# dpkn31/Yade-OpenFOAM-coupling

Hardware: AMD Instinct MI355X
Metric: coupled_steps_per_sec (pimpleFoamYade 4-way, 10M particles / 4M cells per GPU) (higher is better)
Workload: dtype f64

## Files before the change

### yade-openfoam-coupling_amd/csrc/common.hpp

```cpp
#pragma once
#include <hip/hip_runtime.h>

#include <algorithm>
#include <cmath>
#include <cstdarg>
#include <cstdint>
#include <cstdio>
#include <cstring>
#include <string>
#include <vector>

#include "../../include/foamyade_hip.h"

namespace fy {

struct Options {
    std::string tree_cache_dir;
    int rebin_interval;
    int strip_blocks;
    bool halo_overlap;
    int ipc_slot_mb;
    long long ipc_timeout_ms;
    bool wire_trace;
    bool explicit_tree;
    bool no_locate_lists;
    int locate_stack;
    bool locate_wide;
    bool no_deep_vcycle;
    long long mg_replicate_below;
    bool localcomm_stream;
    bool no_fused_corrector;
    bool faces_from_arrays;
    bool no_pairs;
    bool no_tail_cache;
    int ipc_slot_kb;
};
Options options();

std::string& last_error();
int fail(int code, const char* fmt, ...);
bool pairs_disabled();
bool tail_cache_disabled();
bool locate_wide_forced();

#define FY_HIP(expr)                                                                                      \
    do {                                                                                                  \
        hipError_t _e = (expr);                                                                           \
        if (_e != hipSuccess)                                                                             \
            return ::fy::fail(FY_ERR_HIP, "%s failed: %s (%s:%d)", #expr, hipGetErrorString(_e), __FILE__, __LINE__); \
    } while (0)

#define FY_TRY(expr)                 \
    do {                             \
        int _rc = (expr);            \
        if (_rc != FY_OK) return _rc; \
    } while (0)

template <class T>
struct DevBuf {
    T* p = nullptr;
    size_t n = 0;
    DevBuf() = default;
    DevBuf(const DevBuf&) = delete;
    DevBuf& operator=(const DevBuf&) = delete;
    ~DevBuf() { release(); }
    void release() {
        if (p) (void)hipFree(p);
        p = nullptr;
        n = 0;
    }
    int reserve(size_t count) {
        if (count <= n) return FY_OK;
        release();
        size_t cap = count + count / 8 + 64;
        hipError_t e = hipMalloc((void**)&p, cap * sizeof(T));
        if (e != hipSuccess) {
            p = nullptr;
            return fail(FY_ERR_HIP, "hipMalloc(%zu bytes) failed: %s", cap * sizeof(T), hipGetErrorString(e));
        }
        n = cap;
        return FY_OK;
    }
    int alloc_exact(size_t count) {
        release();
        if (count == 0) return FY_OK;
        hipError_t e = hipMalloc((void**)&p, count * sizeof(T));
        if (e != hipSuccess) {
            p = nullptr;
            return fail(FY_ERR_HIP, "hipMalloc(%zu bytes) failed: %s", count * sizeof(T), hipGetErrorString(e));
        }
        n = count;
        return FY_OK;
    }
};

template <class T>
struct HostBuf {
    T* p = nullptr;
    size_t n = 0;
    HostBuf() = default;
    HostBuf(const HostBuf&) = delete;
    HostBuf& operator=(const HostBuf&) = delete;
    ~HostBuf() { release(); }
    void release() {
        if (p) (void)hipHostFree(p);
        p = nullptr;
        n = 0;
    }
    T* data() { return p; }
    T& operator[](size_t i) { return p[i]; }
    int reserve(size_t count) {
        if (count <= n) return FY_OK;
        release();
        const size_t cap = count + count / 8 + 64;
        hipError_t e = hipHostMalloc((void**)&p, cap * sizeof(T), hipHostMallocDefault);
        if (e != hipSuccess) {
            p = nullptr;
            return fail(FY_ERR_HIP, "hipHostMalloc(%zu bytes) failed: %s", cap * sizeof(T), hipGetErrorString(e));
        }
        n = cap;
        return FY_OK;
    }
};

struct EventTimer {
    hipEvent_t a = nullptr, b = nullptr;
    bool armed = false;
    int init() {
        FY_HIP(hipEventCreate(&a));
        FY_HIP(hipEventCreate(&b));
        return FY_OK;
    }
    void destroy() {
        if (a) (void)hipEventDestroy(a);
        if (b) (void)hipEventDestroy(b);
        a = b = nullptr;
    }
    void start(hipStream_t s) { (void)hipEventRecord(a, s); armed = true; }
    void stop(hipStream_t s) { (void)hipEventRecord(b, s); }
    double ms() {
        if (!armed) return 0.0;
        float t = 0.f;
        (void)hipEventSynchronize(b);
        (void)hipEventElapsedTime(&t, a, b);
        armed = false;
        return (double)t;
    }
};

struct PhaseMarks {
    static constexpr int kMax = 8;
    hipEvent_t ev[kMax] = {};
    bool set_[kMax] = {};
    int init() { for (auto& e : ev) FY_HIP(hipEventCreate(&e)); return FY_OK; }
    void destroy() { for (auto& e : ev) { if (e) (void)hipEventDestroy(e); e = nullptr; } }
    void clear() { for (auto& b : set_) b = false; }
    void mark(int i, hipStream_t s) { (void)hipEventRecord(ev[i], s); set_[i] = true; }
    double ms(int i, int j) {
        if (!set_[i] || !set_[j]) return 0.0;
        float t = 0.f;
        (void)hipEventSynchronize(ev[j]);
        (void)hipEventElapsedTime(&t, ev[i], ev[j]);
        return (double)t;
    }
};

struct KernelClock {
    std::vector<hipEvent_t> a, b;
    size_t used = 0;
    double total_ms = 0.0;
    int64_t launches = 0;
    bool on = false;
    size_t per_collect = 1;
    bool open_ = false;
    void begin(hipStream_t s) {
        open_ = false;
        if (!on || used >= per_collect) return;
        if (used == a.size()) { hipEvent_t x, y; (void)hipEventCreate(&x); (void)hipEventCreate(&y); a.push_back(x); b.push_back(y); }
        (void)hipEventRecord(a[used], s);
        open_ = true;
    }
    void end(hipStream_t s) {
        if (!open_) return;
        (void)hipEventRecord(b[used], s);
        ++used;
// ... 21 lines not shown
```

### yade-openfoam-coupling_amd/csrc/coupling.cpp

```cpp
#include "coupling.hpp"
#include "ldu.hpp"

#include <algorithm>
#include <cmath>
#include <chrono>
#include <cstdlib>
#include <functional>
#include <thread>

#include <sys/stat.h>
#include <unistd.h>

#include <atomic>

namespace fy {

static std::atomic<int> g_kernel_flags{-1};
static bool kernel_flag(int bit) {
    if (g_kernel_flags.load(std::memory_order_relaxed) < 0) (void)options();
    return (g_kernel_flags.load(std::memory_order_relaxed) >> bit) & 1;
}
bool pairs_disabled() { return kernel_flag(0); }
bool tail_cache_disabled() { return kernel_flag(1); }
bool locate_wide_forced() { return kernel_flag(2); }

Options options() {
    auto on = [](const char* nm) { const char* e = getenv(nm); return e != nullptr && *e != 0 && strcmp(e, "0") != 0; };
    auto num = [](const char* nm, long long unset) { const char* e = getenv(nm); return e ? atoll(e) : unset; };
    Options q{};
    if (const char* d = getenv("FOAMYADE_TREE_CACHE_DIR")) q.tree_cache_dir = d;
    q.rebin_interval = std::max(1, (int)num("FOAMYADE_REBIN_INTERVAL", 32));
    q.strip_blocks = (int)num("FOAMYADE_STRIP_BLOCKS", -1);
    q.halo_overlap = getenv("FOAMYADE_HALO_OVERLAP") == nullptr || on("FOAMYADE_HALO_OVERLAP");
    q.ipc_slot_mb = (int)num("FOAMYADE_IPC_SLOT_MB", 0);
    q.ipc_timeout_ms = num("FOAMYADE_IPC_TIMEOUT_MS", 0);
    q.wire_trace = getenv("FOAMYADE_WIRE_TRACE") != nullptr;
    q.explicit_tree = on("FOAMYADE_EXPLICIT_TREE");
    q.no_locate_lists = on("FOAMYADE_NO_LOCATE_LISTS");
    q.locate_stack = (int)num("FOAMYADE_LOCATE_STACK", -1);
    q.locate_wide = num("FOAMYADE_LOCATE_WIDE", 0) != 0;
    q.no_deep_vcycle = on("FOAMYADE_NO_DEEP_VCYCLE");
    q.mg_replicate_below = std::max(0LL, num("FOAMYADE_MG_REPLICATE_BELOW", 0));
    const char* ls = getenv("FOAMYADE_LOCALCOMM_STREAM");
    q.localcomm_stream = ls != nullptr && ls[0] == '1';
    q.no_fused_corrector = on("FOAMYADE_NO_FUSED_CORRECTOR");
    q.faces_from_arrays = on("FOAMYADE_FACES_FROM_ARRAYS");
    q.no_pairs = on("FOAMYADE_NO_PAIRS");
    q.no_tail_cache = on("FOAMYADE_NO_TAIL_CACHE");
    q.ipc_slot_kb = (int)num("FOAMYADE_IPC_SLOT_KB", 0);
    g_kernel_flags.store((q.no_pairs ? 1 : 0) | (q.no_tail_cache ? 2 : 0) | (q.locate_wide ? 4 : 0), std::memory_order_relaxed);
    return q;
}

std::string& last_error() {
    static thread_local std::string e;
    return e;
}

int fail(int code, const char* fmt, ...) {
    char buf[1024];
    va_list ap;
    va_start(ap, fmt);
    vsnprintf(buf, sizeof(buf), fmt, ap);
    va_end(ap);
    last_error() = buf;
    return code;
}

static const int TAG_SZ_BUFF = 1003, TAG_GRID_BBOX = 1001, TAG_YADE_DATA = 1002, TAG_FORCE = 1005, TAG_SEARCH_RES = 1004,
                 TAG_FLUID_DT = 1050, TAG_YADE_DT = 1060;

#define FY_TR(expr)                                                                             \
    do {                                                                                        \
        if ((expr) != 0) return fail(FY_ERR_TRANSPORT, "transport call failed: %s", #expr);     \
    } while (0)

int Coupling::create(const fy_mesh_desc* m, const fy_field_ptrs* f, int gaussian_interp, const fy_transport* tr, int device_ordinal) {
    if (!m || !f || m->n_cells <= 0 || !m->centres || !m->volumes) return fail(FY_ERR_INVALID, "fy_create: bad mesh/fields");
    int ndev = 0;
    if (hipGetDeviceCount(&ndev) != hipSuccess || ndev == 0)
        return fail(FY_ERR_NO_DEVICE, "no HIP device visible: libfoamyade_hip has no CPU path");
    if (device_ordinal < 0 || device_ordinal >= ndev) return fail(FY_ERR_INVALID, "device ordinal %d out of range (%d devices)", device_ordinal, ndev);
    device = device_ordinal;
    opt = options();
    FY_HIP(hipSetDevice(device));
    if (ext_stream) { stream = ext_stream; owns_stream = false; }
    else { FY_HIP(hipStreamCreate(&stream)); owns_stream = true; }
    mesh = *m;
    mesh.centres = nullptr; mesh.volumes = nullptr; mesh.xf = mesh.yf = mesh.zf = nullptr;
    n_cells = m->n_cells;
    gaussian = gaussian_interp != 0;
    structured = m->nx > 0;
    rectilinear = structured && m->xf && m->yf && m->zf;
    if (!gaussian && !structured && !ldu_geo) return fail(FY_ERR_UNSUPPORTED, "point-force mode needs the structured block description, or a general mesh's face addressing (fy_ldu_solver): the findCell stand-ins");
    if (structured && (int64_t)m->nx * m->ny * m->nz != m->n_cells) return fail(FY_ERR_INVALID, "nx*ny*nz != n_cells");
    if (tr) { transport = *tr; has_transport = true; }

    if (has_transport) {
        comm_sz_diff = std::abs(transport.world_size - transport.local_size);
        serial_yade = (comm_sz_diff == 1);
    } else {
        comm_sz_diff = 0; serial_yade = true;
    }

    {
        bool exact = structured && !rectilinear && !opt.explicit_tree && m->nx <= 1024 && m->ny <= 1024 && m->nz <= 4096 &&
                     n_cells < (1 << 25);
        if (exact)
            for (int k = 0; k < m->nz && exact; ++k) for (int j = 0; j < m->ny && exact; ++j) for (int i = 0; i < m->nx; ++i) {
                const size_t c = (size_t)i + (size_t)m->nx * (j + (size_t)m->ny * k);
                const double x = m->origin[0] + ((double)i + 0.5) * m->dx, y = m->origin[1] + ((double)j + 0.5) * m->dx, z = m->origin[2] + ((double)k + 0.5) * m->dx;
                if (x != m->centres[3 * c] || y != m->centres[3 * c + 1] || z != m->centres[3 * c + 2]) { exact = false; break; }
            }
        std::vector<int32_t> pre;
        std::string cache;
        const std::string& cache_dir = opt.tree_cache_dir;
        if (exact && !cache_dir.empty()) {
            char nm[512];
            snprintf(nm, sizeof(nm), "%s/fy_tree_%dx%dx%d_%016llx.bin", cache_dir.c_str(), m->nx, m->ny, m->nz,
                     (unsigned long long)(std::hash<double>()(m->dx) ^ (std::hash<double>()(m->origin[0]) << 1) ^ (std::hash<double>()(m->origin[1]) << 2) ^ (std::hash<double>()(m->origin[2]) << 3)));
            cache = nm;
        }
        auto load_cache = [&]() -> bool {
            FILE* f = fopen(cache.c_str(), "rb");
            if (!f) return false;
            pre.resize((size_t)n_cells);
            bool ok = fread(pre.data(), sizeof(int32_t), (size_t)n_cells, f) == (size_t)n_cells && fgetc(f) == EOF;
            fclose(f);
            for (size_t q = 0; ok && q < pre.size(); ++q) ok = pre[q] >= 0 && pre[q] < n_cells;
            if (!ok) pre.clear();
            return ok;
        };
        bool have = false, hold_lock = false;
        const std::string lock = cache + ".lock";
        if (!cache.empty()) {
            have = load_cache();
            if (!have) {
                const double kStaleLock = 60.0;
                auto lock_age = [&]() -> double {
                    struct stat sb;
                    if (stat(lock.c_str(), &sb) != 0) return -1.0;
                    return difftime(time(nullptr), sb.st_mtime);
                };
                for (int attempt = 0; attempt < 2 && !have && !hold_lock; ++attempt) {
                    FILE* lf = fopen(lock.c_str(), "wx");
                    if (lf) { fclose(lf); hold_lock = true; break; }
                    const int max_spins = (int)(kStaleLock * 20);
                    for (int spin = 0; spin < max_spins && !have; ++spin) {
                        const double age = lock_age();
                        if (age < 0 || age > kStaleLock) break;
                        std::this_thread::sleep_for(std::chrono::milliseconds(50));
                        have = load_cache();
                    }
                    if (!have) have = load_cache();
                    if (!have && lock_age() > kStaleLock) remove(lock.c_str());
                }
            }
        }
        const bool publish = !cache.empty() && !have;
        std::vector<KdNode> nodes;
        if (!have) {
            unsigned hw = std::thread::hardware_concurrency();
            build_kdtree_preorder(m->centres, n_cells, nodes, (int)std::min(hw ? hw : 1u, 8u));
            pre.resize((size_t)n_cells);
            for (size_t q = 0; q < nodes.size(); ++q) pre[q] = nodes[q].id;
            if (publish) {
                char sfx[64];
                snprintf(sfx, sizeof(sfx), ".tmp.%ld.%zx", (long)getpid(), std::hash<std::thread::id>()(std::this_thread::get_id()));
                const std::string tmp = cache + sfx;
                bool ok = false;
                if (FILE* f = fopen(tmp.c_str(), "wb")) {
                    ok = fwrite(pre.data(), sizeof(int32_t), pre.size(), f) == pre.size();
                    ok = (fclose(f) == 0) && ok;
                }
                if (!ok || rename(tmp.c_str(), cache.c_str()) != 0) remove(tmp.c_str());
            }
        }
        if (hold_lock) remove(lock.c_str());
        tree_levels = kdtree_levels(n_cells);
        if (exact) {
            std::vector<uint32_t> packed((size_t)n_cells);
            for (size_t q = 0; q < packed.size(); ++q) {
                const int id = pre[q];
                const int i = id % m->nx, j = (id / m->nx) % m->ny, k = id / (m->nx * m->ny);
                packed[q] = (uint32_t)i | ((uint32_t)j << 10) | ((uint32_t)k << 20);
            }
            FY_TRY(d_tree_packed.alloc_exact(packed.size()));
            FY_HIP(hipMemcpyAsync(d_tree_packed.p, packed.data(), packed.size() * sizeof(uint32_t), hipMemcpyHostToDevice, stream));
            implicit.ox = m->origin[0]; implicit.oy = m->origin[1]; implicit.oz = m->origin[2]; implicit.dx = m->dx;
            implicit.nx = m->nx; implicit.ny = m->ny; implicit.nz = m->nz;
            use_implicit = true;
            FY_HIP(hipStreamSynchronize(stream));
        } else {
            if (nodes.empty()) {
                build_kdtree_preorder(m->centres, n_cells, nodes, 1);
            }
            FY_TRY(d_tree.alloc_exact(nodes.size()));
            FY_HIP(hipMemcpyAsync(d_tree.p, nodes.data(), nodes.size() * sizeof(KdNode), hipMemcpyHostToDevice, stream));
            FY_HIP(hipStreamSynchronize(stream));
// ... 1238 lines not shown
```

### yade-openfoam-coupling_amd/csrc/fv_kernels.hip

```cpp
#include "fv_kernels.hpp"

#include "common.hpp"

#ifndef FY_FVK_GRADED
#define FY_FVK_GRADED 0
#endif

namespace fy {
#if FY_FVK_GRADED
namespace gr {
#endif
namespace {

constexpr double kSmall = 1e-15;

__device__ __forceinline__ void ijk_of(const FvGeo& g, int t, int& i, int& j, int& k) {
    i = t % g.nx;
    const int q = t / g.nx;
    j = q % g.ny;
    k = q / g.ny;
}
__device__ __forceinline__ int cidx(const FvGeo& g, int i, int j, int k) { return i + g.nx * (j + g.ny * (k + g.gz)); }
__device__ __forceinline__ int stride_of(const FvGeo& g, int d) { return d == 0 ? 1 : d == 1 ? g.nx : g.nx * g.ny; }
__device__ __forceinline__ size_t g_row_stride(const FvGeo& g) { return 3 * (size_t)g.nx * g.ny * (size_t)(g.nz + 2 * g.gz); }
// ... 426 lines not shown
    } else {
        const int c = cidx(g, i, j, k);
        fl = af * rAUf[f] * geo_sfd_face(g, D, q, ndim(g, D), i, j, k) * (p[c] - p[c - stride_of(g, D)]);
    }
    const double fa = fl / af;
    pflux[f] = g.pimple ? (phiForces[f] - fa) / rAUf[f] : fl;
    phi[f] = phiHbyA[f] - fa;
}
__global__ __launch_bounds__(256) void k_flux_correct_cells(FvGeo g, const double* __restrict__ p, CFace3 phiHbyA, CFace3 rAUf, CFace3 alphaf, CFace3 psn,
                                                            CFace3 phiForces, Face3 pflux, Face3 phi) {
    const int t = fv_block(g, blockIdx.x, gridDim.x) * 256 + (int)threadIdx.x;
    if (t >= g.Nc) return;
    int i, j, k; ijk_of(g, t, i, j, k);
#define FY_CALL(D, fi, fj, fk) { const size_t f = (size_t)fid(g, D, fi, fj, fk); \
        flux_correct_face<D>(g, f, fi, fj, fk, p, phiHbyA.a[D], rAUf.a[D], alphaf.a[D], psn.a[D], phiForces.a[D], pflux.a[D], phi.a[D]); }
    FY_CELL_FACES(g, i, j, k, FY_CALL);
#undef FY_CALL
}

__global__ __launch_bounds__(256) void k_courant(FvGeo g, CFace3 phi, double* __restrict__ partials) {
    double v[2] = {0.0, 0.0};
    FY_RED_LOOP_G(g, t) {
        int i, j, k; ijk_of(g, t, i, j, k);
        double s = 0.0;
#pragma unroll
        for (int d = 0; d < 3; ++d)
#pragma unroll
            for (int sd = 0; sd < 2; ++sd) s += fabs(phi.a[d][cface(g, d, sd, i, j, k)]);
        v[0] = fmax(v[0], s * geo_rV(g, i, j, k));
        v[1] += s;
    }
    const int mx[2] = {1, 0};
    block_reduce_store<2>(v, mx, partials, fy_lb, fy_stride);
}

__global__ __launch_bounds__(256) void k_pre_coupling(FvGeo g, const double* __restrict__ U, const double* __restrict__ p,
                                                      const double* __restrict__ alpha, CFace3 psn, double* __restrict__ vGrad,
                                                      double* __restrict__ gradP, double* __restrict__ divT, double* __restrict__ Gout,
                                                      int write_vgrad, int write_pfields, CFace3 phi, double* __restrict__ ddtU, double* __restrict__ Uold_out,
                                                      double* __restrict__ cellrec, double rec_two_nu, double rec_rhoF, Face3 dcorr) {
    const int t = fv_block(g, blockIdx.x, gridDim.x) * 256 + (int)threadIdx.x;
    if (t >= g.Nc) return;
    int i, j, k; ijk_of(g, t, i, j, k);
    const int c = t + g.c0;
    const bool pf = g.pimple && write_pfields;
    const int ijk[3] = {i, j, k};
    bool bnd[3][2];
#pragma unroll
    for (int d = 0; d < 3; ++d)
#pragma unroll
        for (int s = 0; s < 2; ++s) bnd[d][s] = onb(g, d, s, i, j, k);
    const double uc[3] = {U[3 * (size_t)c], U[3 * (size_t)c + 1], U[3 * (size_t)c + 2]};
    const double pc = pf ? p[c] : 0.0, ac = pf ? alpha[c] : 0.0;
    double un6[3][2][3], pn6[3][2], an6[3][2];
#pragma unroll
    for (int d = 1; d < 3; ++d)
#pragma unroll
        for (int s = 0; s < 2; ++s) {
            const int nb = bnd[d][s] ? c : c + (s ? stride_of(g, d) : -stride_of(g, d));
            un6[d][s][0] = U[3 * (size_t)nb]; un6[d][s][1] = U[3 * (size_t)nb + 1]; un6[d][s][2] = U[3 * (size_t)nb + 2];
            pn6[d][s] = pf ? p[nb] : 0.0; an6[d][s] = pf ? alpha[nb] : 0.0;
        }
    const bool want_phi = ddtU != nullptr || dcorr.a[0] != nullptr;
    double phf[3][2];
#pragma unroll
    for (int d = 0; d < 3; ++d)
#pragma unroll
        for (int s = 0; s < 2; ++s) phf[d][s] = want_phi ? phi.a[d][cface(g, d, s, i, j, k)] : 0.0;
    const int lane = threadIdx.x & 63;
    {
        const int xm = (lane == 0 && i > 0) ? c - 1 : c, xp = (lane == 63 && i + 1 < g.nx) ? c + 1 : c;
        double em[3] = {0, 0, 0}, ep[3] = {0, 0, 0}, epm = 0, epp = 0, eam = 0, eap = 0;
        if (lane == 0 || lane == 63) {
            for (int q = 0; q < 3; ++q) { em[q] = U[3 * (size_t)xm + q]; ep[q] = U[3 * (size_t)xp + q]; }
            if (pf) { epm = p[xm]; epp = p[xp]; eam = alpha[xm]; eap = alpha[xp]; }
        }
#pragma unroll
        for (int q = 0; q < 3; ++q) { un6[0][0][q] = wave_prev(uc[q]); un6[0][1][q] = wave_next(uc[q]); }
        pn6[0][0] = wave_prev(pc); pn6[0][1] = wave_next(pc); an6[0][0] = wave_prev(ac); an6[0][1] = wave_next(ac);
        if (lane == 0 && i > 0) { for (int q = 0; q < 3; ++q) un6[0][0][q] = em[q]; pn6[0][0] = epm; an6[0][0] = eam; }
        if (lane == 63 && i + 1 < g.nx) { for (int q = 0; q < 3; ++q) un6[0][1][q] = ep[q]; pn6[0][1] = epp; an6[0][1] = eap; }
    }
    if (Uold_out) { Uold_out[3 * (size_t)c] = uc[0]; Uold_out[3 * (size_t)c + 1] = uc[1]; Uold_out[3 * (size_t)c + 2] = uc[2]; }
    double lap[3] = {0, 0, 0}, T[9], conv[3] = {0, 0, 0}, gp3[3] = {0, 0, 0};
#pragma unroll
    for (int d = 0; d < 3; ++d) {
        double fv[2][3], fp[2] = {0, 0};
#pragma unroll
        for (int s = 0; s < 2; ++s) {
            if (bnd[d][s]) {
                const int patch = 2 * d + s;
                if (g.u_bc[patch] == 0) { fv[s][0] = g.u_val[patch][0]; fv[s][1] = g.u_val[patch][1]; fv[s][2] = g.u_val[patch][2]; }
                else { fv[s][0] = uc[0]; fv[s][1] = uc[1]; fv[s][2] = uc[2]; }
                if (g.u_bc[patch] == 2) fv[s][d] = 0.0;
                if (pf) {
                    fp[s] = pbv(g, p, psn, c, d, s, cface(g, d, s, i, j, k));
                    for (int q = 0; q < 3; ++q) lap[q] += 1.0 * geo_Af(g, d, i, j, k) * (fv[s][q] - uc[q]) * geo_rhalf(g, d, ijk[d]);
                }
            } else {
                const double* un = un6[d][s];
                const int qc = ijk[d];
                for (int q = 0; q < 3; ++q) fv[s][q] = geo_lerp_side(g, d, s, qc, uc[q], un[q]);
                if (pf) {
                    fp[s] = geo_lerp_side(g, d, s, qc, pc, pn6[d][s]);
                    const double af = geo_lerp_side(g, d, s, qc, ac, an6[d][s]);
                    for (int q = 0; q < 3; ++q) lap[q] += af * geo_Af(g, d, i, j, k) * (un[q] - uc[q]) * geo_rdelta(g, d, qc + s);
                }
            }
        }
        if (dcorr.a[0]) {
#pragma unroll
            for (int s = 0; s < 2; ++s)
                if (owns_face(g, d, s, i, j, k)) {
                    const int fi = i + (d == 0 ? s : 0), fj = j + (d == 1 ? s : 0), fk = k + (d == 2 ? s : 0);
                    const int f = cface(g, d, s, i, j, k);
                    const double uf = fv[s][d] * geo_Af(g, d, fi, fj, fk);
                    const double po = phf[d][s];
                    const double phiCorr = po - uf;
                    const bool fixes = bnd[d][s] && g.u_bc[2 * d + s] == 0;
                    const double coef = fixes ? 0.0 : 1.0 - fmin(fabs(phiCorr) / (fabs(po) + kSmall), 1.0);
                    dcorr.a[d][f] = coef * (1.0 / g.dt) * phiCorr;
                }
        }
        const double rhd = geo_rh(g, d, ijk[d]);
        for (int q = 0; q < 3; ++q) T[3 * d + q] = (fv[1][q] - fv[0][q]) * rhd;
        if (pf) gp3[d] = (fp[1] - fp[0]) * rhd;
        if (ddtU) {
#pragma unroll
            for (int s = 0; s < 2; ++s) {
                const double flux = (s ? 1.0 : -1.0) * phf[d][s];
                for (int q = 0; q < 3; ++q) conv[q] += flux * fv[s][q];
            }
        }
    }
    if (ddtU)
        for (int q = 0; q < 3; ++q) ddtU[3 * (size_t)c + q] = conv[q] * geo_rV(g, i, j, k);
    if (write_vgrad)
        for (int q = 0; q < 9; ++q) vGrad[9 * (size_t)c + q] = T[q];
    if (pf)
        for (int q = 0; q < 3; ++q) gradP[3 * (size_t)c + q] = gp3[q];
    if (pf) {
        double dT[3];
        for (int q = 0; q < 3; ++q) { dT[q] = 2 * g.nu * (lap[q] * geo_rV(g, i, j, k)); divT[3 * (size_t)c + q] = dT[q]; }
        if (cellrec) {
            double2* r = reinterpret_cast<double2*>(cellrec + 8 * (size_t)c);
            r[0] = make_double2(uc[0], uc[1]);
            r[1] = make_double2(uc[2], ac);
            r[2] = make_double2(((rec_two_nu * dT[0]) * rec_rhoF) - gp3[0], ((rec_two_nu * dT[1]) * rec_rhoF) - gp3[1]);
            r[3] = make_double2(((rec_two_nu * dT[2]) * rec_rhoF) - gp3[2], geo_V(g, i, j, k));
        }
    }
    if (Gout) {
        const double tr = T[0] + T[4] + T[8];
        const double an = g.nut ? alpha[c] * (g.nu + g.nut[c]) : alpha[c] * g.nu;
        const size_t rs = g_row_stride(g);
        for (int a = 0; a < 3; ++a)
            for (int b = 0; b < 3; ++b) Gout[(size_t)a * rs + 3 * (size_t)c + b] = an * (T[3 * b + a] - (a == b ? (2.0 / 3.0) * tr : 0.0));
    }
}

__global__ __launch_bounds__(256) void k_div_G(FvGeo g, const double* __restrict__ G, double* __restrict__ divG) {
    const int t = fv_block(g, blockIdx.x, gridDim.x) * 256 + (int)threadIdx.x;
    if (t >= g.Nc) return;
    int i, j, k; ijk_of(g, t, i, j, k);
    const int c = t + g.c0;
    const int ijk[3] = {i, j, k};
    const double g0[3] = {G[3 * (size_t)c], G[3 * (size_t)c + 1], G[3 * (size_t)c + 2]};
    double gx[2][3];
    x_neighbours3(G, c, i, g.nx, g0, gx[0], gx[1]);
    bool bnd[3][2];
    double own[3][3], nbv[3][2][3];
#pragma unroll
    for (int q = 0; q < 3; ++q) { own[0][q] = g0[q]; nbv[0][0][q] = gx[0][q]; nbv[0][1][q] = gx[1][q]; }
#pragma unroll
    for (int d = 0; d < 3; ++d)
#pragma unroll
        for (int s = 0; s < 2; ++s) bnd[d][s] = onb(g, d, s, i, j, k);
#pragma unroll
    for (int d = 1; d < 3; ++d) {
        const double* Gd = G + (size_t)d * g_row_stride(g);
#pragma unroll
        for (int q = 0; q < 3; ++q) own[d][q] = Gd[3 * (size_t)c + q];
#pragma unroll
        for (int s = 0; s < 2; ++s) {
            const int nb = bnd[d][s] ? c : c + (s ? stride_of(g, d) : -stride_of(g, d));
#pragma unroll
            for (int q = 0; q < 3; ++q) nbv[d][s][q] = Gd[3 * (size_t)nb + q];
        }
    }
    double acc[3] = {0, 0, 0};
#pragma unroll
    for (int d = 0; d < 3; ++d) {
        double fv[2][3];
#pragma unroll
        for (int s = 0; s < 2; ++s)
            for (int q = 0; q < 3; ++q) fv[s][q] = bnd[d][s] ? own[d][q] : geo_lerp_side(g, d, s, ijk[d], own[d][q], nbv[d][s][q]);
        for (int q = 0; q < 3; ++q) acc[q] += (fv[1][q] - fv[0][q]) * geo_rh(g, d, ijk[d]);
    }
    for (int q = 0; q < 3; ++q) divG[3 * (size_t)c + q] = acc[q];
}

__global__ __launch_bounds__(256) void k_smagorinsky_nut(FvGeo g, const double* __restrict__ vGrad, double ck, double ce, double delta, double* __restrict__ nut) {
    const int t = blockIdx.x * 256 + threadIdx.x;
    if (t >= g.Nc) return;
    const int c = t + g.c0;
    delta = geo_delta(g, delta, c);
    double T[9];
#pragma unroll
    for (int q = 0; q < 9; ++q) T[q] = vGrad[9 * (size_t)c + q];
    const double Dxx = T[0], Dyy = T[4], Dzz = T[8];
    const double Dxy = 0.5 * (T[1] + T[3]), Dxz = 0.5 * (T[2] + T[6]), Dyz = 0.5 * (T[5] + T[7]);
    const double trD = Dxx + Dyy + Dzz;
    const double a = ce / delta;
    const double b = (2.0 / 3.0) * trD;
    const double third = (1.0 / 3.0) * trD;
    const double dd = (Dxx - third) * Dxx + (Dyy - third) * Dyy + (Dzz - third) * Dzz + 2.0 * (Dxy * Dxy) + 2.0 * (Dxz * Dxz) + 2.0 * (Dyz * Dyz);
    const double cc = 2.0 * ck * delta * dd;
    const double r = (-b + sqrt(b * b + 4.0 * a * cc)) / (2.0 * a);
    const double kk = r * r;
    nut[c] = ck * delta * sqrt(kk);
}

__device__ __forceinline__ double wall_epsilon(const FvGeo& g, const TurbEqn& e, double kc, int c, int i, int j, int k) {
#if FY_FVK_GRADED
    double sum = 0.0;
    int W = 0;
#pragma unroll
    for (int d = 0; d < 3; ++d)
#pragma unroll
        for (int s = 0; s < 2; ++s)
            if (e.wall[2 * d + s] && onb(g, d, s, i, j, k)) { sum += e.cmu75 * pow(kc, 1.5) / (e.kappa * geo_ywall(g, d, c)); ++W; }
    return sum / (double)W;
#else
    return e.cmu75 * pow(kc, 1.5) / (e.kappa * geo_ywall(g, 0, c));
#endif
}

__global__ __launch_bounds__(256) void k_assemble_turb(FvGeo g, TurbEqn e, const double* __restrict__ kf, const double* __restrict__ ef,
                                                       const double* __restrict__ alpha, CFace3 alphaf, CFace3 phi, const double* __restrict__ vGrad,
                                                       const double* __restrict__ U, Mom7 M, double* __restrict__ b3, double* __restrict__ x3) {
    const int t = blockIdx.x * 256 + threadIdx.x;
    if (t >= g.Nc) return;
    int i, j, k; ijk_of(g, t, i, j, k);
    const int c = t + g.c0;
    const double nu = g.nu, dt = g.dt, V = geo_V(g, i, j, k);
    const double aP = alpha[c], nutc = g.nut[c];
    const double* X = e.mode == 1 ? ef : kf;
    const double xc = X[c];
    double dg = aP * V / dt;
    double src = aP * V * xc / dt;
    double sumPhi = 0.0, an[6];
#pragma unroll
    for (int d = 0; d < 3; ++d)
#pragma unroll
        for (int s = 0; s < 2; ++s) {
            const int f = cface(g, d, s, i, j, k);
            const double af = alphaf.a[d][f];
            const double pv = (s ? 1.0 : -1.0) * phi.a[d][f];
            const double phio = af * pv;
            sumPhi += pv;
            if (onb(g, d, s, i, j, k)) {
                an[2 * d + s] = 0.0;
                const int patch = 2 * d + s;
                const double nb = nut_boundary(g, patch, c);
                const double gam = (af * (nu + nb / e.sigma)) * geo_sfd(g, d, s, i, j, k);
                if (e.bc[patch] == 1) {
                    const double gb = kBfac * gam;
                    dg += gb;
                    src += (-phio + gb) * e.val[patch];
                } else {
                    dg += phio;
                }
            } else {
                const int nbc = c + (s ? stride_of(g, d) : -stride_of(g, d));
                const int qc = d == 0 ? i : d == 1 ? j : k;
                const double gam = geo_lerp_side(g, d, s, qc, aP * (nu + nutc / e.sigma), alpha[nbc] * (nu + g.nut[nbc] / e.sigma)) * geo_sfd(g, d, s, i, j, k);
                const double wP = geo_wown(g, d, s, qc);
#if FY_FVK_GRADED
                const double cP = e.upwind ? fmax(phio, 0.0) : wP * phio, cN = e.upwind ? fmin(phio, 0.0) : (1.0 - wP) * phio;
#else
                const double cP = e.upwind ? fmax(phio, 0.0) : wP * phio, cN = e.upwind ? fmin(phio, 0.0) : wP * phio;
#endif
                dg += cP + gam;
                an[2 * d + s] = cN - gam;
            }
        }
    double T[9];
#pragma unroll
    for (int q = 0; q < 9; ++q) T[q] = vGrad[9 * (size_t)c + q];
    const double tr2 = 2.0 * (T[0] + T[4] + T[8]);
    double GG = 0.0;
#pragma unroll
    for (int a = 0; a < 3; ++a)
#pragma unroll
        for (int b = 0; b < 3; ++b) GG += T[3 * a + b] * ((T[3 * a + b] + T[3 * b + a]) - (a == b ? (1.0 / 3.0) * tr2 : 0.0));
    double G = nutc * GG;
    int Wc = 0;
    double Gw = 0.0;
    if (e.mode != 0) {
#pragma unroll
        for (int d = 0; d < 3; ++d)
#pragma unroll
            for (int s = 0; s < 2; ++s)
                if (e.wall[2 * d + s] && onb(g, d, s, i, j, k)) {
                    const int patch = 2 * d + s;
                    double ub[3];
                    Ub(g, U, c, patch, ub);
                    const double ywall = geo_ywall(g, d, c);
                    const double d0 = (ub[0] - U[3 * (size_t)c]) / ywall, d1 = (ub[1] - U[3 * (size_t)c + 1]) / ywall, d2 = (ub[2] - U[3 * (size_t)c + 2]) / ywall;
                    const double magGradUw = sqrt(d0 * d0 + d1 * d1 + d2 * d2);
                    Gw += (nut_boundary(g, patch, c) + nu) * magGradUw * e.cmu25 * sqrt(kf[c]) / (e.kappa * ywall);
                    ++Wc;
                }
        if (Wc) G = Gw / (double)Wc;
    }
    const double divU = sumPhi * geo_rV(g, i, j, k);
    double Su, c1, c2;
    if (e.mode == 0) { Su = aP * G; c1 = (2.0 / 3.0) * aP * divU; c2 = e.ce * aP * sqrt(xc) / geo_delta(g, e.delta, c); }
    else if (e.mode == 1) { const double kc = kf[c]; Su = e.c1 * aP * G * xc / kc; c1 = ((2.0 / 3.0) * e.c1 - e.c3) * aP * divU; c2 = e.c2 * aP * xc / kc; }
    else { Su = aP * G; c1 = (2.0 / 3.0) * aP * divU; c2 = aP * ef[c] / xc; }
    dg += V * (fmax(c1, 0.0) + c2);
    src += V * Su - V * fmin(c1, 0.0) * xc;
    if (e.relax > 0) {
        double so = 0.0;
        for (int q = 0; q < 6; ++q) so += fabs(an[q]);
        const double dn = fmax(fabs(dg), so) / e.relax;
        src += (dn - dg) * xc;
        dg = dn;
    }
    double x0 = xc;
    if (e.mode == 1) {
        if (Wc) {
            const double v = wall_epsilon(g, e, kf[c], c, i, j, k);
            for (int q = 0; q < 6; ++q) an[q] = 0.0;
            src = dg * v;
            x0 = v;
        } else {
#pragma unroll
            for (int d = 0; d < 3; ++d)
#pragma unroll
                for (int s = 0; s < 2; ++s)
                    if (!onb(g, d, s, i, j, k)) {
                        const int ni = i + (d == 0 ? (s ? 1 : -1) : 0), nj = j + (d == 1 ? (s ? 1 : -1) : 0), nk = k + (d == 2 ? (s ? 1 : -1) : 0);
                        bool nwall = false;
#pragma unroll
                        for (int d2 = 0; d2 < 3; ++d2)
#pragma unroll
                            for (int s2 = 0; s2 < 2; ++s2) nwall = nwall || (e.wall[2 * d2 + s2] && onb(g, d2, s2, ni, nj, nk));
                        if (nwall) {
                            const int nbc = c + (s ? stride_of(g, d) : -stride_of(g, d));
                            src -= an[2 * d + s] * wall_epsilon(g, e, kf[nbc], nbc, ni, nj, nk);
                            an[2 * d + s] = 0.0;
                        }
                    }
        }
    }
    M.diag[c] = dg;
    for (int q = 0; q < 6; ++q) M.an[q][c] = an[q];
    b3[3 * (size_t)c] = src; b3[3 * (size_t)c + 1] = 0.0; b3[3 * (size_t)c + 2] = 0.0;
    x3[3 * (size_t)c] = x0; x3[3 * (size_t)c + 1] = 0.0; x3[3 * (size_t)c + 2] = 0.0;
}

__global__ __launch_bounds__(256) void k_turb_finish(FvGeo g, TurbEqn e, const double* __restrict__ x3, double* __restrict__ Xf, int nut_mode, double cmu,
                                                     const double* __restrict__ ef, double* __restrict__ nut) {
    const int t = blockIdx.x * 256 + threadIdx.x;
    if (t >= g.Nc) return;
    int i, j, k; ijk_of(g, t, i, j, k);
    const int c = t + g.c0;
    const double xc = x3[3 * (size_t)c];
    double xb = xc;
    if (!(xc > 0.0)) {
        const double mP = fmax(xc, e.xmin);
        double av = 0.0;
#if FY_FVK_GRADED
        double asum = 0.0;
#endif
#pragma unroll
        for (int d = 0; d < 3; ++d)
#pragma unroll
            for (int s = 0; s < 2; ++s) {
                double xf;
                if (onb(g, d, s, i, j, k)) {
                    const int patch = 2 * d + s;
                    xf = fmax(e.bc[patch] == 1 ? e.val[patch] : xc, e.xmin);
                } else {
                    const int nbc = c + (s ? stride_of(g, d) : -stride_of(g, d));
                    xf = geo_lerp_side(g, d, s, d == 0 ? i : d == 1 ? j : k, mP, fmax(x3[3 * (size_t)nbc], e.xmin));
                }
#if FY_FVK_GRADED
                const double Afc = geo_Af(g, d, i, j, k);
                av += Afc * xf; asum += Afc;
#else
                av += xf;
#endif
            }
#if FY_FVK_GRADED
        xb = fmax(xc, av / asum);
#else
        xb = fmax(xc, av / 6.0);
#endif
    }
    xb = fmax(xb, e.xmin);
    Xf[c] = xb;
    if (nut_mode == 1) nut[c] = e.ck * sqrt(xb) * geo_delta(g, e.delta, c);
    else if (nut_mode == 2) nut[c] = cmu * (xb * xb) / ef[c];
}

__device__ __forceinline__ double magsqr3(const double* __restrict__ F, int c) {
    const double a = F[3 * (size_t)c], b = F[3 * (size_t)c + 1], e = F[3 * (size_t)c + 2];
    return (a * a + b * b) + e * e;
}
__global__ __launch_bounds__(256) void k_grad_magsqr(FvGeo g, const double* __restrict__ U, double* __restrict__ gradL) {
    const int t = blockIdx.x * 256 + threadIdx.x;
    if (t >= g.Nc) return;
    int i, j, k; ijk_of(g, t, i, j, k);
    const int c = t + g.c0;
    const double lc = magsqr3(U, c);
#pragma unroll
    for (int d = 0; d < 3; ++d) {
        double fv[2];
#pragma unroll
        for (int s = 0; s < 2; ++s) {
            if (onb(g, d, s, i, j, k)) { double b[3]; Ub(g, U, c, 2 * d + s, b); fv[s] = (b[0] * b[0] + b[1] * b[1]) + b[2] * b[2]; }
            else fv[s] = geo_lerp_side(g, d, s, d == 0 ? i : d == 1 ? j : k, lc, magsqr3(U, c + (s ? stride_of(g, d) : -stride_of(g, d))));
        }
        gradL[3 * (size_t)c + d] = (fv[1] - fv[0]) * geo_rh(g, d, d == 0 ? i : d == 1 ? j : k);
    }
}
__device__ __forceinline__ double limiter_fn(int scheme, double twoByk, double r) {
    switch (scheme) {
        case 3: return fmax(fmin(twoByk * r, 1.0), 0.0);
        case 4: return (r + fabs(r)) / (1.0 + fabs(r));
        case 5: return fmax(fmin(fmin(2.0 * r, 0.5 * r + 0.5), 2.0), 0.0);
        case 6: return fmax(fmin(fmin(r, 1.0), 2.0), 0.0);
        case 7: return fmax(fmax(fmin(2.0 * r, 1.0), fmin(r, 2.0)), 0.0);
        default: return fmax(fmin((3.0 + r) / 4.0, 2.0), 0.0);
    }
}
__device__ __forceinline__ double limited_weight(const FvGeo& g, const double* __restrict__ U, const double* __restrict__ gradL, int d, int qn, int own,
                                                 int nei, double flux) {
    const double gradf = magsqr3(U, nei) - magsqr3(U, own);
    const double gradcf = (1.0 / geo_rdelta(g, d, qn)) * gradL[3 * (size_t)(flux > 0 ? own : nei) + d];
    double r;
    if (fabs(gradcf) >= 1000.0 * fabs(gradf)) r = 2.0 * 1000.0 * (gradcf >= 0 ? 1.0 : -1.0) * (gradf >= 0 ? 1.0 : -1.0) - 1.0;
    else r = 2.0 * (gradcf / gradf) - 1.0;
    const double lim = limiter_fn(g.upwind, g.lim_twoByk, r);
#if FY_FVK_GRADED
    const double wl = geo_wlow(g, d, qn);
#else
    const double wl = 0.5;
#endif
    return lim * wl + (1.0 - lim) * (flux >= 0 ? 1.0 : 0.0);
}

template <bool LIMITED>
__global__ __launch_bounds__(256) void k_assemble_momentum(FvGeo g, const double* __restrict__ U, const double* __restrict__ Uold,
                                                           const double* __restrict__ alpha, const double* __restrict__ alphaOld, CFace3 alphaf,
                                                           CFace3 phi, const double* __restrict__ uSource, const double* __restrict__ uSourceDrag,
                                                           const double* __restrict__ divG, const double* __restrict__ vGrad, Mom7 M,
                                                           double* __restrict__ src, double* __restrict__ rAU) {
    const int t = fv_block(g, blockIdx.x, gridDim.x) * 256 + (int)threadIdx.x;
    if (t >= g.Nc) return;
    int i, j, k; ijk_of(g, t, i, j, k);
    const int c = t + g.c0;
    const double nu = g.nu, dt = g.dt, V = geo_V(g, i, j, k);
    const bool pim = g.pimple != 0;
    const double aP = pim ? alpha[c] : 1.0, aP0 = pim ? alphaOld[c] : 1.0;
    double dg = aP * V / dt;
    double s3[3];
    for (int q = 0; q < 3; ++q) s3[q] = aP0 * V * Uold[3 * (size_t)c + q] / dt;
    double divAPhi = 0.0, an[6];
    double bd[3] = {0.0, 0.0, 0.0};
#pragma unroll
    for (int d = 0; d < 3; ++d)
#pragma unroll
        for (int s = 0; s < 2; ++s) {
            const int f = cface(g, d, s, i, j, k);
            double af = 1.0;
            if (pim) {
                if (alphaf.a[0]) af = alphaf.a[d][f];
                else if (!onb(g, d, s, i, j, k)) af = lerp_face(g, d, s, (d == 0 ? i : d == 1 ? j : k) + s, aP, alpha[c + (s ? stride_of(g, d) : -stride_of(g, d))]);
            }
            const double phio = (s ? 1.0 : -1.0) * af * phi.a[d][f];
            divAPhi += phio;
            const double geo = geo_sfd(g, d, s, i, j, k);
            double gam = nu * af * geo;
            if (g.nut) {
                if (onb(g, d, s, i, j, k)) {
                    const double nb = nut_boundary(g, 2 * d + s, c);
                    gam = (af * (nu + nb)) * geo;
                } else {
                    const int nbc = c + (s ? stride_of(g, d) : -stride_of(g, d));
                    gam = geo_lerp_side(g, d, s, d == 0 ? i : d == 1 ? j : k, aP * (nu + g.nut[c]), alpha[nbc] * (nu + g.nut[nbc])) * geo;
                }
            }
            if (onb(g, d, s, i, j, k)) {
                an[2 * d + s] = 0.0;
                const int patch = 2 * d + s;
                if (g.u_bc[patch] == 0) {
                    const double gb = kBfac * gam;
                    dg += gb;
                    for (int q = 0; q < 3; ++q) s3[q] += (-phio + gb) * g.u_val[patch][q];
                } else {
                    if (g.u_bc[patch] == 2) bd[d] += kBfac * gam;
                    dg += phio;
                }
            } else {
                const double wP = geo_wown(g, d, s, d == 0 ? i : d == 1 ? j : k);
#if FY_FVK_GRADED
                double cP = g.upwind ? fmax(phio, 0.0) : wP * phio, cN = g.upwind ? fmin(phio, 0.0) : (1.0 - wP) * phio;
#else
                double cP = g.upwind ? fmax(phio, 0.0) : wP * phio, cN = g.upwind ? fmin(phio, 0.0) : wP * phio;
#endif
                if (LIMITED) {
                    const int nb = c + (s ? stride_of(g, d) : -stride_of(g, d));
                    const int qc = d == 0 ? i : d == 1 ? j : k;
                    const double w = limited_weight(g, U, vGrad, d, qc + s, s ? c : nb, s ? nb : c, af * phi.a[d][f]);
                    cP = s ? phio * w : phio * (1.0 - w);
                    cN = s ? phio * (1.0 - w) : phio * w;
                }
                dg += cP + gam;
                an[2 * d + s] = cN - gam;
                if (g.upwind == 2) {
                    const int nb = c + (s ? stride_of(g, d) : -stride_of(g, d));
                    const int uw = phio > 0.0 ? c : nb;
                    const double half = (phio > 0.0 ? (s ? 0.5 : -0.5) : (s ? -0.5 : 0.5)) * geo_hc(g, d, uw);
                    for (int q = 0; q < 3; ++q) s3[q] -= phio * (half * vGrad[9 * (size_t)uw + 3 * d + q]);
                }
            }
        }
    if (pim) {
        const double S = (alpha[c] - alphaOld[c]) / dt + divAPhi / V;
        dg -= V * S;
        dg -= V * uSourceDrag[c];
        for (int q = 0; q < 3; ++q) s3[q] += V * divG[3 * (size_t)c + q];
        double so = 0.0;
        for (int q = 0; q < 6; ++q) so += fabs(an[q]);
        if (g.u_relax > 0) {
            const double dn = fmax(fabs(dg + ((bd[0] + bd[1]) + bd[2])), so) / g.u_relax;
            for (int q = 0; q < 3; ++q) s3[q] += (dn - dg) * U[3 * (size_t)c + q];
            dg = dn;
        }
    } else {
        for (int q = 0; q < 3; ++q) s3[q] += V * uSource[3 * (size_t)c + q];
    }
    M.diag[c] = dg;
    for (int q = 0; q < 6; ++q) M.an[q][c] = an[q];
    for (int q = 0; q < 3; ++q) src[3 * (size_t)c + q] = s3[q];
    double bav = 0.0;
    if (M.bd) { for (int q = 0; q < 3; ++q) M.bd[3 * (size_t)c + q] = bd[q]; bav = ((bd[0] + bd[1]) + bd[2]) / 3.0; }
    rAU[c] = 1.0 / ((dg + bav) / V);
}

__global__ __launch_bounds__(256) void k_bmom(FvGeo g, const double* __restrict__ src, const double* __restrict__ p, CFace3 psn,
                                              CFace3 phiForces, CFace3 rAUf, double* __restrict__ bmom) {
    const int t = fv_block(g, blockIdx.x, gridDim.x) * 256 + (int)threadIdx.x;
    if (t >= g.Nc) return;
    int i, j, k; ijk_of(g, t, i, j, k);
    const int c = t + g.c0;
    double out[3];
#pragma unroll
    for (int d = 0; d < 3; ++d) {
        if (!g.pimple) {
            double fv[2];
#pragma unroll
            for (int s = 0; s < 2; ++s) {
                if (onb(g, d, s, i, j, k)) fv[s] = pbv(g, p, psn, c, d, s, cface(g, d, s, i, j, k));
                else fv[s] = geo_lerp_side(g, d, s, d == 0 ? i : d == 1 ? j : k, p[c], p[c + (s ? stride_of(g, d) : -stride_of(g, d))]);
            }
            out[d] = src[3 * (size_t)c + d] - geo_V(g, i, j, k) * ((fv[1] - fv[0]) * geo_rh(g, d, d == 0 ? i : d == 1 ? j : k));
        } else {
            double sm = 0;
#pragma unroll
            for (int s = 0; s < 2; ++s) {
                const int f = cface(g, d, s, i, j, k);
                double sng;
                const double rds = geo_rdist(g, d, s, i, j, k);
                if (onb(g, d, s, i, j, k)) { const double pbd = pbv(g, p, psn, c, d, s, f); sng = s ? (pbd - p[c]) * rds : (p[c] - pbd) * rds; }
                else sng = s ? (p[c + stride_of(g, d)] - p[c]) * rds : (p[c] - p[c - stride_of(g, d)]) * rds;
                sm += phiForces.a[d][f] / rAUf.a[d][f] - sng * geo_Af(g, d, i, j, k);
            }
            out[d] = src[3 * (size_t)c + d] + geo_V(g, i, j, k) * (sm / (2.0 * geo_Af(g, d, i, j, k)));
        }
    }
    for (int d = 0; d < 3; ++d) bmom[3 * (size_t)c + d] = out[d];
}

__global__ __launch_bounds__(256) void k_bmom_faces(FvGeo g, const double* __restrict__ rAU, const double* __restrict__ uSource, const double* __restrict__ src,
                                                    const double* __restrict__ p, CFace3 psn, Face3 rf_out, Face3 pf_out, double* __restrict__ bmom) {
    const int t = fv_block(g, blockIdx.x, gridDim.x) * 256 + (int)threadIdx.x;
    if (t >= g.Nc) return;
    int i, j, k; ijk_of(g, t, i, j, k);
    const int c = t + g.c0;
    const int ijk[3] = {i, j, k};
    bool bnd[3][2]; int nb[3][2], fx[3][2];
#pragma unroll
    for (int d = 0; d < 3; ++d)
#pragma unroll
        for (int s = 0; s < 2; ++s) {
            bnd[d][s] = onb(g, d, s, i, j, k);
            nb[d][s] = bnd[d][s] ? c : c + (s ? stride_of(g, d) : -stride_of(g, d));
            fx[d][s] = cface(g, d, s, i, j, k);
        }
    const double rc = rAU[c], pc = p[c];
    const double us[3] = {uSource[3 * (size_t)c], uSource[3 * (size_t)c + 1], uSource[3 * (size_t)c + 2]};
    const double sr[3] = {src[3 * (size_t)c], src[3 * (size_t)c + 1], src[3 * (size_t)c + 2]};
    double rn[3][2], un[3][2], pn[3][2];
#pragma unroll
    for (int d = 0; d < 3; ++d)
#pragma unroll
        for (int s = 0; s < 2; ++s) { rn[d][s] = rAU[nb[d][s]]; un[d][s] = uSource[3 * (size_t)nb[d][s] + d]; pn[d][s] = p[nb[d][s]]; }
    double out[3];
#pragma unroll
    for (int d = 0; d < 3; ++d) {
        double sm = 0;
#pragma unroll
        for (int s = 0; s < 2; ++s) {
            const int q = ijk[d] + s;
            const int fi = i + (d == 0 ? s : 0), fj = j + (d == 1 ? s : 0), fk = k + (d == 2 ? s : 0);
            const bool b = bnd[d][s];
            const double Afc = geo_Af(g, d, fi, fj, fk);
            const double r = b ? rc : lerp_face(g, d, s, q, rc, rn[d][s]);
            const double fl = b ? 0.0 : lerp_face(g, d, s, q, rc * us[d], rn[d][s] * un[d][s]) * Afc;
            const double pfv = fl + r * (g.g[d] * Afc);
            if (owns_face(g, d, s, i, j, k)) { pf_out.a[d][fx[d][s]] = pfv; if (rf_out.a[0]) rf_out.a[d][fx[d][s]] = r; }
            double sng;
            const double rds = geo_rdist(g, d, s, i, j, k);
            if (b) { const double pbd = pbv(g, p, psn, c, d, s, fx[d][s]); sng = s ? (pbd - pc) * rds : (pc - pbd) * rds; }
            else sng = s ? (pn[d][s] - pc) * rds : (pc - pn[d][s]) * rds;
            sm += pfv / r - sng * geo_Af(g, d, i, j, k);
        }
        out[d] = sr[d] + geo_V(g, i, j, k) * (sm / (2.0 * geo_Af(g, d, i, j, k)));
    }
    for (int d = 0; d < 3; ++d) bmom[3 * (size_t)c + d] = out[d];
}

template <bool WITH_H>
__global__ __launch_bounds__(256) void k_mom_pass(FvGeo g, Mom7 M, const double* __restrict__ b, const double* __restrict__ x,
                                                  double* __restrict__ xn, const double* __restrict__ xsum, double n_glob, double* __restrict__ partials,
                                                  const double* __restrict__ hsrc, const double* __restrict__ rAU, double* __restrict__ HbyA) {
    double v[6] = {0, 0, 0, 0, 0, 0};
    const double xb[3] = {xsum[0] / n_glob, xsum[1] / n_glob, xsum[2] / n_glob};
    FY_RED_LOOP_G(g, t) {
        int i, j, k; ijk_of(g, t, i, j, k);
        const int c = t + g.c0;
        const double dg = M.diag[c];
        double dq[3] = {dg, dg, dg};
        if (M.bd) for (int q = 0; q < 3; ++q) dq[q] += M.bd[3 * (size_t)c + q];
        double off[3] = {0, 0, 0}, rowsum = dg;
        const double xc[3] = {x[3 * (size_t)c], x[3 * (size_t)c + 1], x[3 * (size_t)c + 2]};
        double hacc[3] = {0, 0, 0};
        if (WITH_H) { hacc[0] = hsrc[3 * (size_t)c]; hacc[1] = hsrc[3 * (size_t)c + 1]; hacc[2] = hsrc[3 * (size_t)c + 2]; }
        double xx[2][3];
        x_neighbours3(x, c, i, g.nx, xc, xx[0], xx[1]);
#pragma unroll
        for (int d = 0; d < 3; ++d)
#pragma unroll
            for (int s = 0; s < 2; ++s)
                if (!onb(g, d, s, i, j, k)) {
                    const int nb = c + (s ? stride_of(g, d) : -stride_of(g, d));
                    const double a = M.an[2 * d + s][c];
                    rowsum += a;
                    double xv[3];
                    if (d == 0) for (int q = 0; q < 3; ++q) xv[q] = xx[s][q];
                    else for (int q = 0; q < 3; ++q) xv[q] = x[3 * (size_t)nb + q];
                    for (int q = 0; q < 3; ++q) off[q] += a * xv[q];
                    if (WITH_H) for (int q = 0; q < 3; ++q) hacc[q] -= a * xv[q];
                }
        if (WITH_H) {
            if (M.bd) {
                const double b0 = M.bd[3 * (size_t)c], b1 = M.bd[3 * (size_t)c + 1], b2 = M.bd[3 * (size_t)c + 2];
                const double bav = ((b0 + b1) + b2) / 3.0;
                hacc[0] += (bav - b0) * xc[0]; hacc[1] += (bav - b1) * xc[1]; hacc[2] += (bav - b2) * xc[2];
            }
            const double r = rAU[c];
            for (int q = 0; q < 3; ++q) HbyA[3 * (size_t)c + q] = r * (hacc[q] * geo_rV(g, i, j, k));
        }
        for (int q = 0; q < 3; ++q) {
            const double bq = b[3 * (size_t)c + q];
            const double Ax = dq[q] * xc[q] + off[q];
            const double Aref = (rowsum + (dq[q] - dg)) * xb[q];
            v[q] += fabs(bq - Ax);
            v[3 + q] += fabs(Ax - Aref) + fabs(bq - Aref);
            xn[3 * (size_t)c + q] = (bq - off[q]) / dq[q];
        }
    }
    const int mx[6] = {0, 0, 0, 0, 0, 0};
    block_reduce_store<6>(v, mx, partials, fy_lb, fy_stride);
// ... 23 lines not shown
                const double a = M.an[2 * d + s][c];
                for (int q = 0; q < 3; ++q) acc[q] -= a * U[3 * (size_t)nb + q];
            }
    if (M.bd) {
        const double b0 = M.bd[3 * (size_t)c], b1 = M.bd[3 * (size_t)c + 1], b2 = M.bd[3 * (size_t)c + 2];
        const double bav = ((b0 + b1) + b2) / 3.0;
        acc[0] += (bav - b0) * U[3 * (size_t)c]; acc[1] += (bav - b1) * U[3 * (size_t)c + 1]; acc[2] += (bav - b2) * U[3 * (size_t)c + 2];
    }
    const double r = rAU[c];
    for (int q = 0; q < 3; ++q) HbyA[3 * (size_t)c + q] = r * (acc[q] * geo_rV(g, i, j, k));
}

template <bool MATRIX>
__global__ __launch_bounds__(256) void k_assemble_pressure(FvGeo g, CFace3 phiHbyA, CFace3 rAUf, CFace3 alphaf, CFace3 psn,
                                                           const double* __restrict__ alpha, const double* __restrict__ alphaOld, PMat A,
                                                           double* __restrict__ rhs) {
    const int t = fv_block(g, blockIdx.x, gridDim.x) * 256 + (int)threadIdx.x;
    if (t >= g.Nc) return;
    int i, j, k; ijk_of(g, t, i, j, k);
    const int c = t + g.c0;
    const bool refc = g.need_ref && (i + g.nx * (j + g.ny * (k + g.kglob0))) == g.p_ref_cell;
    double dg = 0.0, r = 0.0, up[3] = {0, 0, 0};
#pragma unroll
    for (int d = 0; d < 3; ++d)
#pragma unroll
        for (int s = 0; s < 2; ++s) {
            const int f = cface(g, d, s, i, j, k);
            const double af = g.pimple ? alphaf.a[d][f] : 1.0;
            double ph = (s ? 1.0 : -1.0) * af * phiHbyA.a[d][f];
            const bool b = onb(g, d, s, i, j, k);
            if (b && g.p_bc[2 * d + s] == 2) ph = (s ? 1.0 : -1.0) * af * (phiHbyA.a[d][f] - rAUf.a[d][f] * geo_Af(g, d, i, j, k) * psn.a[d][f]);
            r -= ph;
            if (b) {
                const int patch = 2 * d + s;
                if (g.p_bc[patch] == 1) { const double gb = kBfac * af * rAUf.a[d][f] * geo_sfd(g, d, s, i, j, k); dg += gb; r += gb * g.p_val[patch]; }
            } else if (MATRIX || refc) {
                const double gg = af * rAUf.a[d][f] * geo_sfd(g, d, s, i, j, k);
                dg += gg;
                if (s) up[d] = gg;
            }
        }
    if (g.pimple) r -= geo_V(g, i, j, k) * (alpha[c] - alphaOld[c]) / g.dt;
    if (refc) { r += dg * g.p_ref_value; dg += dg; }
    if (MATRIX) { A.diag[c] = dg; A.ux[c] = up[0]; A.uy[c] = up[1]; A.uz[c] = up[2]; }
    rhs[c] = r;
}

__global__ __launch_bounds__(256) void k_p_ghost_uz(FvGeo g, CFace3 rAUf, CFace3 alphaf, PMat A) {
    const int t = blockIdx.x * 256 + threadIdx.x;
    if (t >= g.nx * g.ny) return;
    const double af = g.pimple ? alphaf.a[2][t] : 1.0;
    A.uz[g.c0 - g.nx * g.ny + t] = af * rAUf.a[2][t] * g.dx;
}

__global__ __launch_bounds__(256) void k_cont_err(FvGeo g, CFace3 phi, CFace3 alphaf, const double* __restrict__ alpha,
                                                  const double* __restrict__ alphaOld, double* __restrict__ partials) {
    double v[2] = {0, 0};
    FY_RED_LOOP_G(g, t) {
        int i, j, k; ijk_of(g, t, i, j, k);
        const int c = t + g.c0;
        double dv = 0;
#pragma unroll
        for (int d = 0; d < 3; ++d)
#pragma unroll
            for (int s = 0; s < 2; ++s) { const int f = cface(g, d, s, i, j, k); dv += (s ? 1.0 : -1.0) * (g.pimple ? alphaf.a[d][f] : 1.0) * phi.a[d][f]; }
        double ce = dv * geo_rV(g, i, j, k);
        if (g.pimple) ce += (alpha[c] - alphaOld[c]) / g.dt;
        v[0] += fabs(ce) * geo_V(g, i, j, k);
        v[1] += ce * geo_V(g, i, j, k);
    }
    const int mx[2] = {0, 0};
    block_reduce_store<2>(v, mx, partials, fy_lb, fy_stride);
}

template <bool DIAG>
__global__ __launch_bounds__(256) void k_U_correct(FvGeo g, const double* __restrict__ HbyA, const double* __restrict__ rAU,
                                                   const double* __restrict__ p, CFace3 psn, CFace3 phiForces, CFace3 pflux, CFace3 alphaf,
                                                   CFace3 rAUf, double* __restrict__ U, CFace3 phi, const double* __restrict__ alpha,
                                                   const double* __restrict__ alphaOld, double* __restrict__ partials) {
    double v[4] = {0, 0, 0, 0};
    FY_RED_LOOP_G(g, t) {
        int i, j, k; ijk_of(g, t, i, j, k);
        const int c = t + g.c0;
        const double r = rAU[c];
        double out[3];
        double dv = 0.0, sp = 0.0;
#pragma unroll
        for (int d = 0; d < 3; ++d) {
            if (!g.pimple) {
                double fv[2];
#pragma unroll
                for (int s = 0; s < 2; ++s) {
                    if (onb(g, d, s, i, j, k)) fv[s] = pbv(g, p, psn, c, d, s, cface(g, d, s, i, j, k));
                    else fv[s] = geo_lerp_side(g, d, s, d == 0 ? i : d == 1 ? j : k, p[c], p[c + (s ? stride_of(g, d) : -stride_of(g, d))]);
                }
                out[d] = HbyA[3 * (size_t)c + d] - r * ((fv[1] - fv[0]) * geo_rh(g, d, d == 0 ? i : d == 1 ? j : k));
            } else {
                double sm = 0;
#pragma unroll
                for (int s = 0; s < 2; ++s) sm += pflux.a[d][cface(g, d, s, i, j, k)];
                out[d] = HbyA[3 * (size_t)c + d] + r * (sm / (2.0 * geo_Af(g, d, i, j, k)));
            }
            if (DIAG) {
#pragma unroll
                for (int s = 0; s < 2; ++s) {
                    const int f = cface(g, d, s, i, j, k);
                    const double ph = phi.a[d][f];
                    dv += (s ? 1.0 : -1.0) * (g.pimple ? alphaf.a[d][f] : 1.0) * ph;
                    sp += fabs(ph);
                }
            }
        }
        for (int d = 0; d < 3; ++d) U[3 * (size_t)c + d] = out[d];
        if (DIAG) {
            double ce = dv * geo_rV(g, i, j, k);
            if (g.pimple) ce += (alpha[c] - alphaOld[c]) / g.dt;
            v[0] += fabs(ce) * geo_V(g, i, j, k);
            v[1] += ce * geo_V(g, i, j, k);
            v[2] = fmax(v[2], sp * geo_rV(g, i, j, k));
            v[3] += sp;
        }
    }
    if (DIAG) {
        const int mx[4] = {0, 0, 1, 0};
        block_reduce_store<4>(v, mx, partials, fy_lb, fy_stride);
    }
}

struct FaceSrc { CFace3 arr; const double* cell; };
template <int D>
__device__ __forceinline__ double alphaf_at(const FvGeo& g, const FaceSrc& a, size_t f, int fi, int fj, int fk) {
    if (!a.cell) return a.arr.a[D][f];
    const int q = D == 0 ? fi : D == 1 ? fj : fk;
    if (face_low_b(g, D, q) || face_high_b(g, D, q)) return 1.0;
    const int c = cidx(g, fi, fj, fk);
    return geo_lerp(g, D, q, a.cell[c - stride_of(g, D)], a.cell[c]);
}
template <int D>
__device__ __forceinline__ double rAUf_at(const FvGeo& g, const FaceSrc& a, size_t f, int fi, int fj, int fk) {
    if (!a.cell) return a.arr.a[D][f];
    const int q = D == 0 ? fi : D == 1 ? fj : fk;
    if (face_low_b(g, D, q)) return a.cell[cidx(g, fi, fj, fk)];
    if (face_high_b(g, D, q)) return a.cell[cidx(g, fi - (D == 0), fj - (D == 1), fk - (D == 2))];
    const int c = cidx(g, fi, fj, fk);
    return geo_lerp(g, D, q, a.cell[c - stride_of(g, D)], a.cell[c]);
}
#define FY_ALL_FACES(i, j, k, CALL) \
    do { CALL(0, 0, i, j, k); CALL(0, 1, i + 1, j, k); CALL(1, 0, i, j, k); CALL(1, 1, i, j + 1, k); CALL(2, 0, i, j, k); CALL(2, 1, i, j, k + 1); } while (0)


__device__ __forceinline__ double ub_normal(const FvGeo& g, int patch, int d, double own_d) {
    return g.u_bc[patch] == 0 ? g.u_val[patch][d] : (g.u_bc[patch] == 2 ? 0.0 : own_d);
}
template <bool DIAG, bool FFC>
__global__ __launch_bounds__(256) void k_corr_back(FvGeo g, const double* __restrict__ p, CFace3 phiHbyA, FaceSrc rAUf, FaceSrc alphaf, CFace3 psn,
                                                   CFace3 phiForces, Face3 phi, const double* __restrict__ HbyA, const double* __restrict__ rAU,
                                                   double* __restrict__ U, const double* __restrict__ alpha, const double* __restrict__ alphaOld,
                                                   double* __restrict__ partials) {
    double v[4] = {0, 0, 0, 0};
    FY_RED_LOOP_G(g, t) {
        int i, j, k; ijk_of(g, t, i, j, k);
        const int c = t + g.c0;
        const int ijk[3] = {i, j, k};
        const bool pim = g.pimple != 0;
        bool bnd[3][2]; int nb[3][2], fx[3][2];
#pragma unroll
        for (int d = 0; d < 3; ++d)
#pragma unroll
            for (int s = 0; s < 2; ++s) {
                bnd[d][s] = onb(g, d, s, i, j, k);
                nb[d][s] = bnd[d][s] ? c : c + (s ? stride_of(g, d) : -stride_of(g, d));
                fx[d][s] = cface(g, d, s, i, j, k);
            }
        const double pc = p[c], rc = rAU[c], ac = pim ? alpha[c] : 1.0;
        const double hb[3] = {HbyA[3 * (size_t)c], HbyA[3 * (size_t)c + 1], HbyA[3 * (size_t)c + 2]};
        double pn[3][2], rfv[3][2], afv[3][2], phh[3][2], pfo[3][2];
#pragma unroll
        for (int d = 0; d < 3; ++d)
#pragma unroll
            for (int s = 0; s < 2; ++s) {
                pn[d][s] = p[nb[d][s]];
                phh[d][s] = phiHbyA.a[d][fx[d][s]];
                pfo[d][s] = pim ? phiForces.a[d][fx[d][s]] : 0.0;
                if (FFC) { rfv[d][s] = rAU[nb[d][s]]; afv[d][s] = pim ? alpha[nb[d][s]] : 1.0; }
                else { rfv[d][s] = rAUf.arr.a[d][fx[d][s]]; afv[d][s] = pim ? alphaf.arr.a[d][fx[d][s]] : 1.0; }
            }
        double pfl[3][2], ph[3][2];
#pragma unroll
        for (int d = 0; d < 3; ++d)
#pragma unroll
            for (int s = 0; s < 2; ++s) {
                const int q = ijk[d] + s;
                const int fi = i + (d == 0 ? s : 0), fj = j + (d == 1 ? s : 0), fk = k + (d == 2 ? s : 0);
                const bool b = bnd[d][s];
                if (FFC) {
                    afv[d][s] = pim ? (b ? 1.0 : lerp_face(g, d, s, q, ac, afv[d][s])) : 1.0;
                    rfv[d][s] = b ? rc : lerp_face(g, d, s, q, rc, rfv[d][s]);
                }
                const double af = afv[d][s], rf = rfv[d][s];
                double fl = 0.0;
                if (b) {
                    const int patch = 2 * d + s;
                    if (g.p_bc[patch] == 1) { const double gb = kBfac * af * rf * geo_sfd_face(g, d, q, ndim(g, d), fi, fj, fk); fl = s ? gb * (g.p_val[patch] - pc) : gb * (pc - g.p_val[patch]); }
                    else if (g.p_bc[patch] == 2) fl = af * rf * geo_Af(g, d, fi, fj, fk) * psn.a[d][fx[d][s]];
                } else {
                    fl = af * rf * geo_sfd_face(g, d, q, ndim(g, d), fi, fj, fk) * (s ? pn[d][s] - pc : pc - pn[d][s]);
                }
                const double fa = fl / af;
                pfl[d][s] = pim ? (pfo[d][s] - fa) / rf : fl;
                ph[d][s] = phh[d][s] - fa;
                if (owns_face(g, d, s, i, j, k)) phi.a[d][fx[d][s]] = ph[d][s];
            }
        double out[3];
        double dv = 0.0, sp = 0.0;
#pragma unroll
        for (int d = 0; d < 3; ++d) {
            if (!pim) {
                double fv[2];
#pragma unroll
                for (int s = 0; s < 2; ++s) {
                    if (bnd[d][s]) fv[s] = pbv(g, p, psn, c, d, s, fx[d][s]);
                    else fv[s] = geo_lerp_side(g, d, s, ijk[d], pc, pn[d][s]);
                }
                out[d] = hb[d] - rc * ((fv[1] - fv[0]) * geo_rh(g, d, ijk[d]));
            } else {
                double sm = 0;
#pragma unroll
                for (int s = 0; s < 2; ++s) sm += pfl[d][s];
                out[d] = hb[d] + rc * (sm / (2.0 * geo_Af(g, d, i, j, k)));
            }
            if (DIAG) {
#pragma unroll
                for (int s = 0; s < 2; ++s) {
                    dv += (s ? 1.0 : -1.0) * (pim ? afv[d][s] : 1.0) * ph[d][s];
                    sp += fabs(ph[d][s]);
                }
            }
        }
        for (int d = 0; d < 3; ++d) U[3 * (size_t)c + d] = out[d];
        if (DIAG) {
            double ce = dv * geo_rV(g, i, j, k);
            if (pim) ce += (ac - alphaOld[c]) / g.dt;
            v[0] += fabs(ce) * geo_V(g, i, j, k);
            v[1] += ce * geo_V(g, i, j, k);
            v[2] = fmax(v[2], sp * geo_rV(g, i, j, k));
            v[3] += sp;
        }
    }
    if (DIAG) {
        const int mx[4] = {0, 0, 1, 0};
        block_reduce_store<4>(v, mx, partials, fy_lb, fy_stride);
    }
}

template <bool STORE_A, bool FFC>
__global__ __launch_bounds__(256) __attribute__((amdgpu_waves_per_eu(4))) void k_corr_front(FvGeo g, const double* __restrict__ HbyA, const double* __restrict__ U, CFace3 dcorr,
                                                    FaceSrc rAUf, FaceSrc alphaf, CFace3 phiForces, Face3 phiHbyA, Face3 psn,
                                                    const double* __restrict__ rAU, const double* __restrict__ alpha, const double* __restrict__ alphaOld, PMat A,
                                                    double* __restrict__ rhs, const double* __restrict__ x, const double* __restrict__ xbar_dev, double xsum_val,
                                                    double inv_n, double* __restrict__ res, double* __restrict__ partials) {
    double v[2] = {0, 0};
    const double xbar = (xbar_dev ? xbar_dev[0] : xsum_val) * inv_n;
    FY_RED_LOOP_G(g, t) {
        int i, j, k; ijk_of(g, t, i, j, k);
        const int c = t + g.c0;
        const int ijk[3] = {i, j, k};
        const bool pim = g.pimple != 0;
        const bool refc = g.need_ref && (i + g.nx * (j + g.ny * (k + g.kglob0))) == g.p_ref_cell;
        bool bnd[3][2]; int nb[3][2], fx[3][2];
#pragma unroll
        for (int d = 0; d < 3; ++d)
#pragma unroll
            for (int s = 0; s < 2; ++s) {
                bnd[d][s] = onb(g, d, s, i, j, k);
                nb[d][s] = bnd[d][s] ? c : c + (s ? stride_of(g, d) : -stride_of(g, d));
                fx[d][s] = cface(g, d, s, i, j, k);
            }
        const double xc = x[c], ac = pim ? alpha[c] : 1.0;
        const double rc = FFC ? rAU[c] : 0.0;
        const double hb[3] = {HbyA[3 * (size_t)c], HbyA[3 * (size_t)c + 1], HbyA[3 * (size_t)c + 2]};
        double hn[3][2], dc[3][2], pfo[3][2], xn[3][2], rfv[3][2], afv[3][2];
#pragma unroll
        for (int d = 0; d < 3; ++d)
#pragma unroll
            for (int s = 0; s < 2; ++s) {
                hn[d][s] = HbyA[3 * (size_t)nb[d][s] + d];
                dc[d][s] = dcorr.a[d][fx[d][s]];
                pfo[d][s] = pim ? phiForces.a[d][fx[d][s]] : 0.0;
                xn[d][s] = x[nb[d][s]];
                if (FFC) { rfv[d][s] = rAU[nb[d][s]]; afv[d][s] = pim ? alpha[nb[d][s]] : 1.0; }
                else { rfv[d][s] = rAUf.arr.a[d][fx[d][s]]; afv[d][s] = pim ? alphaf.arr.a[d][fx[d][s]] : 1.0; }
            }
        double dg = 0.0, r = 0.0, up[3] = {0, 0, 0};
        double gg6[3][2];
#pragma unroll
        for (int d = 0; d < 3; ++d)
#pragma unroll
            for (int s = 0; s < 2; ++s) {
                const int q = ijk[d] + s;
                const int fi = i + (d == 0 ? s : 0), fj = j + (d == 1 ? s : 0), fk = k + (d == 2 ? s : 0);
                const bool b = bnd[d][s];
                const int patch = 2 * d + s;
                if (FFC) {
                    afv[d][s] = pim ? (b ? 1.0 : lerp_face(g, d, s, q, ac, afv[d][s])) : 1.0;
                    rfv[d][s] = b ? rc : lerp_face(g, d, s, q, rc, rfv[d][s]);
                }
                const double af = afv[d][s], rf = rfv[d][s];
                const double Afc = geo_Af(g, d, fi, fj, fk);
                double pv = (b ? ub_normal(g, patch, d, hb[d]) : lerp_face(g, d, s, q, hb[d], hn[d][s])) * Afc;
                double add = rf * dc[d][s];
                if (pim) add *= af;
                pv += add;
                if (pim) pv += pfo[d][s];
                const bool own = owns_face(g, d, s, i, j, k);
                if (own) phiHbyA.a[d][fx[d][s]] = pv;
                double ph = (s ? 1.0 : -1.0) * af * pv;
                gg6[d][s] = 0.0;
                if (b) {
                    if (g.p_bc[patch] == 2) {
                        const double ubd = ub_normal(g, patch, d, g.u_bc[patch] == 1 ? U[3 * (size_t)c + d] : 0.0);
                        const double psn_v = (pv - ubd * Afc) / (rf * Afc);
                        if (own) psn.a[d][fx[d][s]] = psn_v;
                        ph = (s ? 1.0 : -1.0) * af * (pv - rf * geo_Af(g, d, i, j, k) * psn_v);
                    }
                    r -= ph;
                    if (g.p_bc[patch] == 1) { const double gb = kBfac * af * rf * geo_sfd(g, d, s, i, j, k); dg += gb; r += gb * g.p_val[patch]; }
                } else {
                    r -= ph;
                    const double gg = af * rf * geo_sfd(g, d, s, i, j, k);
                    dg += gg; gg6[d][s] = gg;
                    if (s) up[d] = gg;
                }
            }
        if (pim) r -= geo_V(g, i, j, k) * (ac - alphaOld[c]) / g.dt;
        if (refc) { r += dg * g.p_ref_value; dg += dg; }
        if (STORE_A) { A.diag[c] = dg; A.ux[c] = up[0]; A.uy[c] = up[1]; A.uz[c] = up[2]; }
        rhs[c] = r;
        double Ax = dg * xc, rs = dg;
#pragma unroll
        for (int d = 0; d < 3; ++d)
#pragma unroll
            for (int s = 0; s < 2; ++s)
                if (!bnd[d][s]) { Ax -= gg6[d][s] * xn[d][s]; rs -= gg6[d][s]; }
        const double Aref = rs * xbar;
        const double rr = r - Ax;
        res[c] = rr;
        v[0] += fabs(rr);
        v[1] += fabs(Ax - Aref) + fabs(r - Aref);
    }
    const int mx[2] = {0, 0};
    block_reduce_store<2>(v, mx, partials, fy_lb, fy_stride);
}

__device__ __forceinline__ double p_row(const PMat& A, const double* __restrict__ x, int c) {
    const int sy = A.nx, sz = A.nx * A.ny, last = A.ntot - 1;
    const int xm = max(c - 1, 0), xp = min(c + 1, last), ym = max(c - sy, 0), yp = min(c + sy, last), zm = max(c - sz, 0), zp = min(c + sz, last);
    const double uxc = A.ux[c], uyc = A.uy[c], uzc = A.uz[c];
    const double t0 = A.ux[xm] * x[xm], t1 = uxc * x[xp], t2 = A.uy[ym] * x[ym], t3 = uyc * x[yp], t4 = A.uz[zm] * x[zm], t5 = uzc * x[zp];
    double a = A.diag[c] * x[c];
    a = (c >= 1) ? a - t0 : a;
    a = (c + 1 < A.ntot) ? a - t1 : a;
    a = (c >= sy) ? a - t2 : a;
    a = (c + sy < A.ntot) ? a - t3 : a;
    a = (c >= sz) ? a - t4 : a;
    a = (c + sz < A.ntot) ? a - t5 : a;
    return a;
}
__device__ __forceinline__ double p_rowsum(const PMat& A, int c) {
    const int sy = A.nx, sz = A.nx * A.ny;
    double rs = A.diag[c];
    if (c >= 1) rs -= A.ux[c - 1];
    if (c + 1 < A.ntot) rs -= A.ux[c];
    if (c >= sy) rs -= A.uy[c - sy];
    if (c + sy < A.ntot) rs -= A.uy[c];
    if (c >= sz) rs -= A.uz[c - sz];
    if (c + sz < A.ntot) rs -= A.uz[c];
    return rs;
}

__global__ __launch_bounds__(256) void k_p_apply(PMat A, const double* __restrict__ x, double* __restrict__ y) {
    const int t = swz_block(blockIdx.x, gridDim.x) * 256 + threadIdx.x;
    if (t >= A.N) return;
    const int c = t + A.c0;
    y[c] = p_row(A, x, c);
}

template <bool WITH_R>
__global__ __launch_bounds__(256) void k_p_apply_dot(PMat A, const double* __restrict__ x, const double* __restrict__ r, double* __restrict__ y, double* __restrict__ partials) {
    double v[2] = {0, 0};
    FY_RED_LOOP(t, A.N) {
        const int c = t + A.c0;
        const double a = p_row(A, x, c);
        y[c] = a;
        const double xc = x[c];
        if (WITH_R) v[0] += xc * r[c];
        v[1] += a * xc;
    }
    if (WITH_R) {
        const int mx[2] = {0, 0};
        block_reduce_store<2>(v, mx, partials);
    } else {
        double v1[1] = {v[1]};
        const int mx[1] = {0};
        block_reduce_store<1>(v1, mx, partials + gridDim.x);
// ... 641 lines not shown
    }
    if (cached) for (int c = tid; c < T.cache_n; c += 1024) T.x1[0][c] = lx1[c];
}

__global__ __launch_bounds__(256) void k_mg_prolong_add(PMat A, double* __restrict__ x, PMat C, const double* __restrict__ xc) {
    const int t = blockIdx.x * 256 + threadIdx.x;
    if (t >= A.N) return;
    const int i = t % A.nx, q = t / A.nx, j = q % A.ny, k = q / A.ny;
    x[t + A.c0] += xc[C.c0 + (i >> 1) + C.nx * ((j >> 1) + C.ny * (k >> 1))];
}

__global__ __launch_bounds__(256) void k_mg_prolong_add_planes(PMat A, int kofs, double* __restrict__ x, PMat C, const double* __restrict__ xc) {
    const int t = blockIdx.x * 256 + threadIdx.x;
    if (t >= A.N) return;
    const int i = t % A.nx, q = t / A.nx, j = q % A.ny, k = q / A.ny + kofs;
    const int K = k >= 0 ? (k >> 1) : -((1 - k) >> 1);
    x[t + A.c0] += xc[C.c0 + (i >> 1) + C.nx * ((j >> 1) + C.ny * K)];
}

template <int Q>
__global__ __launch_bounds__(1024) void k_mg_coarse_factor(PMat A, int bw, double* __restrict__ fac) {
    extern __shared__ double B[];
    __shared__ int bad;
    const int N = A.N, tid = threadIdx.x, NT = (int)blockDim.x, Wd = bw + 1, sy = A.nx, sz = A.nx * A.ny;
    if (tid == 0) bad = 0;
    for (int e = tid; e < N * Wd; e += NT) B[e] = 0.0;
    __syncthreads();
    for (int c = tid; c < N; c += NT) {
        double* row = B + (size_t)c * Wd;
        row[0] += A.diag[c];
        if (c >= 1) row[1] -= A.ux[c - 1];
        if (A.ny > 1 && c >= sy && sy <= bw) row[sy] -= A.uy[c - sy];
        if (A.nz > 1 && c >= sz && sz <= bw) row[sz] -= A.uz[c - sz];
    }
    __syncthreads();
    int ua[Q], ub[Q];
#pragma unroll
    for (int q = 0; q < Q; ++q) {
        const int e = tid + NT * q;
        int a = (int)((sqrt(8.0 * (double)e + 1.0) - 1.0) * 0.5);
        while ((a + 1) * (a + 2) / 2 <= e) ++a;
        while (a * (a + 1) / 2 > e) --a;
        ua[q] = a; ub[q] = e - a * (a + 1) / 2;
    }
    for (int j = 0; j < N; ++j) {
        const double d = B[(size_t)j * Wd];
        if (!(d > 0.0) || !(d < 1e300)) { if (tid == 0) bad = 1; break; }
        const double id = 1.0 / d;
        const int m = min(bw, N - 1 - j);
#pragma unroll
        for (int q = 0; q < Q; ++q) {
            const int a = ua[q], b = ub[q];
            if (a < m) B[(size_t)(j + 1 + a) * Wd + (a - b)] -= (B[(size_t)(j + 1 + a) * Wd + 1 + a] * B[(size_t)(j + 1 + b) * Wd + 1 + b]) * id;
        }
        __syncthreads();
    }
    __syncthreads();
    if (!bad) {
        for (int i = tid; i < N; i += NT) fac[3 + (size_t)i * Wd] = 1.0 / sqrt(B[(size_t)i * Wd]);
        for (int e = tid; e < N * Wd; e += NT) {
            const int i = e / Wd, dd = e - i * Wd;
            if (dd >= 1) fac[3 + e] = dd <= i ? B[e] / sqrt(B[(size_t)(i - dd) * Wd]) : 0.0;
        }
    }
    if (tid == 0) { fac[0] = (double)N; fac[1] = (double)bw; fac[2] = bad ? 0.0 : 1.0; }
}

__global__ __launch_bounds__(1024) void k_mg_coarse_solve(PMat A, const double* __restrict__ b, double* __restrict__ x, double* __restrict__ tmp,
                                                          int sweeps, double w, const double* __restrict__ fac) {
    if (fac && A.N <= kMgDirectMax && fac[2] == 1.0) {
        extern __shared__ double fac_lds[];
        const int bw = (int)fac[1], cnt = A.N * (bw + 1);
        for (int q = threadIdx.x; q < cnt; q += 1024) fac_lds[q] = fac[3 + q];
        __syncthreads();
        if (threadIdx.x < 64) coarse_band_solve(fac_lds, A.N, bw, b, x, threadIdx.x);
        return;
    }
    const int c = threadIdx.x;
    const bool act = c < A.N;
    double* cur = x;
    double* nxt = tmp;
    if (act) cur[c] = w * b[c] / A.diag[c];
    __syncthreads();
    for (int s = 1; s < sweeps; ++s) {
        if (act) nxt[c] = cur[c] + w * (b[c] - p_row(A, cur, c)) / A.diag[c];
        __syncthreads();
        double* t = cur; cur = nxt; nxt = t;
    }
    if (cur != x) { if (act) x[c] = cur[c]; }
}

__global__ __launch_bounds__(256) void k_relax_field(double* __restrict__ x, const double* __restrict__ prev, double alpha, size_t n) {
    const size_t i = (size_t)blockIdx.x * 256 + threadIdx.x;
    if (i < n) x[i] = prev[i] + alpha * (x[i] - prev[i]);
}

__global__ __launch_bounds__(256) void k_copy(double* __restrict__ dst, const double* __restrict__ src, size_t n) {
    const size_t i = (size_t)blockIdx.x * 256 + threadIdx.x;
    if (i < n) dst[i] = src[i];
}

__global__ __launch_bounds__(256) void k_add(double* __restrict__ y, const double* __restrict__ x, size_t n) {
    const size_t i = (size_t)blockIdx.x * 256 + threadIdx.x;
    if (i < n) y[i] += x[i];
}

inline int fv_grid(const FvGeo& g) { return g.win_nblk > 0 ? g.win_nblk : div_up(g.Nc, 256); }
inline int fv_red_grid(const FvGeo& g) { return g.win_nblk > 0 ? g.win_nblk : red_blocks(g.Nc); }

#define FY_LAUNCH_CHECK()                                                                                     \
    do {                                                                                                      \
        hipError_t _e = hipGetLastError();                                                                    \
        if (_e != hipSuccess) return fail(FY_ERR_HIP, "kernel launch failed: %s (%s:%d)", hipGetErrorString(_e), __FILE__, __LINE__); \
    } while (0)

}

int launch_reduce_finalize(hipStream_t s, const double* partials, int n_cells, int nslots, const int* ops, double* out, unsigned long long* flag,
                           unsigned long long seq) {
    hipLaunchKernelGGL(k_reduce_finalize, dim3(nslots), dim3(1024), 0, s, partials, red_blocks(n_cells), ops, out, flag, seq);
    FY_LAUNCH_CHECK();
    return FY_OK;
}

int launch_flux_of(hipStream_t s, FvGeo g, const double* F, Face3 out) {
    hipLaunchKernelGGL(k_flux_of<0>, dim3(div_up(fv_fsize(g, 0), 256)), dim3(256), 0, s, g, F, out.a[0]);
    hipLaunchKernelGGL(k_flux_of<1>, dim3(div_up(fv_fsize(g, 1), 256)), dim3(256), 0, s, g, F, out.a[1]);
    hipLaunchKernelGGL(k_flux_of<2>, dim3(div_up(fv_fsize(g, 2), 256)), dim3(256), 0, s, g, F, out.a[2]);
    FY_LAUNCH_CHECK();
    return FY_OK;
}

int launch_courant(hipStream_t s, FvGeo g, CFace3 phi, double* partials) {
    hipLaunchKernelGGL(k_courant, dim3(fv_red_grid(g)), dim3(256), 0, s, g, phi, partials);
    FY_LAUNCH_CHECK();
    return FY_OK;
}

int launch_pre_coupling(hipStream_t s, FvGeo g, const double* U, const double* p, const double* alpha, CFace3 psn, double* vGrad,
                        double* gradP, double* divT, double* Gout, int write_vgrad, int write_pfields, CFace3 phi, double* ddtU, double* Uold_out,
                        double* cellrec, double rec_nu, double rec_rhoF, Face3 dcorr) {
    hipLaunchKernelGGL(k_pre_coupling, dim3(fv_grid(g)), dim3(256), 0, s, g, U, p, alpha, psn, vGrad, gradP, divT, Gout, write_vgrad, write_pfields,
                       phi, ddtU, Uold_out, cellrec, 2.0 * rec_nu, rec_rhoF, dcorr);
    FY_LAUNCH_CHECK();
    return FY_OK;
}

int launch_interp_alpha(hipStream_t s, FvGeo g, const double* alpha, Face3 af) {
    hipLaunchKernelGGL(k_interp_alpha_cells, dim3(fv_grid(g)), dim3(256), 0, s, g, alpha, af);
    FY_LAUNCH_CHECK();
    return FY_OK;
}

int launch_div_G(hipStream_t s, FvGeo g, const double* G, double* divG) {
    hipLaunchKernelGGL(k_div_G, dim3(fv_grid(g)), dim3(256), 0, s, g, G, divG);
    FY_LAUNCH_CHECK();
    return FY_OK;
}

int launch_assemble_turb(hipStream_t s, FvGeo g, TurbEqn e, const double* k, const double* eps, const double* alpha, CFace3 alphaf, CFace3 phi,
                         const double* vGrad, const double* U, Mom7 M, double* b3, double* x3) {
    hipLaunchKernelGGL(k_assemble_turb, dim3(fv_grid(g)), dim3(256), 0, s, g, e, k, eps, alpha, alphaf, phi, vGrad, U, M, b3, x3);
    FY_LAUNCH_CHECK();
    return FY_OK;
}

int launch_turb_finish(hipStream_t s, FvGeo g, TurbEqn e, const double* x3, double* X, int nut_mode, double cmu, const double* eps, double* nut) {
    hipLaunchKernelGGL(k_turb_finish, dim3(fv_grid(g)), dim3(256), 0, s, g, e, x3, X, nut_mode, cmu, eps, nut);
    FY_LAUNCH_CHECK();
    return FY_OK;
}

int launch_smagorinsky_nut(hipStream_t s, FvGeo g, const double* vGrad, double ck, double ce, double delta, double* nut) {
    hipLaunchKernelGGL(k_smagorinsky_nut, dim3(fv_grid(g)), dim3(256), 0, s, g, vGrad, ck, ce, delta, nut);
    FY_LAUNCH_CHECK();
    return FY_OK;
}

int launch_assemble_momentum(hipStream_t s, FvGeo g, const double* U, const double* Uold, const double* alpha, const double* alphaOld,
                             CFace3 alphaf, CFace3 phi, const double* uSource, const double* uSourceDrag, const double* divG, const double* vGrad,
                             Mom7 M, double* src, double* rAU) {
    if (g.upwind >= 3) hipLaunchKernelGGL(k_assemble_momentum<true>, dim3(fv_grid(g)), dim3(256), 0, s, g, U, Uold, alpha, alphaOld, alphaf, phi, uSource,
                                          uSourceDrag, divG, vGrad, M, src, rAU);
    else hipLaunchKernelGGL(k_assemble_momentum<false>, dim3(fv_grid(g)), dim3(256), 0, s, g, U, Uold, alpha, alphaOld, alphaf, phi, uSource,
                            uSourceDrag, divG, vGrad, M, src, rAU);
    FY_LAUNCH_CHECK();
    return FY_OK;
}
int launch_grad_magsqr(hipStream_t s, FvGeo g, const double* U, double* gradL) {
    hipLaunchKernelGGL(k_grad_magsqr, dim3(fv_grid(g)), dim3(256), 0, s, g, U, gradL);
    FY_LAUNCH_CHECK();
    return FY_OK;
}

int launch_interp_rAU(hipStream_t s, FvGeo g, const double* rAU, Face3 rf) {
    hipLaunchKernelGGL(k_interp_rAU<0>, dim3(div_up(fv_fsize(g, 0), 256)), dim3(256), 0, s, g, rAU, rf.a[0]);
    hipLaunchKernelGGL(k_interp_rAU<1>, dim3(div_up(fv_fsize(g, 1), 256)), dim3(256), 0, s, g, rAU, rf.a[1]);
    hipLaunchKernelGGL(k_interp_rAU<2>, dim3(div_up(fv_fsize(g, 2), 256)), dim3(256), 0, s, g, rAU, rf.a[2]);
    FY_LAUNCH_CHECK();
    return FY_OK;
}

int launch_bmom(hipStream_t s, FvGeo g, const double* src, const double* p, CFace3 psn, CFace3 phiForces, CFace3 rAUf, double* bmom) {
    hipLaunchKernelGGL(k_bmom, dim3(fv_grid(g)), dim3(256), 0, s, g, src, p, psn, phiForces, rAUf, bmom);
    FY_LAUNCH_CHECK();
    return FY_OK;
}

int launch_bmom_faces(hipStream_t s, FvGeo g, const double* rAU, const double* uSource, const double* src, const double* p, CFace3 psn, Face3 rAUf_out,
                      Face3 phiForces, double* bmom) {
    hipLaunchKernelGGL(k_bmom_faces, dim3(fv_grid(g)), dim3(256), 0, s, g, rAU, uSource, src, p, psn, rAUf_out, phiForces, bmom);
    FY_LAUNCH_CHECK();
    return FY_OK;
}

int launch_mom_pass(hipStream_t s, FvGeo g, Mom7 M, const double* b, const double* x, double* xn, const double* xsum, double n_glob, double* partials,
                    const double* hsrc, const double* rAU, double* HbyA) {
    if (HbyA) hipLaunchKernelGGL(k_mom_pass<true>, dim3(fv_red_grid(g)), dim3(256), 0, s, g, M, b, x, xn, xsum, n_glob, partials, hsrc, rAU, HbyA);
    else hipLaunchKernelGGL(k_mom_pass<false>, dim3(fv_red_grid(g)), dim3(256), 0, s, g, M, b, x, xn, xsum, n_glob, partials, hsrc, rAU, HbyA);
    FY_LAUNCH_CHECK();
    return FY_OK;
}

int launch_sum3(hipStream_t s, const double* x, int n, double* partials) {
    hipLaunchKernelGGL(k_sum3, dim3(red_blocks(n)), dim3(256), 0, s, x, n, partials);
    FY_LAUNCH_CHECK();
    return FY_OK;
}

int launch_HbyA(hipStream_t s, FvGeo g, Mom7 M, const double* src, const double* U, const double* rAU, double* HbyA) {
    hipLaunchKernelGGL(k_HbyA, dim3(fv_grid(g)), dim3(256), 0, s, g, M, src, U, rAU, HbyA);
    FY_LAUNCH_CHECK();
    return FY_OK;
}

int launch_phiHbyA(hipStream_t s, FvGeo g, const double* HbyA, const double* U, const double* Uold, CFace3 phiOld, CFace3 rAUf,
                   CFace3 alphaf, CFace3 phiForces, Face3 out, Face3 psn, Face3 ddtc, int keep) {
    if (keep == 1) hipLaunchKernelGGL(k_phiHbyA_cells<1>, dim3(fv_grid(g)), dim3(256), 0, s, g, HbyA, U, Uold, phiOld, rAUf, alphaf, phiForces, out, psn, ddtc);
    else if (keep == 2) hipLaunchKernelGGL(k_phiHbyA_cells<2>, dim3(fv_grid(g)), dim3(256), 0, s, g, HbyA, U, Uold, phiOld, rAUf, alphaf, phiForces, out, psn, ddtc);
    else hipLaunchKernelGGL(k_phiHbyA_cells<0>, dim3(fv_grid(g)), dim3(256), 0, s, g, HbyA, U, Uold, phiOld, rAUf, alphaf, phiForces, out, psn, ddtc);
    FY_LAUNCH_CHECK();
    return FY_OK;
}

int launch_adjust_phi_sums(hipStream_t s, FvGeo g, CFace3 phiHbyA, CFace3 phiForces, double* partials) {
    hipLaunchKernelGGL(k_adjust_phi_sums, dim3(fv_red_grid(g)), dim3(256), 0, s, g, phiHbyA, phiForces, partials);
    FY_LAUNCH_CHECK();
    return FY_OK;
}

int launch_adjust_phi_apply(hipStream_t s, FvGeo g, const double* sums, Face3 phiHbyA, CFace3 phiForces, CFace3 rAUf, const double* U, Face3 psn, int* err) {
    const size_t nbf = 2 * ((size_t)g.ny * g.nz + (size_t)g.nx * g.nz + (size_t)g.nx * g.ny);
    hipLaunchKernelGGL(k_adjust_phi_apply, dim3(div_up(nbf, 256)), dim3(256), 0, s, g, sums, phiHbyA, phiForces, rAUf, U, psn, err);
    FY_LAUNCH_CHECK();
    return FY_OK;
}

int launch_rAUf_phi_forces(hipStream_t s, FvGeo g, const double* rAU, const double* uSource, Face3 rf, Face3 out) {
    hipLaunchKernelGGL(k_rAUf_phi_forces_cells, dim3(fv_grid(g)), dim3(256), 0, s, g, rAU, uSource, rf, out);
    FY_LAUNCH_CHECK();
    return FY_OK;
}

int launch_assemble_pressure(hipStream_t s, FvGeo g, CFace3 phiHbyA, CFace3 rAUf, CFace3 alphaf, CFace3 psn, const double* alpha,
                             const double* alphaOld, PMat A, double* rhs, bool matrix) {
    if (matrix) hipLaunchKernelGGL(k_assemble_pressure<true>, dim3(fv_grid(g)), dim3(256), 0, s, g, phiHbyA, rAUf, alphaf, psn, alpha, alphaOld, A, rhs);
    else hipLaunchKernelGGL(k_assemble_pressure<false>, dim3(fv_grid(g)), dim3(256), 0, s, g, phiHbyA, rAUf, alphaf, psn, alpha, alphaOld, A, rhs);
    FY_LAUNCH_CHECK();
    return FY_OK;
}

int launch_flux_correct(hipStream_t s, FvGeo g, const double* p, CFace3 phiHbyA, CFace3 rAUf, CFace3 alphaf, CFace3 psn, CFace3 phiForces, Face3 pflux, Face3 phi) {
    hipLaunchKernelGGL(k_flux_correct_cells, dim3(fv_grid(g)), dim3(256), 0, s, g, p, phiHbyA, rAUf, alphaf, psn, phiForces, pflux, phi);
    FY_LAUNCH_CHECK();
    return FY_OK;
}

int launch_cont_err(hipStream_t s, FvGeo g, CFace3 phi, CFace3 alphaf, const double* alpha, const double* alphaOld, double* partials) {
    hipLaunchKernelGGL(k_cont_err, dim3(fv_red_grid(g)), dim3(256), 0, s, g, phi, alphaf, alpha, alphaOld, partials);
    FY_LAUNCH_CHECK();
    return FY_OK;
}

int launch_U_correct(hipStream_t s, FvGeo g, const double* HbyA, const double* rAU, const double* p, CFace3 psn, CFace3 phiForces,
                     CFace3 pflux, CFace3 alphaf, CFace3 rAUf, double* U) {
    hipLaunchKernelGGL(k_U_correct<false>, dim3(fv_red_grid(g)), dim3(256), 0, s, g, HbyA, rAU, p, psn, phiForces, pflux, alphaf, rAUf, U, CFace3{}, nullptr, nullptr, nullptr);
    FY_LAUNCH_CHECK();
    return FY_OK;
}

int launch_U_correct_diag(hipStream_t s, FvGeo g, const double* HbyA, const double* rAU, const double* p, CFace3 psn, CFace3 phiForces,
                          CFace3 pflux, CFace3 alphaf, CFace3 rAUf, double* U, CFace3 phi, const double* alpha, const double* alphaOld, double* partials) {
    hipLaunchKernelGGL(k_U_correct<true>, dim3(fv_red_grid(g)), dim3(256), 0, s, g, HbyA, rAU, p, psn, phiForces, pflux, alphaf, rAUf, U, phi, alpha, alphaOld, partials);
    FY_LAUNCH_CHECK();
    return FY_OK;
}

int launch_corr_back(hipStream_t s, FvGeo g, const double* p, CFace3 phiHbyA, CFace3 rAUf, CFace3 alphaf, CFace3 psn, CFace3 phiForces, Face3 phi,
                     const double* HbyA, const double* rAU, double* U, const double* alpha, const double* alphaOld, double* partials, bool faces_from_cells) {
    const FaceSrc rs{rAUf, faces_from_cells ? rAU : nullptr}, as{alphaf, faces_from_cells ? alpha : nullptr};
    const dim3 grid(fv_red_grid(g)), blk(256);
#define FY_BACK(DG, FC) hipLaunchKernelGGL((k_corr_back<DG, FC>), grid, blk, 0, s, g, p, phiHbyA, rs, as, psn, phiForces, phi, HbyA, rAU, U, alpha, alphaOld, partials)
    if (partials) { if (faces_from_cells) FY_BACK(true, true); else FY_BACK(true, false); }
    else { if (faces_from_cells) FY_BACK(false, true); else FY_BACK(false, false); }
#undef FY_BACK
    FY_LAUNCH_CHECK();
    return FY_OK;
}

int launch_corr_front(hipStream_t s, FvGeo g, const double* HbyA, const double* U, CFace3 dcorr, CFace3 rAUf, CFace3 alphaf, CFace3 phiForces, Face3 phiHbyA,
                      Face3 psn, const double* rAU, const double* alpha, const double* alphaOld, PMat A, double* rhs, bool store_A, const double* x,
                      const double* xsum_dev, double xsum_val, double inv_n, double* res, double* partials, bool faces_from_cells) {
    const FaceSrc rs{rAUf, faces_from_cells ? rAU : nullptr}, as{alphaf, faces_from_cells ? alpha : nullptr};
    const dim3 grid(fv_red_grid(g)), blk(256);
#define FY_FRONT(SA, FC) hipLaunchKernelGGL((k_corr_front<SA, FC>), grid, blk, 0, s, g, HbyA, U, dcorr, rs, as, phiForces, phiHbyA, psn, rAU, alpha, alphaOld, A, rhs, \
                                            x, xsum_dev, xsum_val, inv_n, res, partials)
    if (store_A) { if (faces_from_cells) FY_FRONT(true, true); else FY_FRONT(true, false); }
    else { if (faces_from_cells) FY_FRONT(false, true); else FY_FRONT(false, false); }
#undef FY_FRONT
    FY_LAUNCH_CHECK();
    return FY_OK;
}

static bool al16(const void* p) { return (reinterpret_cast<uintptr_t>(p) & 15u) == 0; }
static bool pairs_ok(const PMat& A) {
    return !pairs_disabled() && A.N >= 2 && A.nx % 2 == 0 && A.c0 % 2 == 0 && A.N % 2 == 0 && A.ntot % 2 == 0 && al16(A.diag) && al16(A.ux) && al16(A.uy) && al16(A.uz);
}
static bool pairs_ok(int n, int c0) {
    return !pairs_disabled() && n >= 2 && n % 2 == 0 && c0 % 2 == 0;
}

int launch_p_apply(hipStream_t s, PMat A, const double* x, double* y) {
    if (pairs_ok(A) && al16(x) && al16(y)) {
        hipLaunchKernelGGL(k_p_apply2, dim3(div_up(A.N, 512)), dim3(256), 0, s, A, x, y);
        FY_LAUNCH_CHECK();
        return FY_OK;
    }
    hipLaunchKernelGGL(k_p_apply, dim3(div_up(A.N, 256)), dim3(256), 0, s, A, x, y);
    FY_LAUNCH_CHECK();
    return FY_OK;
}

int launch_p_apply_dot(hipStream_t s, PMat A, const double* x, const double* r, double* y, double* partials) {
    if (pairs_ok(A) && al16(x) && al16(y) && al16(r)) {
        if (r) hipLaunchKernelGGL(k_p_apply_dot2<true>, dim3(red_blocks(A.N)), dim3(128), 0, s, A, x, r, y, partials);
        else hipLaunchKernelGGL(k_p_apply_dot2<false>, dim3(red_blocks(A.N)), dim3(128), 0, s, A, x, r, y, partials);
    }
    else if (r) hipLaunchKernelGGL(k_p_apply_dot<true>, dim3(red_blocks(A.N)), dim3(256), 0, s, A, x, r, y, partials);
    else hipLaunchKernelGGL(k_p_apply_dot<false>, dim3(red_blocks(A.N)), dim3(256), 0, s, A, x, r, y, partials);
    FY_LAUNCH_CHECK();
    return FY_OK;
}

int launch_p_init(hipStream_t s, PMat A, const double* b, const double* x, const double* xsum_dev, double xsum_val, double inv_n, double* r, double* partials) {
    hipLaunchKernelGGL(k_p_init, dim3(red_blocks(A.N)), dim3(256), 0, s, A, b, x, xsum_dev, xsum_val, inv_n, r, partials);
    FY_LAUNCH_CHECK();
    return FY_OK;
}

int launch_dot(hipStream_t s, int n, int c0, const double* a, const double* b, double* partials) {
    hipLaunchKernelGGL(k_dot, dim3(red_blocks(n)), dim3(256), 0, s, n, c0, a, b, partials);
    FY_LAUNCH_CHECK();
    return FY_OK;
}

int launch_pcg_cg_update(hipStream_t s, int n, int c0, const double* u, const double* w, double* p, double* sv, double* x, double* r, double* sc, int it, double* partials) {
    if (pairs_ok(n, c0) && al16(u) && al16(w) && al16(p) && al16(sv) && al16(x) && al16(r)) {
        if (it == 0) hipLaunchKernelGGL(k_pcg_cg_update2<true>, dim3(red_blocks(n)), dim3(128), 0, s, n, c0, u, w, p, sv, x, r, sc, it, partials);
        else hipLaunchKernelGGL(k_pcg_cg_update2<false>, dim3(red_blocks(n)), dim3(128), 0, s, n, c0, u, w, p, sv, x, r, sc, it, partials);
    }
    else if (it == 0) hipLaunchKernelGGL(k_pcg_cg_update<true>, dim3(red_blocks(n)), dim3(256), 0, s, n, c0, u, w, p, sv, x, r, sc, it, partials);
    else hipLaunchKernelGGL(k_pcg_cg_update<false>, dim3(red_blocks(n)), dim3(256), 0, s, n, c0, u, w, p, sv, x, r, sc, it, partials);
    FY_LAUNCH_CHECK();
    return FY_OK;
}

int launch_jacobi_precond(hipStream_t s, PMat A, const double* r, double* z) {
    hipLaunchKernelGGL(k_jacobi_precond, dim3(div_up(A.N, 256)), dim3(256), 0, s, A, r, z);
    FY_LAUNCH_CHECK();
    return FY_OK;
}

int launch_mg_ref_term(hipStream_t s, PMat A0, int ref_local, double* out) {
    hipLaunchKernelGGL(k_mg_ref_term, dim3(1), dim3(64), 0, s, A0, ref_local, out);
    FY_LAUNCH_CHECK();
    return FY_OK;
}

int launch_mg_coarsen(hipStream_t s, PMat F, PMat C, int ref_c, const double* ref_term) {
    hipLaunchKernelGGL(k_mg_coarsen, dim3(div_up(C.N, 256)), dim3(256), 0, s, F, C, ref_term ? ref_c : -1, ref_term);
    FY_LAUNCH_CHECK();
    return FY_OK;
}

int launch_mg_smooth_first(hipStream_t s, PMat A, const double* b, double* x, double w) {
    hipLaunchKernelGGL(k_mg_smooth_first, dim3(div_up(A.N, 256)), dim3(256), 0, s, A, b, x, w);
    FY_LAUNCH_CHECK();
    return FY_OK;
}

int launch_mg_smooth_two_from_zero(hipStream_t s, PMat A, const double* b, double* xn, double w, double w2) {
    if (pairs_ok(A) && al16(b) && al16(xn)) hipLaunchKernelGGL(k_mg_smooth_two_from_zero2, dim3(div_up(A.N, 512)), dim3(256), 0, s, A, b, xn, w, w2);
    else hipLaunchKernelGGL(k_mg_smooth_two_from_zero, dim3(div_up(A.N, 256)), dim3(256), 0, s, A, b, xn, w, w2);
    FY_LAUNCH_CHECK();
    return FY_OK;
}

int launch_mg_smooth_dot(hipStream_t s, PMat A, const double* b, const double* x, double* xn, double w, double* partials) {
    if (pairs_ok(A) && al16(b) && al16(x) && al16(xn)) hipLaunchKernelGGL(k_mg_smooth_dot2, dim3(red_blocks(A.N)), dim3(128), 0, s, A, b, x, xn, w, partials);
    else hipLaunchKernelGGL(k_mg_smooth_dot, dim3(red_blocks(A.N)), dim3(256), 0, s, A, b, x, xn, w, partials);
    FY_LAUNCH_CHECK();
    return FY_OK;
}

int launch_mg_smooth(hipStream_t s, PMat A, const double* b, const double* x, double* xn, double w) {
    if (pairs_ok(A) && al16(b) && al16(x) && al16(xn)) hipLaunchKernelGGL(k_mg_smooth2, dim3(div_up(A.N, 512)), dim3(256), 0, s, A, b, x, xn, w);
    else hipLaunchKernelGGL(k_mg_smooth, dim3(div_up(A.N, 256)), dim3(256), 0, s, A, b, x, xn, w);
    FY_LAUNCH_CHECK();
    return FY_OK;
}

static int band_width(const PMat& A) { return A.nz > 1 ? A.nx * A.ny : (A.ny > 1 ? A.nx : 1); }
static size_t fac_lds_bytes(int N, int bw) { return (size_t)N * (size_t)(bw + 1) * sizeof(double); }
static int allow_big_lds(const void* fn) {
    return hipFuncSetAttribute(fn, hipFuncAttributeMaxDynamicSharedMemorySize, (int)fac_lds_bytes(kMgDirectMax, kMgDirectBand)) == hipSuccess ? FY_OK
           : fail(FY_ERR_HIP, "hipFuncSetAttribute(MaxDynamicSharedMemorySize) failed");
}

int mg_coarse_factor_doubles(PMat A) { return 3 + A.N * (band_width(A) + 1); }
bool mg_coarse_direct_ok(PMat A) { return A.c0 == 0 && A.N <= kMgDirectMax && band_width(A) <= kMgDirectBand; }

int launch_mg_coarse_factor(hipStream_t s, PMat A, double* fac) {
    if (!(mg_coarse_direct_ok)(A)) return fail(FY_ERR_INVALID, "direct coarse solve: level of %d cells, band %d (ghost offset %d)", A.N, band_width(A), A.c0);
    static bool attr_set = false;
    if (!attr_set) {
        FY_TRY(allow_big_lds(reinterpret_cast<const void*>(k_mg_coarse_factor<1>)));
        FY_TRY(allow_big_lds(reinterpret_cast<const void*>(k_mg_coarse_factor<2>)));
        FY_TRY(allow_big_lds(reinterpret_cast<const void*>(k_mg_coarse_factor<3>)));
        attr_set = true;
    }
    const int bw = band_width(A);
    const int tri = bw * (bw + 1) / 2;
    const int q = tri <= 1024 ? 1 : (tri <= 2048 ? 2 : 3);
    const int nt = std::min(1024, ((tri + q - 1) / q + 63) / 64 * 64);
    if (q == 1) hipLaunchKernelGGL(k_mg_coarse_factor<1>, dim3(1), dim3(nt), fac_lds_bytes(A.N, bw), s, A, bw, fac);
    else if (q == 2) hipLaunchKernelGGL(k_mg_coarse_factor<2>, dim3(1), dim3(nt), fac_lds_bytes(A.N, bw), s, A, bw, fac);
    else hipLaunchKernelGGL(k_mg_coarse_factor<3>, dim3(1), dim3(nt), fac_lds_bytes(A.N, bw), s, A, bw, fac);
    FY_LAUNCH_CHECK();
    return FY_OK;
}

int launch_mg_tail(hipStream_t s, const PMat* A, double* const* x0, double* const* x1, double* const* b, int n, double w, int coarse_sweeps, MgWeights W,
                   const double* fac) {
    if (n < 1 || n > kMgTailMax) return fail(FY_ERR_INVALID, "bad multigrid tail depth %d", n);
    MgTail T;
// ... 119 lines not shown
```

### yade-openfoam-coupling_amd/csrc/fv_kernels_api.inc

```
int launch_reduce_finalize(hipStream_t s, const double* partials, int n_cells, int nslots, const int* ops , double* out,
                           unsigned long long* flag = nullptr, unsigned long long seq = 0);

int launch_flux_of(hipStream_t s, FvGeo g, const double* F, Face3 out);
int launch_courant(hipStream_t s, FvGeo g, CFace3 phi, double* partials);
int launch_pre_coupling(hipStream_t s, FvGeo g, const double* U, const double* p, const double* alpha, CFace3 psn,
                        double* vGrad, double* gradP, double* divT, double* Gout, int write_vgrad, int write_pfields,
                        CFace3 phi = CFace3{}, double* ddtU = nullptr, double* Uold_out = nullptr,
                        double* cellrec = nullptr ,
                        double rec_nu = 0.0, double rec_rhoF = 0.0,
                        Face3 dcorr = Face3{} );
int launch_interp_alpha(hipStream_t s, FvGeo g, const double* alpha, Face3 alphaf);
int launch_div_G(hipStream_t s, FvGeo g, const double* G, double* divG);
int launch_assemble_turb(hipStream_t s, FvGeo g, TurbEqn e, const double* k, const double* eps, const double* alpha, CFace3 alphaf, CFace3 phi,
                         const double* vGrad, const double* U, Mom7 M, double* b3, double* x3);
int launch_turb_finish(hipStream_t s, FvGeo g, TurbEqn e, const double* x3, double* X, int nut_mode, double cmu, const double* eps, double* nut);
int launch_smagorinsky_nut(hipStream_t s, FvGeo g, const double* vGrad, double ck, double ce, double delta, double* nut);
int launch_assemble_momentum(hipStream_t s, FvGeo g, const double* U, const double* Uold, const double* alpha, const double* alphaOld,
                             CFace3 alphaf, CFace3 phi, const double* uSource, const double* uSourceDrag, const double* divG,
                             const double* vGrad , Mom7 M, double* src, double* rAU);
int launch_grad_magsqr(hipStream_t s, FvGeo g, const double* U, double* gradL);
int launch_interp_rAU(hipStream_t s, FvGeo g, const double* rAU, Face3 rAUf);
int launch_adjust_phi_sums(hipStream_t s, FvGeo g, CFace3 phiHbyA, CFace3 phiForces, double* partials);
int launch_adjust_phi_apply(hipStream_t s, FvGeo g, const double* sums, Face3 phiHbyA, CFace3 phiForces, CFace3 rAUf, const double* U, Face3 psn, int* err);
int launch_rAUf_phi_forces(hipStream_t s, FvGeo g, const double* rAU, const double* uSource, Face3 rf, Face3 out);
int launch_bmom(hipStream_t s, FvGeo g, const double* src, const double* p, CFace3 psn, CFace3 phiForces, CFace3 rAUf, double* bmom);
int launch_bmom_faces(hipStream_t s, FvGeo g, const double* rAU, const double* uSource, const double* src, const double* p, CFace3 psn, Face3 rAUf_out,
                      Face3 phiForces, double* bmom);
int launch_mom_pass(hipStream_t s, FvGeo g, Mom7 M, const double* b, const double* x, double* xn, const double* xsum ,
                    double n_glob, double* partials, const double* hsrc = nullptr, const double* rAU = nullptr, double* HbyA = nullptr);
int launch_sum3(hipStream_t s, const double* x, int n, double* partials);
int launch_HbyA(hipStream_t s, FvGeo g, Mom7 M, const double* src, const double* U, const double* rAU, double* HbyA);
int launch_phiHbyA(hipStream_t s, FvGeo g, const double* HbyA, const double* U, const double* Uold, CFace3 phiOld, CFace3 rAUf,
                   CFace3 alphaf, CFace3 phiForces, Face3 phiHbyA, Face3 psn, Face3 ddtc = Face3{} ,
                   int keep = 0 );
int launch_assemble_pressure(hipStream_t s, FvGeo g, CFace3 phiHbyA, CFace3 rAUf, CFace3 alphaf, CFace3 psn, const double* alpha,
                             const double* alphaOld, PMat A, double* rhs, bool matrix = true );
int launch_flux_correct(hipStream_t s, FvGeo g, const double* p, CFace3 phiHbyA, CFace3 rAUf, CFace3 alphaf, CFace3 psn, CFace3 phiForces ,
                        Face3 pflux , Face3 phi);
int launch_cont_err(hipStream_t s, FvGeo g, CFace3 phi, CFace3 alphaf, const double* alpha, const double* alphaOld, double* partials);
int launch_U_correct(hipStream_t s, FvGeo g, const double* HbyA, const double* rAU, const double* p, CFace3 psn, CFace3 phiForces,
                     CFace3 pflux, CFace3 alphaf, CFace3 rAUf, double* U);
int launch_U_correct_diag(hipStream_t s, FvGeo g, const double* HbyA, const double* rAU, const double* p, CFace3 psn, CFace3 phiForces,
                          CFace3 pflux, CFace3 alphaf, CFace3 rAUf, double* U, CFace3 phi, const double* alpha, const double* alphaOld, double* partials);

int launch_corr_back(hipStream_t s, FvGeo g, const double* p, CFace3 phiHbyA, CFace3 rAUf, CFace3 alphaf, CFace3 psn, CFace3 phiForces, Face3 phi,
                     const double* HbyA, const double* rAU, double* U, const double* alpha, const double* alphaOld, double* partials, bool faces_from_cells);
int launch_corr_front(hipStream_t s, FvGeo g, const double* HbyA, const double* U, CFace3 dcorr, CFace3 rAUf, CFace3 alphaf, CFace3 phiForces, Face3 phiHbyA,
                      Face3 psn, const double* rAU, const double* alpha, const double* alphaOld, PMat A, double* rhs, bool store_A, const double* x,
                      const double* xsum_dev, double xsum_val, double inv_n, double* res, double* partials, bool faces_from_cells);

int launch_p_apply(hipStream_t s, PMat A, const double* x, double* y);
int launch_p_apply_dot(hipStream_t s, PMat A, const double* x, const double* r , double* y, double* partials);
int launch_p_init(hipStream_t s, PMat A, const double* b, const double* x, const double* xsum_dev , double xsum_val, double inv_n,
                  double* r, double* partials);
int launch_dot(hipStream_t s, int n, int c0, const double* a, const double* b , double* partials);
int launch_pcg_cg_update(hipStream_t s, int n, int c0, const double* u, const double* w, double* p, double* sv, double* x, double* r, double* sc, int it, double* partials);
int launch_jacobi_precond(hipStream_t s, PMat A, const double* r, double* z);
int launch_mg_coarsen(hipStream_t s, PMat F, PMat C, int ref_c = -1, const double* ref_term = nullptr);
int launch_mg_ref_term(hipStream_t s, PMat A0, int ref_local, double* out);
int launch_mg_smooth_first(hipStream_t s, PMat A, const double* b, double* x, double w);
int launch_mg_smooth_two_from_zero(hipStream_t s, PMat A, const double* b, double* xn, double w, double w2);
int launch_mg_smooth(hipStream_t s, PMat A, const double* b, const double* x, double* xn, double w);
int launch_mg_smooth_dot(hipStream_t s, PMat A, const double* b, const double* x, double* xn, double w, double* partials);
int launch_mg_residual_restrict(hipStream_t s, PMat A, const double* b, const double* x, PMat C, double* bc);
int launch_mg_prolong_add(hipStream_t s, PMat A, double* x, PMat C, const double* xc);
int launch_mg_prolong_add_planes(hipStream_t s, PMat A , int kofs , double* x, PMat C, const double* xc);
int launch_mg_smooth_prolong(hipStream_t s, PMat A, const double* b, const double* x, PMat C, const double* xc, double* xn, double w);
bool mg_coarse_direct_ok(PMat A);
int mg_coarse_factor_doubles(PMat A);
int launch_mg_coarse_factor(hipStream_t s, PMat A, double* fac);
int launch_mg_coarse_solve(hipStream_t s, PMat A, const double* b, double* x, double* tmp, int sweeps, double w, const double* fac = nullptr);
int launch_mg_tail(hipStream_t s, const PMat* A, double* const* x0, double* const* x1, double* const* b, int n, double w, int coarse_sweeps, MgWeights W,
                   const double* fac = nullptr);

int launch_copy_f64(hipStream_t s, double* dst, const double* src, size_t n);
int launch_relax_field(hipStream_t s, double* x, const double* prev, double alpha, size_t n);
int launch_p_ghost_uz(hipStream_t s, FvGeo g, CFace3 rAUf, CFace3 alphaf, PMat A);
int launch_mg_coarsen_ghost(hipStream_t s, PMat F, PMat C);
int launch_add_f64(hipStream_t s, double* y, const double* x, size_t n);
```

### yade-openfoam-coupling_amd/csrc/fv_solver.cpp

```cpp
#include "fv_solver.hpp"

namespace fy {

int Solver::create(const fy_case_desc* c, const fy_transport* tr, int dev, Comm* cm) {
    if (c && (c->convection_scheme < FY_CONVECTION_LINEAR || c->convection_scheme > FY_CONVECTION_QUICK)) return fail(FY_ERR_INVALID, "fy_solver_create: unknown convection_scheme");
    if (c && c->convection_scheme == FY_CONVECTION_LIMITED_LINEAR && !(c->convection_limiter_k >= 0 && c->convection_limiter_k <= 1)) return fail(FY_ERR_INVALID, "fy_solver_create: limitedLinear's coefficient must lie in [0, 1]");
    const bool gradedc = c && (c->hx || c->hy || c->hz);
    if (!c || c->nx <= 0 || c->ny <= 0 || c->nz <= 0 || (!gradedc && !(c->dx > 0)) || !(c->dt > 0)) return fail(FY_ERR_INVALID, "fy_solver_create: bad case");
    if (gradedc) {
        if (!(c->hx && c->hy && c->hz)) return fail(FY_ERR_INVALID, "fy_solver_create: a graded block needs hx, hy AND hz");
        if (cm && cm->size > 1) return fail(FY_ERR_UNSUPPORTED, "fy_solver_create: z-slabs need the uniform block (a graded block runs on one domain)");
        const double* hh[3] = {c->hx, c->hy, c->hz};
        const int nn[3] = {c->nx, c->ny, c->nz};
        for (int a = 0; a < 3; ++a) for (int q = 0; q < nn[a]; ++q) if (!(hh[a][q] > 0)) return fail(FY_ERR_INVALID, "fy_solver_create: graded block with a non-positive cell size");
    }
    int ndev = 0;
    if (hipGetDeviceCount(&ndev) != hipSuccess || ndev == 0) return fail(FY_ERR_NO_DEVICE, "no HIP device visible: libfoamyade_hip has no CPU path");
    if (dev < 0 || dev >= ndev) return fail(FY_ERR_INVALID, "device ordinal out of range");
    cs = *c; device = dev; pimple = c->solver == FY_SOLVER_PIMPLE;
    cs.hx = cs.hy = cs.hz = nullptr;
    comm = cm ? cm : &self_comm;
    FY_HIP(hipSetDevice(device));
    FY_HIP(hipStreamCreate(&stream));
    FY_HIP(hipStreamCreateWithFlags(&comm_stream, hipStreamNonBlocking));
    FY_HIP(hipEventCreateWithFlags(&ev_ready, hipEventDisableTiming));
    FY_HIP(hipEventCreateWithFlags(&ev_halo, hipEventDisableTiming));
    FY_HIP(hipEventCreateWithFlags(&ev_assembled, hipEventDisableTiming));
    FY_HIP(hipEventCreateWithFlags(&ev_usum0, hipEventDisableTiming));
    FY_HIP(hipEventCreateWithFlags(&ev_usum1, hipEventDisableTiming));
    FY_HIP(hipEventCreateWithFlags(&ev_coarse, hipEventDisableTiming));
    FY_HIP(hipEventCreateWithFlags(&ev_factor, hipEventDisableTiming));
    const Options opt = options();
    overlap_halos = opt.halo_overlap;
    fused_corrector = !opt.no_fused_corrector;
    faces_from_cells = !opt.faces_from_arrays;
    comm->set_aux_stream(comm_stream);
    const int S = comm->size;
    if (c->nz % S != 0) return fail(FY_ERR_INVALID, "nz (%d) must be divisible by the number of slabs (%d)", c->nz, S);
    const int nzl = c->nz / S;
    if (S > 1 && (nzl % 2 != 0 || nzl < 2)) return fail(FY_ERR_INVALID, "each slab needs an even number (>= 2) of z-planes, got %d", nzl);
    const int gz = S == 1 ? 0 : (pimple ? 5 : 1);
    if (S > 1 && nzl < gz) return fail(FY_ERR_INVALID, "slab thinner (%d planes) than the particle halo (%d)", nzl, gz);
    plane = (size_t)c->nx * c->ny;
    Nc = (int)(plane * nzl);
    nstore = plane * (size_t)(nzl + 2 * gz);
    Nglob = (int64_t)plane * c->nz;
    g.nx = c->nx; g.ny = c->ny; g.nz = nzl; g.Nc = Nc; g.gz = gz; g.c0 = (int)(plane * gz); g.kglob0 = comm->rank * nzl; g.nzglob = c->nz;
    g.dx = c->dx; g.Af = c->dx * c->dx; g.V = c->dx * c->dx * c->dx;
    g.graded = 0; g.h[0] = g.h[1] = g.h[2] = nullptr;
    total_volume = g.V * (double)Nglob;
    if (gradedc) {
        const double* hh[3] = {c->hx, c->hy, c->hz};
        const int nn[3] = {c->nx, c->ny, c->nz};
        double len[3] = {0, 0, 0};
        for (int a = 0; a < 3; ++a) {
            h_host[a].assign(hh[a], hh[a] + nn[a]);
            for (double v : h_host[a]) len[a] += v;
            FY_TRY(d_h[a].alloc_exact((size_t)nn[a]));
            FY_HIP(hipMemcpyAsync(d_h[a].p, hh[a], (size_t)nn[a] * sizeof(double), hipMemcpyHostToDevice, stream));
            g.h[a] = d_h[a].p;
        }
        FY_HIP(hipStreamSynchronize(stream));
        g.graded = 1;
        g.dx = std::cbrt((h_host[0][0] * h_host[1][0]) * h_host[2][0]);
        g.Af = g.dx * g.dx; g.V = g.dx * g.dx * g.dx;
        total_volume = (len[0] * len[1]) * len[2];
    }
    g.strip_B = g.strip_bp = g.strip_nzx = 0;
    {
        const int want = opt.strip_blocks;
        if (want != 0 && plane % 256 == 0 && nzl % 8 == 0) {
            const int bp = (int)(plane / 256);
            const int target = want > 0 ? want : std::max(1, (int)std::lround(8.0 * c->nx / 256.0));
            int best = 1;
            for (int d = 1; d <= bp; ++d) if (bp % d == 0 && std::abs(d - target) < std::abs(best - target)) best = d;
            g.strip_B = best; g.strip_bp = bp; g.strip_nzx = nzl / 8;
        }
    }
    g.upwind = c->convection_scheme;
    g.lim_twoByk = 2.0 / std::max(c->convection_limiter_k, 1e-15);
    g.rdx = 1.0 / g.dx; g.rhdx = 1.0 / (0.5 * g.dx); g.rV = 1.0 / g.V;
    g.pimple = pimple ? 1 : 0; g.dt = c->dt; g.nu = c->nu;
    bool need_ref = true;
    for (int q = 0; q < 6; ++q) {
        if (c->u_bc[q] != FY_BC_U_FIXED_VALUE && c->u_bc[q] != FY_BC_U_ZERO_GRADIENT && c->u_bc[q] != FY_BC_U_SLIP) return fail(FY_ERR_INVALID, "fy_solver_create: unknown velocity boundary type %d on side %d", c->u_bc[q], q);
        if (c->p_bc[q] != FY_BC_P_ZERO_GRADIENT && c->p_bc[q] != FY_BC_P_FIXED_VALUE && c->p_bc[q] != FY_BC_P_FIXED_FLUX) return fail(FY_ERR_INVALID, "fy_solver_create: unknown pressure boundary type %d on side %d", c->p_bc[q], q);
        g.u_bc[q] = c->u_bc[q]; g.p_bc[q] = c->p_bc[q]; g.p_val[q] = c->p_value[q];
        for (int a = 0; a < 3; ++a) g.u_val[q][a] = c->u_value[q][a];
        if (c->p_bc[q] == FY_BC_P_FIXED_VALUE) need_ref = false;
    }
    for (int a = 0; a < 3; ++a) g.g[a] = c->g[a];
    g.need_ref = need_ref ? 1 : 0; g.p_ref_cell = c->p_ref_cell; g.p_ref_value = c->p_ref_value;
    g.u_relax = c->u_relax;
    if (c->turbulence_model != FY_TURBULENCE_LAMINAR && c->turbulence_model != FY_TURBULENCE_SMAGORINSKY && c->turbulence_model != FY_TURBULENCE_KEQN && c->turbulence_model != FY_TURBULENCE_KEPSILON) return fail(FY_ERR_UNSUPPORTED, "fy_solver_create: unknown turbulence_model %d (DPMTurbulenceModels.C:67-77: laminar Stokes, RAS kEpsilon, LES Smagorinsky, LES kEqn)", c->turbulence_model);
    if (c->turbulence_model != FY_TURBULENCE_LAMINAR) {
        if (!pimple) return fail(FY_ERR_INVALID, "fy_solver_create: icoFoamYade has no turbulence model (icoFoamYade.C:79-85 is laplacian(nu, U))");
        if (!(c->les_ck > 0 && c->les_ce > 0 && c->les_delta_coeff > 0) || c->nut_initial < 0) return fail(FY_ERR_INVALID, "fy_solver_create: Smagorinsky needs Ck, Ce, deltaCoeff > 0 and nut >= 0");
        for (int q = 0; q < 6; ++q) {
            const bool has_k = c->turbulence_model == FY_TURBULENCE_KEQN || c->turbulence_model == FY_TURBULENCE_KEPSILON;
            if (c->nut_bc[q] != FY_BC_NUT_ZERO_GRADIENT && c->nut_bc[q] != FY_BC_NUT_FIXED_VALUE && !((c->nut_bc[q] == FY_BC_WALL_FUNCTION || c->nut_bc[q] == FY_BC_NUT_CALCULATED) && has_k))
                return fail(FY_ERR_INVALID, "fy_solver_create: unknown nut boundary type (nutkWallFunction / calculated need a model with a k equation)");
            g.nut_bc[q] = c->nut_bc[q]; g.nut_val[q] = c->nut_value[q];
        }
        les_delta = c->les_delta_coeff * std::pow(g.V, 1.0 / 3.0);
        {
            if (!(c->wf_kappa > 0 && c->wf_E > 0)) return fail(FY_ERR_INVALID, "fy_solver_create: wall-function constants kappa, E must be positive");
            g.wf_yPlusLam = wall_yplus_lam(c->wf_kappa, c->wf_E); g.wf_kappa = c->wf_kappa; g.wf_E = c->wf_E; g.wf_cmu25 = std::pow(c->ras_cmu, 0.25);
            g.nut_wall_live = 0;
            g.turb_model = c->turbulence_model; g.turb_ck = c->les_ck; g.turb_cmu = c->ras_cmu; g.turb_delta = les_delta; g.turb_dcoeff = c->les_delta_coeff;
            for (int q = 0; q < 6; ++q) {
                g.k_bc[q] = c->k_bc[q]; g.k_val[q] = c->k_value[q];
                g.eps_bc[q] = c->eps_bc[q] == FY_BC_NUT_FIXED_VALUE ? 1 : 0; g.eps_val[q] = c->eps_value[q];
            }
        }
        const bool keqn = c->turbulence_model == FY_TURBULENCE_KEQN, keps = c->turbulence_model == FY_TURBULENCE_KEPSILON;
        if (keqn || keps) {
            if (!(c->k_initial >= 0) || (keps && !(c->k_initial > 0)) || !(c->k_tol >= 0) || c->k_max_iter < 0 || c->k_relax > 1) return fail(FY_ERR_INVALID, "fy_solver_create: the k equation needs k >= 0 (> 0 for kEpsilon), a solver tolerance and a relaxation factor in (0, 1]");
            if (c->k_convection_scheme != FY_CONVECTION_LINEAR && c->k_convection_scheme != FY_CONVECTION_UPWIND) return fail(FY_ERR_UNSUPPORTED, "fy_solver_create: div(alphaPhic,k) must be Gauss linear or Gauss upwind");
            eq_k.mode = keqn ? 0 : 2;
            eq_k.ck = c->les_ck; eq_k.ce = c->les_ce; eq_k.delta = les_delta; eq_k.xmin = 1e-15;
            eq_k.c1 = c->ras_c1; eq_k.c2 = c->ras_c2; eq_k.c3 = c->ras_c3; eq_k.sigma = keqn ? 1.0 : c->ras_sigmak;
            eq_k.relax = c->k_relax; eq_k.upwind = c->k_convection_scheme == FY_CONVECTION_UPWIND ? 1 : 0;
            for (int q = 0; q < 6; ++q) {
                if (c->k_bc[q] != FY_BC_NUT_ZERO_GRADIENT && c->k_bc[q] != FY_BC_NUT_FIXED_VALUE) return fail(FY_ERR_INVALID, "fy_solver_create: unknown k boundary type");
                eq_k.bc[q] = c->k_bc[q]; eq_k.val[q] = c->k_value[q];
            }
        }
        if (keps) {
            if (!(c->eps_initial > 0) || !(c->eps_tol >= 0) || c->eps_max_iter < 0 || c->eps_relax > 1 || !(c->ras_cmu > 0 && c->ras_sigmak > 0 && c->ras_sigmaeps > 0))
                return fail(FY_ERR_INVALID, "fy_solver_create: kEpsilon needs epsilon > 0, Cmu / sigmak / sigmaEps > 0, a solver tolerance and a relaxation factor in (0, 1]");
            if (c->eps_convection_scheme != FY_CONVECTION_LINEAR && c->eps_convection_scheme != FY_CONVECTION_UPWIND) return fail(FY_ERR_UNSUPPORTED, "fy_solver_create: div(alphaPhic,epsilon) must be Gauss linear or Gauss upwind");
            eq_eps = eq_k;
            eq_eps.mode = 1; eq_eps.sigma = c->ras_sigmaeps; eq_eps.xmin = 1e-15;
            eq_eps.relax = c->eps_relax; eq_eps.upwind = c->eps_convection_scheme == FY_CONVECTION_UPWIND ? 1 : 0;
            for (int q = 0; q < 6; ++q) {
                if (c->eps_bc[q] != FY_BC_NUT_ZERO_GRADIENT && c->eps_bc[q] != FY_BC_NUT_FIXED_VALUE && c->eps_bc[q] != FY_BC_WALL_FUNCTION) return fail(FY_ERR_INVALID, "fy_solver_create: unknown epsilon boundary type");
                eq_eps.bc[q] = c->eps_bc[q] == FY_BC_WALL_FUNCTION ? 0 : c->eps_bc[q]; eq_eps.val[q] = c->eps_value[q];
                eq_eps.wall[q] = eq_k.wall[q] = c->eps_bc[q] == FY_BC_WALL_FUNCTION ? 1 : 0;
            }
            eq_eps.cmu75 = eq_k.cmu75 = std::pow(c->ras_cmu, 0.75); eq_eps.cmu25 = eq_k.cmu25 = std::pow(c->ras_cmu, 0.25); eq_eps.kappa = eq_k.kappa = c->wf_kappa;
        }
    }
    if (c->adjust_time_step && !(c->max_co > 0 && c->max_delta_t > 0)) return fail(FY_ERR_INVALID, "adjustTimeStep needs maxCo > 0 and maxDeltaT > 0");
    if (c->u_relax > 1 || c->u_relax_final > 1 || c->p_relax > 1 || c->p_relax_final > 1) return fail(FY_ERR_INVALID, "relaxation factors lie in (0, 1]");
    if (need_ref) {
        double net = 0.0, mag = 0.0;
        bool adjustable = false;
        const double area[3] = {(double)c->ny * c->nz, (double)c->nx * c->nz, (double)c->nx * c->ny};
        for (int q = 0; q < 6; ++q) {
            if (c->u_bc[q] == FY_BC_U_SLIP) continue;
            if (c->u_bc[q] != FY_BC_U_FIXED_VALUE) { adjustable = true; continue; }
            const double un = c->u_value[q][q / 2] * ((q & 1) ? 1.0 : -1.0) * area[q / 2];
            net += un; mag += std::fabs(un);
        }
        if (!adjustable && std::fabs(net) > 1e-8 * (mag + 1e-300))
            return fail(FY_ERR_UNSUPPORTED, "no patch fixes the pressure and the fixed-value velocity patches do not balance (net flux %g of %g): OpenFOAM's adjustPhi "
                                            "ends such a run with 'Continuity error cannot be removed by adjusting the outflow'", net, mag);
        adjust_phi = adjustable || mag > 0.0;
    }

    const size_t n = nstore;
    DevBuf<double>* v3[] = {&U, &Uold, &uSource, &uParticle, &gradP, &divT, &ddtU, &src, &HbyA, &bmom, &divG, &xscr};
    for (auto* b : v3) { FY_TRY(b->alloc_exact(3 * n)); FY_TRY(zero(*b)); }
    DevBuf<double>* v1[] = {&p, &alpha, &uSourceDrag, &mdiag, &rAU, &prhs, &pr, &pw, &pp, &ps, &pzj};
    for (auto* b : v1) { FY_TRY(b->alloc_exact(n)); FY_TRY(zero(*b)); }
    for (auto& b : man) { FY_TRY(b.alloc_exact(n)); FY_TRY(zero(b)); }
    for (int q = 0; q < 6; ++q) if (c->u_bc[q] == FY_BC_U_SLIP && !mbd.p) { FY_TRY(mbd.alloc_exact(3 * n)); FY_TRY(zero(mbd)); }
    FY_TRY(vGrad.alloc_exact(9 * n)); FY_TRY(zero(vGrad));
    if (c->convection_scheme >= FY_CONVECTION_LIMITED_LINEAR) { FY_TRY(gradL.alloc_exact(3 * n)); FY_TRY(zero(gradL)); }
    if (c->turbulence_model != FY_TURBULENCE_LAMINAR) { FY_TRY(nut.alloc_exact(n)); FY_TRY(launch_fill_f64(stream, nut.p, n, c->nut_initial)); g.nut = nut.p; }
    if (c->turbulence_model == FY_TURBULENCE_KEQN || c->turbulence_model == FY_TURBULENCE_KEPSILON) { FY_TRY(kturb.alloc_exact(n)); FY_TRY(launch_fill_f64(stream, kturb.p, n, c->k_initial)); g.kturb = kturb.p; }
    if (c->turbulence_model == FY_TURBULENCE_KEPSILON) { FY_TRY(epsturb.alloc_exact(n)); FY_TRY(launch_fill_f64(stream, epsturb.p, n, c->eps_initial)); g.epsturb = epsturb.p; }
    FY_TRY(Gt.alloc_exact(9 * n)); FY_TRY(zero(Gt));
    for (int d = 0; d < 3; ++d) {
        DevBuf<double>* fs[] = {&phi[d], &phiOld[d], &psn[d], &alphaf[d], &phiHbyA[d], &phiForces[d], &rAUf[d], &pflux[d], &ddtc[d], &dcorr[d]};
        for (auto* b : fs) { FY_TRY(b->alloc_exact(fv_fsize(g, d))); FY_TRY(zero(*b)); }
        FY_TRY(launch_fill_f64(stream, alphaf[d].p, alphaf[d].n, 1.0));
    }
    FY_TRY(launch_fill_f64(stream, alpha.p, n, 1.0));
    FY_TRY(launch_fill_f64(stream, rAU.p, n, 1.0));
    FY_TRY(partials.alloc_exact(8 * (size_t)red_blocks(Nc))); FY_TRY(red_out.alloc_exact(8)); FY_TRY(sc.alloc_exact(8)); FY_TRY(xbar3.alloc_exact(3));
    FY_TRY(zero(partials)); FY_TRY(zero(sc)); FY_TRY(zero(red_out));
    if (adjust_phi) { FY_TRY(adj_sums.alloc_exact(4)); FY_TRY(adj_err.alloc_exact(1)); FY_HIP(hipMemsetAsync(adj_err.p, 0, sizeof(int), stream)); }
    if (hipHostMalloc((void**)&red_host, (kDeferBase + kDeferMax) * sizeof(double), hipHostMallocMapped) == hipSuccess) {
        if (hipHostGetDevicePointer((void**)&red_host_dev, red_host, 0) != hipSuccess) { (void)hipHostFree(red_host); red_host = nullptr; }
    } else {
        red_host = nullptr;
    }
// ... 144 lines not shown
                }
                h[q] = red_host[q];
            }
            return FY_OK;
        }
        FY_TRY(launch_reduce_finalize(stream, partials.p, Nc, nslots, courant ? ops_courant.p : nullptr, red_host_dev));
        FY_HIP(hipStreamSynchronize(stream));
        for (int q = 0; q < nslots; ++q) h[q] = red_host[q];
        return FY_OK;
    }
    FY_TRY(launch_reduce_finalize(stream, partials.p, Nc, nslots, courant ? ops_courant.p : nullptr, red_out.p));
    FY_TRY(comm->allreduce_ops(stream, red_out.p, nslots, courant ? 1u : 0u));
    double* land = (red_host && nslots <= 8) ? red_host : h;
    FY_HIP(hipMemcpyAsync(land, red_out.p, nslots * sizeof(double), hipMemcpyDeviceToHost, stream));
    FY_HIP(hipStreamSynchronize(stream));
    if (land != h) for (int q = 0; q < nslots; ++q) h[q] = land[q];
    return FY_OK;
}
bool Solver::reduce_deferred(int nslots, bool courant, int* slot, int* rc, const int* ops) {
    *rc = FY_OK;
    if (!red_host || n_deferred + nslots > kDeferMax) return false;
    *slot = kDeferBase + n_deferred;
    n_deferred += nslots;
    if (comm->size == 1) {
        *rc = launch_reduce_finalize(stream, partials.p, Nc, nslots, ops ? ops : (courant ? ops_courant.p : nullptr), red_host_dev + *slot);
        return true;
    }
    *rc = launch_reduce_finalize(stream, partials.p, Nc, nslots, ops ? ops : (courant ? ops_courant.p : nullptr), red_out.p);
    if (*rc == FY_OK) {
        *rc = comm->allreduce_ops(stream, red_out.p, nslots, ops ? 4u : (courant ? 1u : 0u));
    }
    if (*rc == FY_OK && hipMemcpyAsync(red_host + *slot, red_out.p, nslots * sizeof(double), hipMemcpyDeviceToHost, stream) != hipSuccess)
        *rc = fail(FY_ERR_HIP, "deferred read-back failed");
    return true;
}
int Solver::reduce_to_device(double* dst) {
    FY_TRY(launch_reduce_finalize(stream, partials.p, Nc, 1, nullptr, dst));
    return comm->allreduce(stream, dst, 1, false);
}

int Solver::solve_vec3(DevBuf<double>& X, const double* rhs, double tol, double rel_tol, int max_iter, int* iters, bool momentum) {
    Comm::Tag tag(comm, momentum ? "momentum_solve" : "turbulence_solve");
    double h[6];
    if (momentum && usum_pending) {
        usum_pending = false;
        FY_HIP(hipStreamWaitEvent(stream, ev_usum1, 0));
    } else {
        FY_TRY(launch_sum3(stream, X.p + 3 * (size_t)g.c0, Nc, partials.p));
        FY_TRY(launch_reduce_finalize(stream, partials.p, Nc, 3, nullptr, xbar3.p));
        FY_TRY(comm->allreduce(stream, xbar3.p, 3, false));
    }
    double* xc = X.p; double* xn = xscr.p;
    double norm[3] = {1, 1, 1}, res0[3] = {0, 0, 0}, res[3];
    int it = 0;
    for (;;) {
        const bool need_x = !(it == 0 && &X == &U && U_ghosts_fresh);
        kc[KC_MOM_PASS].begin(stream);
        const bool with_h = momentum && fused_corrector && cs.n_correctors > 0 && it >= 1;
        FY_TRY(overlapped(XW_MOMENTUM, need_x, [&](hipStream_t on) { return halo(xc, 3, plane, g.nz, g.gz, 1, on); }, [&](const FvGeo& gw) {
            return FVK(launch_mom_pass, stream, gw, M7(momentum), rhs, xc, xn, xbar3.p, (double)Nglob, partials.p, with_h ? src.p : nullptr, with_h ? rAU.p : nullptr,
                       with_h ? HbyA.p : nullptr);
        }));
        if (momentum) hbya_ready = with_h;
        kc[KC_MOM_PASS].end(stream);
        FY_TRY(reduce_read(6, false, h));
        if (it == 0) for (int q = 0; q < 3; ++q) { norm[q] = h[3 + q] + 1e-20; res0[q] = h[q] / norm[q]; }
        bool conv = true;
        for (int q = 0; q < 3; ++q) {
            res[q] = h[q] / norm[q];
            if (!(res[q] < tol || (rel_tol > 0 && res[q] < rel_tol * res0[q]))) conv = false;
        }
        if (conv || it >= max_iter) break;
        std::swap(xc, xn);
        ++it;
    }
    if (xc != X.p) {
        std::swap(X.p, xscr.p);
        if (&X == &U && cpl) cpl->c.dU = U.p;
    }
    if (&X == &U) U_ghosts_fresh = true;
    *iters = it;
    return FY_OK;
}

int Solver::corrector(bool final_inner) {
    Comm::Tag tag(comm, "corrector");
    if (hbya_ready) hbya_ready = false;
    else FY_TRY(overlapped(XW_CORRECTOR, !U_ghosts_fresh, [&](hipStream_t on) { return halo_U(on); },
                           [&](const FvGeo& gw) { return FVK(launch_HbyA, stream, gw, M7(), src.p, U.p, rAU.p, HbyA.p); }));
    if (!pimple && rAU_new) { FY_TRY(halo_cells(rAU, 1, 1)); if (face_arrays) FY_TRY(FVK(launch_interp_rAU, stream, g, rAU.p, F3(rAUf))); }
    MgLev& L = *mg[0];
    const bool fused_front = fused_corrector && !adjust_phi;
    const bool fused_back = fused_corrector;
    const bool ffc = faces_from_cells;
    if (fused_front) {
        clk_pres.begin(stream);
        FY_TRY(prepare_p_init(false));
        FY_TRY(overlapped(XW_CORRECTOR, true, [&](hipStream_t on) {
            comm->group_begin();
            FY_TRY(halo_cells(HbyA, 3, 1, on));
            FY_TRY(halo_p(on));
            return comm->group_end(on);
        }, [&](const FvGeo& gw) {
            return FVK(launch_corr_front, stream, gw, HbyA.p, U.p, C3(dcorr), C3(rAUf), C3(alphaf), C3(phiForces), F3(phiHbyA), F3(psn), rAU.p, alpha.p,  alpha.p,
                       L.A, prhs.p, rAU_new, p.p, p_sum_valid ? nullptr : sc.p + 6, p_sum, 1.0 / (double)Nglob, pr.p, partials.p, ffc);
        }));
    } else {
        FY_TRY(halo_cells(HbyA, 3, 1));
        FY_TRY(FVK(launch_phiHbyA, stream, g, HbyA.p, U.p, Uold.p, C3(phiOld), C3(rAUf), C3(alphaf), C3(phiForces), F3(phiHbyA), F3(psn), F3(ddtc), rAU_new ? 1 : 2));
        if (adjust_phi) {
            FY_TRY(FVK(launch_adjust_phi_sums, stream, g, C3(phiHbyA), C3(phiForces), partials.p));
            FY_TRY(launch_reduce_finalize(stream, partials.p, Nc, 4, nullptr, adj_sums.p));
            FY_TRY(comm->allreduce(stream, adj_sums.p, 4, false));
            FY_TRY(FVK(launch_adjust_phi_apply, stream, g, adj_sums.p, F3(phiHbyA), C3(phiForces), C3(rAUf), U.p, F3(psn), adj_err.p));
        }
        clk_pres.begin(stream);
    }
    for (int no = 0; no <= cs.n_non_orth_correctors; ++no) {
        const bool front_done = fused_front && no == 0;
        if (!front_done) FY_TRY(FVK(launch_assemble_pressure, stream, g, C3(phiHbyA), C3(rAUf), C3(alphaf), C3(psn), alpha.p,  alpha.p, L.A, prhs.p, rAU_new));
        if (rAU_new && L.distributed && comm->has_down() && !mg_deep) FY_TRY(FVK(launch_p_ghost_uz, stream, g, C3(rAUf), C3(alphaf), L.A));
        if (rAU_new) {
            if (comm->size == 1 && cs.p_solver == FY_PSOLVER_PCG_MG && mg.size() > 1) {
                FY_HIP(hipEventRecord(ev_assembled, stream));
                FY_HIP(hipStreamWaitEvent(comm_stream, ev_assembled, 0));
                std::swap(stream, comm_stream);
                coarse_on_side = true; coarse_marked = false;
                const int rc = build_coarse_operators();
                coarse_on_side = false;
                std::swap(stream, comm_stream);
                FY_TRY(rc);
                if (coarse_marked) { FY_HIP(hipEventRecord(ev_factor, comm_stream)); factor_pending = true; }
                else FY_HIP(hipEventRecord(ev_coarse, comm_stream));
                coarse_pending = true;
            } else {
                FY_TRY(build_coarse_operators());
            }
        }
        rAU_new = false;
        FY_TRY(solve_pressure(final_inner && no == cs.n_non_orth_correctors, front_done));
        FY_TRY(wait_factor());
        if (no == cs.n_non_orth_correctors && !fused_back) {
            FY_TRY(halo_p());
            FY_TRY(FVK(launch_flux_correct, stream, g, p.p, C3(phiHbyA), C3(rAUf), C3(alphaf), C3(psn), C3(phiForces), F3(pflux), F3(phi)));
            phi_fresh = true;
            if (pimple && p_relax_now > 0 && p_relax_now < 1) { FY_TRY(launch_relax_field(stream, p.p, pPrev.p, p_relax_now, nstore)); p_sum_valid = false; p_ghosts_fresh = false; }
        }
    }
    clk_pres.end(stream);
    double h[2];
    int slot = 0, rc = FY_OK;
    const bool diag_fused = fuse_diag && red_host && n_deferred + 4 <= kDeferMax;
    if (fused_back) {
        FY_TRY(overlapped(XW_CORRECTOR, !p_ghosts_fresh, [&](hipStream_t on) { return halo_p(on); }, [&](const FvGeo& gw) {
            return FVK(launch_corr_back, stream, gw, p.p, C3(phiHbyA), C3(rAUf), C3(alphaf), C3(psn), C3(phiForces), F3(phi), HbyA.p, rAU.p, U.p, alpha.p,
                        alpha.p, diag_fused ? partials.p : nullptr, ffc);
        }));
        phi_fresh = true;
        U_ghosts_fresh = false;
        if (pimple && p_relax_now > 0 && p_relax_now < 1) { FY_TRY(launch_relax_field(stream, p.p, pPrev.p, p_relax_now, nstore)); p_sum_valid = false; p_ghosts_fresh = false; }
        if (diag_fused) {
            if (!reduce_deferred(4, false, &slot, &rc, ops_diag.p)) return fail(FY_ERR_INVALID, "no room for the deferred diagnostics");
            FY_TRY(rc);
            cont_slots.push_back(slot);
            carry_slot = slot + 2;
            return FY_OK;
        }
        carry_slot = -1;
        if (pimple && !face_arrays) FY_TRY(FVK(launch_interp_alpha, stream, g, alpha.p, F3(alphaf)));
        FY_TRY(FVK(launch_cont_err, stream, g, C3(phi), C3(alphaf), alpha.p,  alpha.p, partials.p));
        if (reduce_deferred(2, false, &slot, &rc)) { FY_TRY(rc); cont_slots.push_back(slot); }
        else { FY_TRY(reduce_read(2, false, h)); note_cont_err(h); }
        return FY_OK;
    }
    if (diag_fused) {
        FY_TRY(FVK(launch_U_correct_diag, stream, g, HbyA.p, rAU.p, p.p, C3(psn), C3(phiForces), C3(pflux), C3(alphaf), C3(rAUf), U.p, C3(phi), alpha.p,
                                      alpha.p, partials.p));
        U_ghosts_fresh = false;
        if (!reduce_deferred(4, false, &slot, &rc, ops_diag.p)) return fail(FY_ERR_INVALID, "no room for the deferred diagnostics");
        FY_TRY(rc);
        cont_slots.push_back(slot);
        carry_slot = slot + 2;
        return FY_OK;
    }
    carry_slot = -1;
    FY_TRY(FVK(launch_cont_err, stream, g, C3(phi), C3(alphaf), alpha.p,  alpha.p, partials.p));
    if (reduce_deferred(2, false, &slot, &rc)) { FY_TRY(rc); cont_slots.push_back(slot); }
    else { FY_TRY(reduce_read(2, false, h)); note_cont_err(h); }
    FY_TRY(FVK(launch_U_correct, stream, g, HbyA.p, rAU.p, p.p, C3(psn), C3(phiForces), C3(pflux), C3(alphaf), C3(rAUf), U.p));
    U_ghosts_fresh = false;
    return FY_OK;
}

int Solver::turbulence_correct() {
    Comm::Tag tag(comm, "turbulence");
    FY_TRY(halo_U());
    FY_TRY(FVK(launch_pre_coupling, stream, g, U.p, p.p, alpha.p, C3(psn), vGrad.p, gradP.p, divT.p, nullptr, 1, 0));
    if (cs.turbulence_model == FY_TURBULENCE_KEQN || cs.turbulence_model == FY_TURBULENCE_KEPSILON) {
        const bool keps = cs.turbulence_model == FY_TURBULENCE_KEPSILON;
        int it = 0;
        FY_TRY(halo_cells(kturb, 1, 1));
        if (keps) {
            FY_TRY(halo_cells(epsturb, 1, 1));
            FY_TRY(FVK(launch_assemble_turb, stream, g, eq_eps, kturb.p, epsturb.p, alpha.p, C3(alphaf), C3(phi), vGrad.p, U.p, M7(), bmom.p, HbyA.p));
            FY_TRY(solve_vec3(HbyA, bmom.p, cs.eps_tol, cs.eps_rel_tol, cs.eps_max_iter, &it));
            st_k_iters += it;
            FY_TRY(halo_cells(HbyA, 3, 1));
            FY_TRY(FVK(launch_turb_finish, stream, g, eq_eps, HbyA.p, epsturb.p, 0, 0.0, nullptr, nullptr));
        }
        FY_TRY(FVK(launch_assemble_turb, stream, g, eq_k, kturb.p, epsturb.p, alpha.p, C3(alphaf), C3(phi), vGrad.p, U.p, M7(), bmom.p, HbyA.p));
        FY_TRY(solve_vec3(HbyA, bmom.p, cs.k_tol, cs.k_rel_tol, cs.k_max_iter, &it));
        st_k_iters += it;
        FY_TRY(halo_cells(HbyA, 3, 1));
        FY_TRY(FVK(launch_turb_finish, stream, g, eq_k, HbyA.p, kturb.p, keps ? 2 : 1, cs.ras_cmu, epsturb.p, nut.p));
        FY_TRY(halo_cells(kturb, 1, 1));
        g.nut_wall_live = 1;
        return halo_cells(nut, 1, 1);
    }
    FY_TRY(FVK(launch_smagorinsky_nut, stream, g, vGrad.p, cs.les_ck, cs.les_ce, les_delta, nut.p));
    return halo_cells(nut, 1, 1);
}

int Solver::step() {
    Comm::Tag tag(comm, "step_start");
    FY_HIP(hipSetDevice(device));
    st = fy_step_stats{}; st.cont_err_cumulative = cumulative_cont_err;
    clk_mom.on = clk_pres.on = timing; clk_mom.per_collect = clk_pres.per_collect = 1024; clk_mom.reset(); clk_pres.reset();
    if (timing) tim[3].start(stream);
    if (sources_pending) { FY_TRY(cpl->c.set_source_zero()); sources_pending = false; }
    double h[2];
    const bool carried = carry_valid;
    carry_valid = false; carry_slot = -1;
    if (!carried) FY_TRY(FVK(launch_courant, stream, g, C3(phi), partials.p));
    n_deferred = 0; cont_slots.clear(); courant_slot = -1;
    if (carried) note_courant(carry_h);
    if (cs.adjust_time_step) {
        if (!carried) { FY_TRY(reduce_read(2, true, h)); note_courant(h); }
        const double maxDeltaTFact = cs.max_co / (st.courant_max + 1e-15);
        const double deltaTFact = std::min(std::min(maxDeltaTFact, 1.0 + 0.1 * maxDeltaTFact), 1.2);
        cs.dt = std::min(deltaTFact * cs.dt, cs.max_delta_t);
        g.dt = cs.dt;
    } else if (!carried) {
        int slot = 0, rc = FY_OK;
        if (reduce_deferred(2, true, &slot, &rc)) { FY_TRY(rc); courant_slot = slot; }
        else { FY_TRY(reduce_read(2, true, h)); note_courant(h); }
    }
    st.delta_t = cs.dt;
    if (cs.n_correctors > 0) {
        for (int d = 0; d < 3; ++d) { std::swap(phi[d].p, phiOld[d].p); std::swap(phi[d].n, phiOld[d].n); }
        phi_fresh = false;
    } else {
        for (int d = 0; d < 3; ++d) FY_TRY(launch_copy_f64(stream, phiOld[d].p, phi[d].p, phi[d].n));
    }
    const unsigned fm = cpl->c.force_models;
    const bool curl_models = (fm & (FY_FORCE_GAUSSIAN_TORQUE | FY_FORCE_SAFFMAN_MEI_LIFT)) != 0;
    const bool want_vgrad = !pimple || curl_models, want_ddtU = pimple && (fm & FY_FORCE_ADDED_MASS);
    double* rec_out = (pimple && comm->size == 1) ? cpl->c.d_cellrec.p : nullptr;
    const bool defer_sweep = comm->size == 1 && cpl->c.gaussian;
    auto sweep_on = [&](const FvGeo& gw) -> int {
        return FVK(launch_pre_coupling, stream, gw, U.p, p.p, alpha.p, C3(psn), vGrad.p, gradP.p, divT.p, nullptr, want_vgrad ? 1 : 0, 1, phi_now(),
                   want_ddtU ? ddtU.p : nullptr, Uold.p, rec_out, cpl->c.nu, cpl->c.rhoF,
                   (fused_corrector && !adjust_phi) ? F3(dcorr) : Face3{});
    };
    std::function<int()> pre_sweep = [&]() -> int { return sweep_on(g); };
    auto opening_exchange = [&](hipStream_t on) -> int {
        comm->group_begin();
        FY_TRY(halo_cells(U, 3, g.gz > 1 ? g.gz : 1, on));
        if (!p_ghosts_fresh) FY_TRY(halo_cells(p, 1, 1, on));
        FY_TRY(halo_cells(alpha, 1, 1, on));
        return comm->group_end(on);
    };
    if (defer_sweep) {
        FY_TRY(opening_exchange(stream));
        cpl->c.mid_hook = [](void* u) -> int { return (*static_cast<std::function<int()>*>(u))(); };
        cpl->c.mid_hook_user = &pre_sweep;
    } else {
        cpl->c.mid_hook = nullptr;
        FY_TRY(overlapped(XW_STEP, true, opening_exchange, sweep_on));
    }
    p_ghosts_fresh = true; U_ghosts_fresh = true;
    if (comm->size > 1 && g.gz > 0) {
        const size_t gh = 3 * plane * (size_t)g.gz;
        FY_TRY(launch_copy_f64(stream, Uold.p, U.p, gh));
        FY_TRY(launch_copy_f64(stream, Uold.p + 3 * plane * (size_t)(g.gz + g.nz), U.p + 3 * plane * (size_t)(g.gz + g.nz), gh));
    }
    cpl->c.cellrec_external = rec_out != nullptr;

    if (timing) tim[0].start(stream);
    comm->tag = "particle";
    if (g.gz > 1) {
        const bool side_ch = cpl->c.slab.aux != nullptr;
        hipStream_t on = side_ch ? comm_stream : stream;
        if (side_ch) {
            if (!ev_fields) FY_HIP(hipEventCreateWithFlags(&ev_fields, hipEventDisableTiming));
            FY_HIP(hipEventRecord(ev_ready, stream));
            FY_HIP(hipStreamWaitEvent(comm_stream, ev_ready, 0));
        }
        comm->group_begin();
        FY_TRY(halo_cells(gradP, 3, g.gz, on)); FY_TRY(halo_cells(divT, 3, g.gz, on));
        if (curl_models) FY_TRY(halo_cells(vGrad, 9, g.gz, on));
        if (want_ddtU) FY_TRY(halo_cells(ddtU, 3, g.gz, on));
        FY_TRY(comm->group_end(on));
        if (side_ch) { FY_HIP(hipEventRecord(ev_fields, comm_stream)); cpl->c.slab.fields_event = ev_fields; }
    }
    usum_pending = false;
    if (comm->size == 1 && cs.momentum_predictor) {
        if (!usum_partials.p) FY_TRY(usum_partials.alloc_exact(3 * (size_t)red_blocks(Nc)));
        FY_HIP(hipEventRecord(ev_usum0, stream));
        FY_HIP(hipStreamWaitEvent(comm_stream, ev_usum0, 0));
        FY_TRY(launch_sum3(comm_stream, U.p + 3 * (size_t)g.c0, Nc, usum_partials.p));
        FY_TRY(launch_reduce_finalize(comm_stream, usum_partials.p, Nc, 3, nullptr, xbar3.p));
        FY_HIP(hipEventRecord(ev_usum1, comm_stream));
        usum_pending = true;
    }
    {
        cpl->c.async_results = true;
        const int rc = cpl->c.set_particle_action(cs.dt);
        cpl->c.mid_hook = nullptr; cpl->c.mid_hook_user = nullptr;
        FY_TRY(rc);
    }
    if (timing) { tim[0].stop(stream); }
    comm->tag = "momentum";

    if (pimple && face_arrays) FY_TRY(FVK(launch_interp_alpha, stream, g, alpha.p, F3(alphaf)));
    const int nOuter = pimple ? std::max(cs.n_outer_correctors, 1) : 1;
    for (int outer = 0; outer < nOuter; ++outer) {
        const bool final_outer = outer == nOuter - 1;
        g.u_relax = (final_outer && cs.u_relax_final > 0) ? cs.u_relax_final : cs.u_relax;
        p_relax_now = (final_outer && cs.p_relax_final > 0) ? cs.p_relax_final : cs.p_relax;
        if (pimple && p_relax_now > 0 && p_relax_now < 1) {
            if (!pPrev.p) FY_TRY(pPrev.alloc_exact(nstore));
            FY_TRY(launch_copy_f64(stream, pPrev.p, p.p, nstore));
        }
        clk_mom.begin(stream);
        if (pimple) {
            if (outer > 0) FY_TRY(halo_U());
            FY_TRY(FVK(launch_pre_coupling, stream, g, U.p, p.p, alpha.p, C3(psn), vGrad.p, gradP.p, divT.p, Gt.p, g.upwind == 2 ? 1 : 0, 0));
            FY_TRY(overlapped(XW_MOMENTUM, true, [&](hipStream_t on) { return halo(Gt.p + 2 * 3 * nstore, 3, plane, g.nz, g.gz, 1, on); },
                              [&](const FvGeo& gw) { return FVK(launch_div_G, stream, gw, Gt.p, divG.p); }));
        }
        if (g.upwind == 2) FY_TRY(halo_cells(vGrad, 9, 1));
        if (g.upwind >= 3) {
            FY_TRY(halo_U());
            FY_TRY(FVK(launch_grad_magsqr, stream, g, U.p, gradL.p));
            FY_TRY(halo_cells(gradL, 3, 1));
        }
        FY_TRY(FVK(launch_assemble_momentum, stream, g, U.p, Uold.p, alpha.p,  alpha.p, face_arrays ? C3(alphaf) : CFace3{}, phi_now(), uSource.p, uSourceDrag.p,
                                        divG.p, g.upwind >= 3 ? gradL.p : vGrad.p, M7(), src.p, rAU.p));
        rAU_new = true; hbya_ready = false;
        const bool bmom_fused = pimple && cs.momentum_predictor && fused_corrector;
        if (pimple) {
            if (cpl->c.slab.tail_pending) { FY_HIP(hipStreamWaitEvent(stream, cpl->c.slab.ev_tail, 0)); cpl->c.slab.tail_pending = false; }
            if (bmom_fused) {
                FY_TRY(overlapped(XW_MOMENTUM, true, [&](hipStream_t on) { return halo_cells(rAU, 1, 1, on); }, [&](const FvGeo& gw) {
                    return FVK(launch_bmom_faces, stream, gw, rAU.p, uSource.p, src.p, p.p, C3(psn), face_arrays ? F3(rAUf) : Face3{}, F3(phiForces), bmom.p);
                }));
            } else {
                FY_TRY(halo_cells(rAU, 1, 1));
                FY_TRY(FVK(launch_rAUf_phi_forces, stream, g, rAU.p, uSource.p, F3(rAUf), F3(phiForces)));
            }
        }
        if (cs.momentum_predictor) {
            if (!bmom_fused) FY_TRY(FVK(launch_bmom, stream, g, src.p, p.p, C3(psn), C3(phiForces), C3(rAUf), bmom.p));
            int it = 0;
            FY_TRY(solve_momentum(&it));
            st.u_iters_total += it;
        }
        clk_mom.end(stream);
        for (int corr = 0; corr < cs.n_correctors; ++corr) FY_TRY(corrector(outer == nOuter - 1 && corr == cs.n_correctors - 1));
        if (g.nut && final_outer) FY_TRY(turbulence_correct());
    }
    FY_TRY(cpl->c.finish_results());
    avg.elapsed += cs.dt;
    if (avg.on()) FY_TRY(avg.sample(stream, cs.dt, [this](const std::string& nm, int* comp) { return avg_source(nm, comp); }));
    if (hold_sources) sources_pending = true;
    else FY_TRY(cpl->c.set_source_zero());
    if (timing) tim[3].stop(stream);
    FY_HIP(hipStreamSynchronize(stream));
    if (adjust_phi) {
        int e = 0;
        FY_HIP(hipMemcpy(&e, adj_err.p, sizeof(int), hipMemcpyDeviceToHost));
        if (e) return fail(FY_ERR_UNSUPPORTED, "adjustPhi: continuity error cannot be removed by adjusting the outflow (the in- and outflow through the "
                                               "fixed-value patches do not balance and no adjustable outflow is left) -- OpenFOAM stops here too");
    }
    if (courant_slot >= 0) note_courant(red_host + courant_slot);
    for (int sl : cont_slots) note_cont_err(red_host + sl);
    if (carry_slot >= 0) { carry_h[0] = red_host[carry_slot]; carry_h[1] = red_host[carry_slot + 1]; carry_valid = true; }
    if (timing) {
        clk_mom.collect(); clk_pres.collect();
        st.ms_momentum = clk_mom.total_ms; st.ms_pressure = clk_pres.total_ms;
        st.ms_particle = tim[0].ms() - cpl->c.marks.ms(6, 7);
        st.ms_total = tim[3].ms();
        st.ms_other = st.ms_total - st.ms_particle - st.ms_momentum - st.ms_pressure;
        for (auto& k : kc) k.collect();
        avg.clock.collect();
    }
    if (xwait_timing) {
        for (auto& k : clk_xwait) k.collect();
    }
    return FY_OK;
}

int Solver::field(const char* name, double** ptr, size_t* count) {
    const std::string s = name ? name : "";
    const size_t n = (size_t)Nc;
    struct E { const char* nm; double* p; size_t c; int comp; };
    const E tab[] = {{"U", U.p, 3 * n, 3}, {"p", p.p, n, 1}, {"phi_x", phi[0].p, phi[0].n, 0}, {"phi_y", phi[1].p, phi[1].n, 0}, {"phi_z", phi[2].p, phi[2].n, 0},
                     {"rAU", rAU.p, n, 1}, {"HbyA", HbyA.p, 3 * n, 3}, {"p_rhs", prhs.p, n, 1}, {"mom_diag", mdiag.p, n, 1}, {"mom_src", src.p, 3 * n, 3},
                     {"alpha", alpha.p, n, 1}, {"uSource", uSource.p, 3 * n, 3}, {"uSourceDrag", uSourceDrag.p, n, 1}, {"uParticle", uParticle.p, 3 * n, 3},
                     {"gradP", gradP.p, 3 * n, 3}, {"divT", divT.p, 3 * n, 3}, {"vGrad", vGrad.p, 9 * n, 9}, {"ddtU", ddtU.p, 3 * n, 3}, {"nut", nut.p, n, 1}, {"k", kturb.p, n, 1}, {"epsilon", epsturb.p, n, 1}};
    for (const E& e : tab) if (s == e.nm) {
        if (!e.p) return fail(FY_ERR_INVALID, "solver field '%s' does not exist in this case (no turbulence model)", s.c_str());
        const bool transport = cs.turbulence_model == FY_TURBULENCE_KEQN || cs.turbulence_model == FY_TURBULENCE_KEPSILON;
        if (transport && (s == "HbyA" || s == "mom_diag" || s == "mom_src"))
            return fail(FY_ERR_UNSUPPORTED, "solver field '%s' is overwritten by the turbulence transport solve in this case (kEqn / kEpsilon reuse the momentum matrix's storage)", s.c_str());
        *ptr = e.p + (size_t)e.comp * g.c0;
        *count = e.c;
        return FY_OK;
    }
    MgLev& L = *mg[0];
    const struct { const char* nm; double* p; } pm[] = {{"p_diag", L.diag.p}, {"p_ux", L.ux.p}, {"p_uy", L.uy.p}, {"p_uz", L.uz.p}};
    for (auto& e : pm) if (s == e.nm) { *ptr = e.p + L.A.c0; *count = n; return FY_OK; }
    if (s.size() > 2 && s.compare(0, 2, "mg") == 0 && s[2] >= '1' && s[2] <= '9') {
        size_t q = 2, lvl = 0;
        while (q < s.size() && s[q] >= '0' && s[q] <= '9' && lvl < 1000) lvl = 10 * lvl + (size_t)(s[q++] - '0');
        const std::string arr = s.substr(q);
        if (lvl < mg.size() && (arr == "_diag" || arr == "_ux" || arr == "_uy" || arr == "_uz")) {
            MgLev& M = *mg[lvl];
            double* base = arr == "_diag" ? M.diag.p : arr == "_ux" ? M.ux.p : arr == "_uy" ? M.uy.p : M.uz.p;
            *ptr = base + M.A.c0; *count = (size_t)M.A.N;
            return FY_OK;
        }
        return fail(FY_ERR_INVALID, "unknown solver field '%s' (the multigrid hierarchy has %zu levels)", s.c_str(), mg.size());
    }
    if (avg.lookup(s, ptr, count)) return FY_OK;
    return fail(FY_ERR_INVALID, "unknown solver field '%s'", s.c_str());
}

}
```

### yade-openfoam-coupling_amd/csrc/fv_solver.hpp

```cpp
#pragma once
#include <algorithm>
#include <cmath>
#include <memory>
#include <string>
#include <functional>
#include <vector>

#include "comm.hpp"
#include "coupling.hpp"
#include "field_average.hpp"
#include "fv_kernels.hpp"

#define FVK(fn, ...) (g.graded ? ::fy::gr::fn(__VA_ARGS__) : ::fy::fn(__VA_ARGS__))

namespace fy {

constexpr int kMgCoarsest = kMgDirectMax, kMgCoarsestEdge = 8;
constexpr int kMgDeepGhost = 5;
constexpr int kMgReplicateBelow = 1 << 20;

struct MgLev {
    PMat A{};
    bool distributed = false;
    int gz = 0;
    size_t plane = 0;
    DevBuf<double> diag, ux, uy, uz, x0, x1, b;
    double* xcur = nullptr;
    double* xalt = nullptr;
    const double* bptr = nullptr;
};

struct Solver {
    fy_case_desc cs{};
    std::vector<double> h_host[3];
    DevBuf<double> d_h[3];
    double total_volume = 0.0;
    FvGeo g{};
    int device = 0;
    hipStream_t stream = nullptr;
    hipStream_t comm_stream = nullptr;
    hipEvent_t ev_ready = nullptr, ev_halo = nullptr;
    hipEvent_t ev_fields = nullptr;
    hipEvent_t ev_assembled = nullptr, ev_coarse = nullptr, ev_factor = nullptr;
    hipEvent_t ev_usum0 = nullptr, ev_usum1 = nullptr;
    DevBuf<double> usum_partials;
    bool usum_pending = false;
    bool coarse_pending = false, factor_pending = false, coarse_on_side = false, coarse_marked = false;
    int wait_coarse() { if (coarse_pending) { coarse_pending = false; FY_HIP(hipStreamWaitEvent(stream, ev_coarse, 0)); } return FY_OK; }
    int wait_factor() { FY_TRY(wait_coarse()); if (factor_pending) { factor_pending = false; FY_HIP(hipStreamWaitEvent(stream, ev_factor, 0)); } return FY_OK; }
    fy_ctx* cpl = nullptr;
    bool pimple = false;
    int Nc = 0;
    size_t nstore = 0, plane = 0;
    int64_t Nglob = 0;
    Comm* comm = nullptr;
    SelfComm self_comm;

    DevBuf<double> U, Uold, p, alpha, uSource, uSourceDrag, uParticle, gradP, divT, vGrad, ddtU;
    DevBuf<double> nut;
    DevBuf<double> kturb, epsturb;
    TurbEqn eq_k{}, eq_eps{};
    double les_delta = 0.0;
    bool phi_fresh = true;
    CFace3 phi_now() const { return phi_fresh ? CFace3{{phi[0].p, phi[1].p, phi[2].p}} : CFace3{{phiOld[0].p, phiOld[1].p, phiOld[2].p}}; }
    bool rAU_new = true;
    DevBuf<double> phi[3], phiOld[3], psn[3], alphaf[3], phiHbyA[3], phiForces[3], rAUf[3], pflux[3], ddtc[3];
    DevBuf<double> dcorr[3];
    DevBuf<double> gradL;
    DevBuf<double> mbd;
    DevBuf<double> mdiag, man[6], src, rAU, HbyA, bmom, Gt, divG, xscr;
    std::vector<std::unique_ptr<MgLev> > mg;
    size_t mg_rep = 0;
    DevBuf<double> rep_stage;
    DevBuf<double> prhs, pr, pw, pp, ps, pzj;
    DevBuf<double> rep_gather;
    bool mg_deep = false;
    bool p_ghosts_fresh = false;
    bool U_ghosts_fresh = false;
    int halo_U(hipStream_t on = nullptr) { if (comm->size > 1 && !U_ghosts_fresh) { FY_TRY(halo_cells(U, 3, 1, on)); U_ghosts_fresh = true; } return FY_OK; }
    int halo_p(hipStream_t on = nullptr) { if (comm->size > 1 && !p_ghosts_fresh) { FY_TRY(halo_cells(p, 1, 1, on)); p_ghosts_fresh = true; } return FY_OK; }
    DevBuf<double> pPrev;
    double p_relax_now = 0.0;
    bool adjust_phi = false;
    DevBuf<double> adj_sums;
    DevBuf<int> adj_err;
    DevBuf<double> partials, red_out, sc, xbar3;
    bool hold_sources = false, sources_pending = false;
    bool overlap_halos = true;
    double* red_host = nullptr;
    double* red_host_dev = nullptr;
    unsigned long long* red_flag = nullptr;
    unsigned long long* red_flag_dev = nullptr;
    unsigned long long red_seq = 0;
    DevBuf<int> ops_courant, ops_diag;
    fy_step_stats st{};
    double cumulative_cont_err = 0.0;
    EventTimer tim[4];
    KernelClock clk_mom, clk_pres;
    bool timing = true;
    enum { KC_MG_SMOOTH0 = 0, KC_P_APPLY_DOT, KC_MOM_PASS, KC_COUNT };
    KernelClock kc[KC_COUNT];

    Face3 F3(DevBuf<double>* a) { Face3 f; for (int d = 0; d < 3; ++d) f.a[d] = a[d].p; return f; }
    CFace3 C3(DevBuf<double>* a) { CFace3 f; for (int d = 0; d < 3; ++d) f.a[d] = a[d].p; return f; }
    Mom7 M7(bool with_bd = true) { Mom7 m; m.diag = mdiag.p; for (int q = 0; q < 6; ++q) m.an[q] = man[q].p; m.bd = with_bd ? mbd.p : nullptr; return m; }

    ~Solver() {
        if (cpl) fy_destroy(cpl);
        for (auto& t : tim) t.destroy();
        for (auto& k : kc) k.destroy();
        for (auto& k : clk_xwait) k.destroy();
        clk_mom.destroy(); clk_pres.destroy();
        if (ev_ready) (void)hipEventDestroy(ev_ready);
        if (ev_halo) (void)hipEventDestroy(ev_halo);
        if (ev_fields) (void)hipEventDestroy(ev_fields);
        if (ev_assembled) (void)hipEventDestroy(ev_assembled);
        if (ev_usum0) (void)hipEventDestroy(ev_usum0);
        if (ev_usum1) (void)hipEventDestroy(ev_usum1);
        if (ev_coarse) (void)hipEventDestroy(ev_coarse);
        if (ev_factor) (void)hipEventDestroy(ev_factor);
        if (comm_stream) (void)hipStreamDestroy(comm_stream);
        if (red_host) (void)hipHostFree(red_host);
        if (red_flag) (void)hipHostFree(red_flag);
        if (stream) (void)hipStreamDestroy(stream);
    }

    int zero(DevBuf<double>& b) { if (b.n) FY_HIP(hipMemsetAsync(b.p, 0, b.n * sizeof(double), stream)); return FY_OK; }

    int halo(double* f, int ncomp, size_t pl, int nzl, int gzl, int w, hipStream_t on = nullptr) {
        if (comm->size == 1) return FY_OK;
        if (!on) on = stream;
        const size_t P = pl * (size_t)ncomp;
        double* own_lo = f + (size_t)gzl * P;
        double* own_hi = f + (size_t)(gzl + nzl - w) * P;
        double* gh_lo = f + (size_t)(gzl - w) * P;
        double* gh_hi = f + (size_t)(gzl + nzl) * P;
        return comm->neighbour_exchange(on, own_hi, gh_lo, own_lo, gh_hi, (size_t)w * P);
    }
    int halo_cells(DevBuf<double>& f, int ncomp, int w, hipStream_t on = nullptr) { return halo(f.p, ncomp, plane, g.nz, g.gz, w, on); }

    bool can_window() const { return comm->size > 1 && overlap_halos && plane % 256 == 0 && g.nz >= 3; }
    FvGeo window(int ka, int kb) const {
        FvGeo w = g;
        const int bp = (int)(plane / 256);
        w.red_stride = red_blocks(Nc);
        w.win_blk0 = ka * bp;
        w.win_nblk = (kb >= g.nz ? w.red_stride : kb * bp) - w.win_blk0;
        return w;
    }
    enum { XW_STEP = 0, XW_PARTICLE, XW_MOMENTUM, XW_CORRECTOR, XW_COUNT };
    KernelClock clk_xwait[XW_COUNT];
    bool xwait_timing = false;
    double xwait_ms[XW_COUNT] = {0, 0, 0, 0};
    template <class X, class L>
    int overlapped(int phase, bool needed, X&& xchg, L&& launch) {
        if (!needed || comm->size == 1) return launch(g);
        KernelClock& ck = clk_xwait[phase];
        if (!can_window()) {
            ck.begin(stream);
            FY_TRY(xchg(stream));
            ck.end(stream);
            return launch(g);
        }
        FY_HIP(hipEventRecord(ev_ready, stream));
        FY_TRY(launch(window(1, g.nz - 1)));
        FY_HIP(hipStreamWaitEvent(comm_stream, ev_ready, 0));
        FY_TRY(xchg(comm_stream));
        FY_HIP(hipEventRecord(ev_halo, comm_stream));
        ck.begin(stream);
        FY_HIP(hipStreamWaitEvent(stream, ev_halo, 0));
        ck.end(stream);
        FY_TRY(launch(window(0, 1)));
        return launch(window(g.nz - 1, g.nz));
    }
    int halo_level(MgLev& L, double* x) { return L.distributed ? halo(x, 1, L.plane, L.A.nz, L.gz, 1) : FY_OK; }

    int create(const fy_case_desc* c, const fy_transport* tr, int dev, Comm* cm);

    int reduce_read(int nslots, bool courant, double* h);
    static constexpr int kDeferBase = 8, kDeferMax = 2 + 4 * 255;
    int n_deferred = 0;
    bool reduce_deferred(int nslots, bool courant, int* slot, int* rc, const int* ops = nullptr);
    int reduce_to_device(double* dst);

    int solve_momentum(int* iters) { return solve_vec3(U, bmom.p, cs.u_tol, cs.u_rel_tol, cs.u_max_iter, iters, true); }
    int solve_vec3(DevBuf<double>& X, const double* rhs, double tol, double rel_tol, int max_iter, int* iters, bool momentum = false);

    int smooth(size_t l, MgLev& L, double w, bool with_dot = false);
    PMat slice_of(const MgLev& L, const MgLev& Cc) const;
    static constexpr double kMgWa = 1.7318685872766142, kMgWb = 0.5695012757370842;
    MgWeights mgw{2, {kMgWa, kMgWb, 0, 0}};
    int vcycle(size_t l);
    PMat planes_of(const MgLev& L, int ext, int* kofs = nullptr) const;
    int vcycle_deep(size_t l, int E);
    int exchange_operator_ghosts(MgLev& L);
    bool want_vcycle_dot = false, vcycle_dot_done = false;
    static constexpr int kMgCoarseSweeps = 120;
    int coarse_sweeps = kMgCoarseSweeps;
    bool fuse_prolong = true;
    int ref_cell_at(size_t lvl, const PMat& A, int k0) const;
    int build_coarse_operators();
    DevBuf<double> mg_inv, mg_ref;
    double p_sum = 0.0;
    bool p_sum_valid = false;
    int solve_pressure(bool final_iter, bool init_done = false);
    int precondition(const double* r_host, double* z_host);
    int prepare_p_init(bool with_halo = true);
    bool fused_corrector = true;
    bool hbya_ready = false;
    bool face_arrays = true;
    bool faces_from_cells = true;

    int corrector(bool final_inner);
    bool fuse_diag = true;
    int carry_slot = -1;
    bool carry_valid = false;
    double carry_h[2] = {0, 0};

    std::vector<int> cont_slots;
    int courant_slot = -1;
    void note_cont_err(const double* h) {
        const double tv = total_volume;
        st.cont_err_sum_local = cs.dt * h[0] / tv; st.cont_err_global = cs.dt * h[1] / tv;
        cumulative_cont_err += st.cont_err_global; st.cont_err_cumulative = cumulative_cont_err;
    }
    void note_courant(const double* h) { st.courant_max = 0.5 * h[0] * cs.dt; st.courant_mean = 0.5 * (h[1] / total_volume) * cs.dt; }
    int turbulence_correct();
    int st_k_iters = 0;

    int step();
    FieldAverage avg;
    const double* avg_source(const std::string& name, int* comp) const;
    int set_field_average(const fy_average_desc* d);
    int field(const char* name, double** ptr, size_t* count);
};

}

struct fy_solver { fy::Solver s; };
```

### yade-openfoam-coupling_amd/csrc/fv_solver_api.cpp

```cpp
#include "fv_solver.hpp"

extern "C" {

void fy_case_defaults(fy_case_desc* c, int solver) {
    if (!c) return;
    std::memset(c, 0, sizeof(*c));
    c->solver = solver;
    c->nx = c->ny = c->nz = 32; c->dx = 0.1 / 32; c->dt = 0.005; c->nu = 0.01; c->rho_fluid = 1000.0; c->rho_particle = 2650.0;
    for (int q = 0; q < 6; ++q) { c->u_bc[q] = FY_BC_U_FIXED_VALUE; c->p_bc[q] = FY_BC_P_ZERO_GRADIENT; }
    c->n_outer_correctors = 1; c->n_correctors = 2; c->n_non_orth_correctors = 0; c->momentum_predictor = 1;
    c->p_ref_cell = 0; c->p_ref_value = 0.0;
    c->p_solver = FY_PSOLVER_PCG_MG;
    c->p_tol = 1e-6; c->p_rel_tol = 0.05; c->p_final_tol = 1e-6; c->p_final_rel_tol = 0.0; c->p_max_iter = 1000;
    c->u_tol = 1e-5; c->u_rel_tol = 0.0; c->u_max_iter = 1000;
    c->adjust_time_step = 0; c->max_co = 1.0; c->max_delta_t = 1e300;
    c->u_relax = 1.0; c->u_relax_final = 0.0; c->p_relax = 0.0; c->p_relax_final = 0.0;
    c->convection_limiter_k = 1.0;
    c->k_tol = 1e-6; c->k_rel_tol = 0.0; c->k_max_iter = 1000; c->k_relax = 0.0; c->k_convection_scheme = FY_CONVECTION_UPWIND;
    c->eps_tol = 1e-6; c->eps_rel_tol = 0.0; c->eps_max_iter = 1000; c->eps_relax = 0.0; c->eps_convection_scheme = FY_CONVECTION_UPWIND;
    c->wf_kappa = 0.41; c->wf_E = 9.8;
    c->ras_cmu = 0.09; c->ras_c1 = 1.44; c->ras_c2 = 1.92; c->ras_c3 = 0.0; c->ras_sigmak = 1.0; c->ras_sigmaeps = 1.3;
    c->turbulence_model = FY_TURBULENCE_LAMINAR; c->les_ck = 0.094; c->les_ce = 1.048; c->les_delta_coeff = 1.0;
}

static int solver_create_impl(const fy_case_desc* c, const fy_transport* tr, int device_ordinal, fy::Comm* cm, fy_solver** out) {
    if (!out) return fy::fail(FY_ERR_INVALID, "null out");
    *out = nullptr;
    fy_solver* s = new (std::nothrow) fy_solver();
    if (!s) return fy::fail(FY_ERR_INVALID, "out of host memory");
    int rc = s->s.create(c, tr, device_ordinal, cm);
    if (rc != FY_OK) { delete s; return rc; }
    *out = s;
    return FY_OK;
}

int fy_solver_create(const fy_case_desc* c, const fy_transport* tr, int device_ordinal, fy_solver** out) {
    return solver_create_impl(c, tr, device_ordinal, nullptr, out);
}

int fy_solver_create_slab(const fy_case_desc* c, const fy_transport* tr, int device_ordinal, fy_comm* comm, fy_solver** out) {
    if (!comm || !comm->c) return fy::fail(FY_ERR_INVALID, "null communicator");
    return solver_create_impl(c, tr, device_ordinal, comm->c, out);
}

int fy_comm_create_local_group(int n, fy_comm** out) {
    if (n < 1 || !out) return fy::fail(FY_ERR_INVALID, "bad arguments");
    std::vector<fy::Comm*> cs((size_t)n);
    FY_TRY(fy::local_comm_group_create(n, cs.data()));
    for (int r = 0; r < n; ++r) { out[r] = new fy_comm(); out[r]->c = cs[(size_t)r]; }
    return FY_OK;
}
int fy_comm_create_host(int rank, int size, const fy_comm_callbacks* cb, fy_comm** out) {
    if (!out) return fy::fail(FY_ERR_INVALID, "null out");
    fy::Comm* c = nullptr;
    FY_TRY(fy::host_comm_create(rank, size, cb, &c));
    *out = new fy_comm(); (*out)->c = c;
    return FY_OK;
}
int fy_comm_create_ipc(int rank, int size, const fy_comm_callbacks* cb, int device, fy_comm** out) {
    if (!out) return fy::fail(FY_ERR_INVALID, "null out");
    fy::Comm* c = nullptr;
    FY_TRY(fy::ipc_comm_create(rank, size, cb, device, &c));
    *out = new fy_comm(); (*out)->c = c;
    return FY_OK;
}
int fy_rccl_unique_id(void* out128) { return fy::rccl_unique_id(out128); }
int fy_comm_create_rccl(int rank, int size, const void* id128, int device, fy_comm** out) {
    if (!out) return fy::fail(FY_ERR_INVALID, "null out");
    fy::Comm* c = nullptr;
    FY_TRY(fy::rccl_comm_create(rank, size, id128, device, &c));
    *out = new fy_comm(); (*out)->c = c;
    return FY_OK;
}
int fy_comm_destroy(fy_comm* c) { if (c) { delete c->c; delete c; } return FY_OK; }
int fy_comm_stats(fy_comm* c, uint64_t* out4) {
    if (!c || !c->c || !out4) return fy::fail(FY_ERR_INVALID, "fy_comm_stats: null argument");
    out4[0] = c->c->n_exchange; out4[1] = c->c->n_allreduce; out4[2] = c->c->n_allgather; out4[3] = c->c->exchange_bytes;
    return FY_OK;
}
int fy_comm_stats_by_tag(fy_comm* c, char* buf, size_t cap) {
    if (!c || !c->c || !buf || cap == 0) return fy::fail(FY_ERR_INVALID, "fy_comm_stats_by_tag: null argument");
    std::string out;
    for (const auto& kv : c->c->by_tag)
        out += (kv.first.empty() ? std::string("-") : kv.first) + " " + std::to_string(kv.second[0]) + " " + std::to_string(kv.second[1]) + " " + std::to_string(kv.second[2]) + "\n";
    if (out.size() + 1 > cap) return fy::fail(FY_ERR_INVALID, "fy_comm_stats_by_tag: buffer too small (%zu needed)", out.size() + 1);
    std::memcpy(buf, out.c_str(), out.size() + 1);
    return FY_OK;
}
int fy_comm_selftest(fy_comm* c, int device_ordinal) { if (!c || !c->c) return fy::fail(FY_ERR_INVALID, "null communicator"); return fy::comm_selftest(c->c, device_ordinal); }
int fy_comm_rank(fy_comm* c) { return c && c->c ? c->c->rank : -1; }
int fy_comm_size(fy_comm* c) { return c && c->c ? c->c->size : -1; }

#define FY_S(s) if (!(s)) return fy::fail(FY_ERR_INVALID, "null fy_solver")

fy_ctx* fy_solver_coupling(fy_solver* s) { return s ? s->s.cpl : nullptr; }
int fy_solver_step(fy_solver* s) { FY_S(s); return s->s.step(); }
int fy_solver_get_stats(fy_solver* s, fy_step_stats* out) { FY_S(s); if (!out) return fy::fail(FY_ERR_INVALID, "null out"); *out = s->s.st; return FY_OK; }
int fy_solver_local_cells(fy_solver* s) { return s ? s->s.Nc : -1; }

int fy_solver_hold_sources(fy_solver* s, int hold) {
    FY_S(s);
    s->s.hold_sources = hold != 0;
    if (!hold && s->s.sources_pending) { FY_HIP(hipSetDevice(s->s.device)); FY_TRY(s->s.cpl->c.set_source_zero()); s->s.sources_pending = false; }
    return FY_OK;
}

int fy_solver_field_count(fy_solver* s, const char* name, int64_t* count) {
    FY_S(s);
    if (!count) return fy::fail(FY_ERR_INVALID, "null count");
    double* p; size_t n;
    FY_TRY(s->s.field(name, &p, &n));
    *count = (int64_t)n;
    return FY_OK;
}

int fy_solver_read_field_host(fy_solver* s, const char* name, double* out) {
    FY_S(s);
    double* p; size_t n;
    FY_TRY(s->s.field(name, &p, &n));
    FY_HIP(hipSetDevice(s->s.device));
    if (name && std::strncmp(name, "mg", 2) == 0) FY_TRY(s->s.wait_coarse());
    FY_HIP(hipMemcpyAsync(out, p, n * sizeof(double), hipMemcpyDeviceToHost, s->s.stream));
    FY_HIP(hipStreamSynchronize(s->s.stream));
    return FY_OK;
}

int fy_solver_write_field_host(fy_solver* s, const char* name, const double* in) {
    FY_S(s);
    double* p; size_t n;
    FY_TRY(s->s.field(name, &p, &n));
    if (name && std::strncmp(name, "mg", 2) == 0) return fy::fail(FY_ERR_INVALID, "fy_solver_write_field_host: '%s' is read-only (rebuilt from the pressure matrix at every assembly)", name);
    FY_HIP(hipSetDevice(s->s.device));
    FY_HIP(hipMemcpyAsync(p, in, n * sizeof(double), hipMemcpyHostToDevice, s->s.stream));
    {
        double* ap; size_t an;
        if (s->s.avg.lookup(name ? name : "", &ap, &an)) {
            FY_HIP(hipStreamSynchronize(s->s.stream));
            return FY_OK;
        }
    }
    s->s.carry_valid = false;
    s->s.p_sum_valid = false; s->s.p_ghosts_fresh = false;
    if (std::string(name) == "U") {
        s->s.U_ghosts_fresh = false;
        FY_TRY(s->s.halo_U());
        FY_TRY(s->s.g.graded ? fy::gr::launch_flux_of(s->s.stream, s->s.g, s->s.U.p, s->s.F3(s->s.phi)) : fy::launch_flux_of(s->s.stream, s->s.g, s->s.U.p, s->s.F3(s->s.phi)));
    }
    if (std::string(name) == "nut") FY_TRY(s->s.halo_cells(s->s.nut, 1, 1));
    if (std::string(name) == "k") FY_TRY(s->s.halo_cells(s->s.kturb, 1, 1));
    if (std::string(name) == "epsilon") FY_TRY(s->s.halo_cells(s->s.epsturb, 1, 1));
    FY_HIP(hipStreamSynchronize(s->s.stream));
    return FY_OK;
}

int fy_solver_destroy(fy_solver* s) { delete s; return FY_OK; }

int fy_solver_set_field_average(fy_solver* s, const fy_average_desc* d) { FY_S(s); return s->s.set_field_average(d); }
int fy_solver_get_average_state(fy_solver* s, int item, int64_t* samples, double* time_averaged) { FY_S(s); return s->s.avg.get_state(item, samples, time_averaged); }
int fy_solver_set_average_state(fy_solver* s, int item, int64_t samples, double time_averaged) { FY_S(s); return s->s.avg.set_state(item, samples, time_averaged); }

int fy_solver_apply_p_matrix_host(fy_solver* s, const double* x, double* y) {
    FY_S(s);
    fy::Solver& S = s->s;
    FY_HIP(hipSetDevice(S.device));
    FY_HIP(hipMemcpyAsync(S.pp.p + S.g.c0, x, (size_t)S.Nc * sizeof(double), hipMemcpyHostToDevice, S.stream));
    FY_TRY(S.halo_cells(S.pp, 1, 1));
    FY_TRY(fy::launch_p_apply(S.stream, S.mg[0]->A, S.pp.p, S.pw.p));
    FY_HIP(hipMemcpyAsync(y, S.pw.p + S.g.c0, (size_t)S.Nc * sizeof(double), hipMemcpyDeviceToHost, S.stream));
    FY_HIP(hipStreamSynchronize(S.stream));
    return FY_OK;
}

int fy_solver_solve_p_host(fy_solver* s, const double* rhs, double* x, int* iterations) {
    FY_S(s);
    if (!rhs || !x) return fy::fail(FY_ERR_INVALID, "fy_solver_solve_p_host: null argument");
    fy::Solver& S = s->s;
    FY_HIP(hipSetDevice(S.device));
    FY_HIP(hipMemcpyAsync(S.prhs.p + S.g.c0, rhs, (size_t)S.Nc * sizeof(double), hipMemcpyHostToDevice, S.stream));
    FY_HIP(hipMemcpyAsync(S.p.p + S.g.c0, x, (size_t)S.Nc * sizeof(double), hipMemcpyHostToDevice, S.stream));
    S.p_sum_valid = false; S.p_ghosts_fresh = false;
    const int before = S.st.p_iters_total;
    FY_TRY(S.solve_pressure(true));
    FY_HIP(hipMemcpyAsync(x, S.p.p + S.g.c0, (size_t)S.Nc * sizeof(double), hipMemcpyDeviceToHost, S.stream));
    FY_HIP(hipStreamSynchronize(S.stream));
    if (iterations) *iterations = S.st.p_iters_total - before;
    return FY_OK;
}

int fy_solver_precondition_host(fy_solver* s, const double* r, double* z) {
    FY_S(s);
    if (!r || !z) return fy::fail(FY_ERR_INVALID, "fy_solver_precondition_host: null argument");
    FY_HIP(hipSetDevice(s->s.device));
    return s->s.precondition(r, z);
}

int fy_solver_mg_levels(fy_solver* s, int cap, int32_t* nx, int32_t* ny, int32_t* nz_owned, int32_t* distributed, int* n_levels) {
    FY_S(s);
    if (!n_levels) return fy::fail(FY_ERR_INVALID, "fy_solver_mg_levels: null n_levels");
    *n_levels = (int)s->s.mg.size();
    for (int l = 0; l < *n_levels && l < cap; ++l) {
        const fy::MgLev& L = *s->s.mg[(size_t)l];
        if (nx) nx[l] = L.A.nx;
        if (ny) ny[l] = L.A.ny;
        if (nz_owned) nz_owned[l] = L.A.nz;
        if (distributed) distributed[l] = L.distributed ? 1 : 0;
    }
    return FY_OK;
}

int fy_solver_time_p_apply(fy_solver* s, int reps, double* avg_ms) {
    FY_S(s);
    if (reps < 1 || !avg_ms) return fy::fail(FY_ERR_INVALID, "bad arguments");
    fy::Solver& S = s->s;
    fy::EventTimer t;
    FY_TRY(t.init());
    for (int i = 0; i < 3; ++i) FY_TRY(fy::launch_p_apply(S.stream, S.mg[0]->A, S.pp.p, S.pw.p));
    t.start(S.stream);
    for (int i = 0; i < reps; ++i) FY_TRY(fy::launch_p_apply(S.stream, S.mg[0]->A, S.pp.p, S.pw.p));
    t.stop(S.stream);
    *avg_ms = t.ms() / reps;
    t.destroy();
    return FY_OK;
}

int fy_solver_enable_kernel_timing(fy_solver* s, int on) {
    FY_S(s);
    for (auto& k : s->s.kc) { k.reset(); k.on = on != 0; }
    s->s.avg.clock.reset(); s->s.avg.clock.on = on != 0;
    return FY_OK;
}

int fy_solver_enable_exchange_timing(fy_solver* s, int on) {
    FY_S(s);
    s->s.xwait_timing = on != 0;
    for (auto& k : s->s.clk_xwait) { k.reset(); k.on = on != 0; k.per_collect = 4096; }
    return FY_OK;
}

int fy_solver_get_exchange_wait(fy_solver* s, double ms[4], int64_t waits[4]) {
    FY_S(s);
    if (!ms) return fy::fail(FY_ERR_INVALID, "fy_solver_get_exchange_wait: null argument");
    for (int q = 0; q < fy::Solver::XW_COUNT; ++q) { ms[q] = s->s.clk_xwait[q].total_ms; if (waits) waits[q] = s->s.clk_xwait[q].launches; }
    return FY_OK;
}

int fy_solver_get_kernel_timing(fy_solver* s, const char* kernel, double* total_ms, int64_t* launches) {
    FY_S(s);
    const std::string k = kernel ? kernel : "";
    if (k == "field_average" && total_ms && launches) { *total_ms = s->s.avg.clock.total_ms; *launches = s->s.avg.clock.launches; return FY_OK; }
    int idx = k == "mg_smooth_l0" ? fy::Solver::KC_MG_SMOOTH0 : k == "p_apply_dot" ? fy::Solver::KC_P_APPLY_DOT : k == "mom_pass" ? fy::Solver::KC_MOM_PASS : -1;
    if (idx < 0 || !total_ms || !launches) return fy::fail(FY_ERR_INVALID, "unknown kernel clock '%s'", k.c_str());
    *total_ms = s->s.kc[idx].total_ms; *launches = s->s.kc[idx].launches;
    return FY_OK;
}

}
```

Measured before the change: 203.2.

## Fold stress divergence into momentum assembly and carry U sums from corrector

The nut-weighted coefficient is moved out of the stored stress tensor and applied inside a new div_stress device routine. The momentum assembly kernel now computes the stress divergence inline, which removes the separate div_G launch and its divG round-trip. In PIMPLE runs the first-outer stress tensor is produced by the pre-coupling sweep instead of a separate launch. Separately, the final corrector back-substitution kernel accumulates per-block U component sums, so a later launch_sum3 pass can be skipped. The cost is extra neighbour loads and registers in the assembly kernel, plus more complex state tracking. Env flags can disable both paths.

```diff
diff --git a/yade-openfoam-coupling_amd/csrc/common.hpp b/yade-openfoam-coupling_amd/csrc/common.hpp
--- a/yade-openfoam-coupling_amd/csrc/common.hpp
+++ b/yade-openfoam-coupling_amd/csrc/common.hpp
@@ -31,6 +31,8 @@
     bool localcomm_stream;
     bool no_fused_corrector;
     bool faces_from_arrays;
+    bool stress_per_sweep;
+    bool no_carried_usum;
     bool no_pairs;
     bool no_tail_cache;
     int ipc_slot_kb;
diff --git a/yade-openfoam-coupling_amd/csrc/coupling.cpp b/yade-openfoam-coupling_amd/csrc/coupling.cpp
--- a/yade-openfoam-coupling_amd/csrc/coupling.cpp
+++ b/yade-openfoam-coupling_amd/csrc/coupling.cpp
@@ -45,6 +45,8 @@
     q.localcomm_stream = ls != nullptr && ls[0] == '1';
     q.no_fused_corrector = on("FOAMYADE_NO_FUSED_CORRECTOR");
     q.faces_from_arrays = on("FOAMYADE_FACES_FROM_ARRAYS");
+    q.stress_per_sweep = on("FOAMYADE_STRESS_PER_SWEEP");
+    q.no_carried_usum = on("FOAMYADE_NO_CARRIED_USUM");
     q.no_pairs = on("FOAMYADE_NO_PAIRS");
     q.no_tail_cache = on("FOAMYADE_NO_TAIL_CACHE");
     q.ipc_slot_kb = (int)num("FOAMYADE_IPC_SLOT_KB", 0);
diff --git a/yade-openfoam-coupling_amd/csrc/fv_kernels.hip b/yade-openfoam-coupling_amd/csrc/fv_kernels.hip
--- a/yade-openfoam-coupling_amd/csrc/fv_kernels.hip
+++ b/yade-openfoam-coupling_amd/csrc/fv_kernels.hip
@@ -602,51 +602,74 @@
     }
     if (Gout) {
         const double tr = T[0] + T[4] + T[8];
-        const double an = g.nut ? alpha[c] * (g.nu + g.nut[c]) : alpha[c] * g.nu;
         const size_t rs = g_row_stride(g);
         for (int a = 0; a < 3; ++a)
-            for (int b = 0; b < 3; ++b) Gout[(size_t)a * rs + 3 * (size_t)c + b] = an * (T[3 * b + a] - (a == b ? (2.0 / 3.0) * tr : 0.0));
-    }
-}
-
-__global__ __launch_bounds__(256) void k_div_G(FvGeo g, const double* __restrict__ G, double* __restrict__ divG) {
+            for (int b = 0; b < 3; ++b) Gout[(size_t)a * rs + 3 * (size_t)c + b] = T[3 * b + a] - (a == b ? (2.0 / 3.0) * tr : 0.0);
+    }
+}
+
+__device__ __forceinline__ double stress_coef(const FvGeo& g, const double* __restrict__ alpha, int c) {
+    return g.nut ? alpha[c] * (g.nu + g.nut[c]) : alpha[c] * g.nu;
+}
+__device__ __forceinline__ void div_stress(const FvGeo& g, const double* __restrict__ D, const double* __restrict__ alpha, int c, int i, int j, int k,
+                                           double (&acc)[3]) {
+    const int ijk[3] = {i, j, k};
+    const int lane = threadIdx.x & 63;
+    bool bnd[3][2];
+#pragma unroll
+    for (int d = 0; d < 3; ++d)
+#pragma unroll
+        for (int s = 0; s < 2; ++s) bnd[d][s] = onb(g, d, s, i, j, k);
+    double own[3][3], nbv[3][2][3], an[3][2];
+    const double a0 = stress_coef(g, alpha, c);
+#pragma unroll
+    for (int d = 0; d < 3; ++d) {
+        const double* Dd = D + (size_t)d * g_row_stride(g);
+#pragma unroll
+        for (int q = 0; q < 3; ++q) own[d][q] = Dd[3 * (size_t)c + q];
+        if (d == 0) continue;
+#pragma unroll
+        for (int s = 0; s < 2; ++s) {
+            const int nb = bnd[d][s] ? c : c + (s ? stride_of(g, d) : -stride_of(g, d));
+            an[d][s] = stress_coef(g, alpha, nb);
+#pragma unroll
+            for (int q = 0; q < 3; ++q) nbv[d][s][q] = Dd[3 * (size_t)nb + q];
+        }
+    }
+    const bool end_lo = lane == 0 && i > 0, end_hi = lane == 63 && i + 1 < g.nx;
+    double em[3] = {0, 0, 0}, ep[3] = {0, 0, 0}, eam = 0, eap = 0;
+    if (end_lo) { em[0] = D[3 * (size_t)(c - 1)]; em[1] = D[3 * (size_t)(c - 1) + 1]; em[2] = D[3 * (size_t)(c - 1) + 2]; eam = stress_coef(g, alpha, c - 1); }
+    if (end_hi) { ep[0] = D[3 * (size_t)(c + 1)]; ep[1] = D[3 * (size_t)(c + 1) + 1]; ep[2] = D[3 * (size_t)(c + 1) + 2]; eap = stress_coef(g, alpha, c + 1); }
+#pragma unroll
+    for (int d = 0; d < 3; ++d)
+#pragma unroll
+        for (int q = 0; q < 3; ++q) {
+            own[d][q] = a0 * own[d][q];
+            if (d > 0) { nbv[d][0][q] = an[d][0] * nbv[d][0][q]; nbv[d][1][q] = an[d][1] * nbv[d][1][q]; }
+        }
+#pragma unroll
+    for (int q = 0; q < 3; ++q) { nbv[0][0][q] = wave_prev(own[0][q]); nbv[0][1][q] = wave_next(own[0][q]); }
+    if (end_lo) { nbv[0][0][0] = eam * em[0]; nbv[0][0][1] = eam * em[1]; nbv[0][0][2] = eam * em[2]; }
+    if (end_hi) { nbv[0][1][0] = eap * ep[0]; nbv[0][1][1] = eap * ep[1]; nbv[0][1][2] = eap * ep[2]; }
+    acc[0] = acc[1] = acc[2] = 0.0;
+#pragma unroll
+    for (int d = 0; d < 3; ++d) {
+        double fv[2][3];
+#pragma unroll
+        for (int s = 0; s < 2; ++s)
+#pragma unroll
+            for (int q = 0; q < 3; ++q) fv[s][q] = bnd[d][s] ? own[d][q] : geo_lerp_side(g, d, s, ijk[d], own[d][q], nbv[d][s][q]);
+#pragma unroll
+        for (int q = 0; q < 3; ++q) acc[q] += (fv[1][q] - fv[0][q]) * geo_rh(g, d, ijk[d]);
+    }
+}
+__global__ __launch_bounds__(256) void k_div_G(FvGeo g, const double* __restrict__ D, const double* __restrict__ alpha, double* __restrict__ divG) {
     const int t = fv_block(g, blockIdx.x, gridDim.x) * 256 + (int)threadIdx.x;
     if (t >= g.Nc) return;
     int i, j, k; ijk_of(g, t, i, j, k);
     const int c = t + g.c0;
-    const int ijk[3] = {i, j, k};
-    const double g0[3] = {G[3 * (size_t)c], G[3 * (size_t)c + 1], G[3 * (size_t)c + 2]};
-    double gx[2][3];
-    x_neighbours3(G, c, i, g.nx, g0, gx[0], gx[1]);
-    bool bnd[3][2];
-    double own[3][3], nbv[3][2][3];
-#pragma unroll
-    for (int q = 0; q < 3; ++q) { own[0][q] = g0[q]; nbv[0][0][q] = gx[0][q]; nbv[0][1][q] = gx[1][q]; }
-#pragma unroll
-    for (int d = 0; d < 3; ++d)
-#pragma unroll
-        for (int s = 0; s < 2; ++s) bnd[d][s] = onb(g, d, s, i, j, k);
-#pragma unroll
-    for (int d = 1; d < 3; ++d) {
-        const double* Gd = G + (size_t)d * g_row_stride(g);
-#pragma unroll
-        for (int q = 0; q < 3; ++q) own[d][q] = Gd[3 * (size_t)c + q];
-#pragma unroll
-        for (int s = 0; s < 2; ++s) {
-            const int nb = bnd[d][s] ? c : c + (s ? stride_of(g, d) : -stride_of(g, d));
-#pragma unroll
-            for (int q = 0; q < 3; ++q) nbv[d][s][q] = Gd[3 * (size_t)nb + q];
-        }
-    }
-    double acc[3] = {0, 0, 0};
-#pragma unroll
-    for (int d = 0; d < 3; ++d) {
-        double fv[2][3];
-#pragma unroll
-        for (int s = 0; s < 2; ++s)
-            for (int q = 0; q < 3; ++q) fv[s][q] = bnd[d][s] ? own[d][q] : geo_lerp_side(g, d, s, ijk[d], own[d][q], nbv[d][s][q]);
-        for (int q = 0; q < 3; ++q) acc[q] += (fv[1][q] - fv[0][q]) * geo_rh(g, d, ijk[d]);
-    }
+    double acc[3];
+    div_stress(g, D, alpha, c, i, j, k, acc);
     for (int q = 0; q < 3; ++q) divG[3 * (size_t)c + q] = acc[q];
 }
 
@@ -903,12 +926,12 @@
     return lim * wl + (1.0 - lim) * (flux >= 0 ? 1.0 : 0.0);
 }
 
-template <bool LIMITED>
+template <bool LIMITED, bool FOLD>
 __global__ __launch_bounds__(256) void k_assemble_momentum(FvGeo g, const double* __restrict__ U, const double* __restrict__ Uold,
                                                            const double* __restrict__ alpha, const double* __restrict__ alphaOld, CFace3 alphaf,
                                                            CFace3 phi, const double* __restrict__ uSource, const double* __restrict__ uSourceDrag,
-                                                           const double* __restrict__ divG, const double* __restrict__ vGrad, Mom7 M,
-                                                           double* __restrict__ src, double* __restrict__ rAU) {
+                                                           const double* __restrict__ divG, const double* __restrict__ Dt, const double* __restrict__ vGrad,
+                                                           Mom7 M, double* __restrict__ src, double* __restrict__ rAU) {
     const int t = fv_block(g, blockIdx.x, gridDim.x) * 256 + (int)threadIdx.x;
     if (t >= g.Nc) return;
     int i, j, k; ijk_of(g, t, i, j, k);
@@ -983,7 +1006,9 @@
         const double S = (alpha[c] - alphaOld[c]) / dt + divAPhi / V;
         dg -= V * S;
         dg -= V * uSourceDrag[c];
-        for (int q = 0; q < 3; ++q) s3[q] += V * divG[3 * (size_t)c + q];
+        double dvG[3] = {0.0, 0.0, 0.0};
+        if (FOLD) div_stress(g, Dt, alpha, c, i, j, k, dvG);
+        for (int q = 0; q < 3; ++q) s3[q] += V * (FOLD ? dvG[q] : divG[3 * (size_t)c + q]);
         double so = 0.0;
         for (int q = 0; q < 6; ++q) so += fabs(an[q]);
         if (g.u_relax > 0) {
@@ -1313,12 +1338,13 @@
 __device__ __forceinline__ double ub_normal(const FvGeo& g, int patch, int d, double own_d) {
     return g.u_bc[patch] == 0 ? g.u_val[patch][d] : (g.u_bc[patch] == 2 ? 0.0 : own_d);
 }
-template <bool DIAG, bool FFC>
+template <bool DIAG, bool FFC, bool USUM>
 __global__ __launch_bounds__(256) void k_corr_back(FvGeo g, const double* __restrict__ p, CFace3 phiHbyA, FaceSrc rAUf, FaceSrc alphaf, CFace3 psn,
                                                    CFace3 phiForces, Face3 phi, const double* __restrict__ HbyA, const double* __restrict__ rAU,
                                                    double* __restrict__ U, const double* __restrict__ alpha, const double* __restrict__ alphaOld,
-                                                   double* __restrict__ partials) {
+                                                   double* __restrict__ partials, double* __restrict__ usum) {
     double v[4] = {0, 0, 0, 0};
+    double u3[3] = {0, 0, 0};
     FY_RED_LOOP_G(g, t) {
         int i, j, k; ijk_of(g, t, i, j, k);
         const int c = t + g.c0;
@@ -1399,6 +1425,7 @@
             }
         }
         for (int d = 0; d < 3; ++d) U[3 * (size_t)c + d] = out[d];
+        if (USUM) for (int d = 0; d < 3; ++d) u3[d] += out[d];
         if (DIAG) {
             double ce = dv * geo_rV(g, i, j, k);
             if (pim) ce += (ac - alphaOld[c]) / g.dt;
@@ -1411,6 +1438,11 @@
     if (DIAG) {
         const int mx[4] = {0, 0, 1, 0};
         block_reduce_store<4>(v, mx, partials, fy_lb, fy_stride);
+    }
+    if (USUM) {
+        const int mx3[3] = {0, 0, 0};
+        const int nblk = (int)gridDim.x;
+        block_reduce_store<3>(u3, mx3, usum, nblk % 8 ? fy_lb : (fy_lb % (nblk / 8)) * 8 + fy_lb / (nblk / 8), nblk);
     }
 }
 
@@ -2358,8 +2390,8 @@
     return FY_OK;
 }
 
-int launch_div_G(hipStream_t s, FvGeo g, const double* G, double* divG) {
-    hipLaunchKernelGGL(k_div_G, dim3(fv_grid(g)), dim3(256), 0, s, g, G, divG);
+int launch_div_G(hipStream_t s, FvGeo g, const double* D, const double* alpha, double* divG) {
+    hipLaunchKernelGGL(k_div_G, dim3(fv_grid(g)), dim3(256), 0, s, g, D, alpha, divG);
     FY_LAUNCH_CHECK();
     return FY_OK;
 }
@@ -2384,12 +2416,16 @@
 }
 
 int launch_assemble_momentum(hipStream_t s, FvGeo g, const double* U, const double* Uold, const double* alpha, const double* alphaOld,
-                             CFace3 alphaf, CFace3 phi, const double* uSource, const double* uSourceDrag, const double* divG, const double* vGrad,
-                             Mom7 M, double* src, double* rAU) {
-    if (g.upwind >= 3) hipLaunchKernelGGL(k_assemble_momentum<true>, dim3(fv_grid(g)), dim3(256), 0, s, g, U, Uold, alpha, alphaOld, alphaf, phi, uSource,
-                                          uSourceDrag, divG, vGrad, M, src, rAU);
-    else hipLaunchKernelGGL(k_assemble_momentum<false>, dim3(fv_grid(g)), dim3(256), 0, s, g, U, Uold, alpha, alphaOld, alphaf, phi, uSource,
-                            uSourceDrag, divG, vGrad, M, src, rAU);
+                             CFace3 alphaf, CFace3 phi, const double* uSource, const double* uSourceDrag, const double* divG, const double* Dt,
+                             const double* vGrad, Mom7 M, double* src, double* rAU) {
+    const dim3 grid(fv_grid(g)), blk(256);
+    const bool fold = Dt != nullptr && g.pimple;
+    if (fold && g.upwind >= 3) return fail(FY_ERR_INVALID, "launch_assemble_momentum: the limited convection schemes take the stress term from divG");
+#define FY_ASM(LIM, FOLD) hipLaunchKernelGGL((k_assemble_momentum<LIM, FOLD>), grid, blk, 0, s, g, U, Uold, alpha, alphaOld, alphaf, phi, uSource, uSourceDrag, \
+                                             divG, Dt, vGrad, M, src, rAU)
+    if (g.upwind >= 3) FY_ASM(true, false);
+    else { if (fold) FY_ASM(false, true); else FY_ASM(false, false); }
+#undef FY_ASM
     FY_LAUNCH_CHECK();
     return FY_OK;
 }
@@ -2503,10 +2539,13 @@
 }
 
 int launch_corr_back(hipStream_t s, FvGeo g, const double* p, CFace3 phiHbyA, CFace3 rAUf, CFace3 alphaf, CFace3 psn, CFace3 phiForces, Face3 phi,
-                     const double* HbyA, const double* rAU, double* U, const double* alpha, const double* alphaOld, double* partials, bool faces_from_cells) {
+                     const double* HbyA, const double* rAU, double* U, const double* alpha, const double* alphaOld, double* partials, bool faces_from_cells,
+                     double* usum) {
     const FaceSrc rs{rAUf, faces_from_cells ? rAU : nullptr}, as{alphaf, faces_from_cells ? alpha : nullptr};
     const dim3 grid(fv_red_grid(g)), blk(256);
-#define FY_BACK(DG, FC) hipLaunchKernelGGL((k_corr_back<DG, FC>), grid, blk, 0, s, g, p, phiHbyA, rs, as, psn, phiForces, phi, HbyA, rAU, U, alpha, alphaOld, partials)
+    if (usum && g.win_nblk > 0) return fail(FY_ERR_INVALID, "launch_corr_back: U's component sums need the whole-domain launch");
+#define FY_BACK(DG, FC) do { if (usum) hipLaunchKernelGGL((k_corr_back<DG, FC, true>), grid, blk, 0, s, g, p, phiHbyA, rs, as, psn, phiForces, phi, HbyA, rAU, U, alpha, alphaOld, partials, usum); \
+                             else hipLaunchKernelGGL((k_corr_back<DG, FC, false>), grid, blk, 0, s, g, p, phiHbyA, rs, as, psn, phiForces, phi, HbyA, rAU, U, alpha, alphaOld, partials, usum); } while (0)
     if (partials) { if (faces_from_cells) FY_BACK(true, true); else FY_BACK(true, false); }
     else { if (faces_from_cells) FY_BACK(false, true); else FY_BACK(false, false); }
 #undef FY_BACK
diff --git a/yade-openfoam-coupling_amd/csrc/fv_kernels_api.inc b/yade-openfoam-coupling_amd/csrc/fv_kernels_api.inc
--- a/yade-openfoam-coupling_amd/csrc/fv_kernels_api.inc
+++ b/yade-openfoam-coupling_amd/csrc/fv_kernels_api.inc
@@ -10,13 +10,13 @@
                         double rec_nu = 0.0, double rec_rhoF = 0.0,
                         Face3 dcorr = Face3{} );
 int launch_interp_alpha(hipStream_t s, FvGeo g, const double* alpha, Face3 alphaf);
-int launch_div_G(hipStream_t s, FvGeo g, const double* G, double* divG);
+int launch_div_G(hipStream_t s, FvGeo g, const double* D, const double* alpha, double* divG);
 int launch_assemble_turb(hipStream_t s, FvGeo g, TurbEqn e, const double* k, const double* eps, const double* alpha, CFace3 alphaf, CFace3 phi,
                          const double* vGrad, const double* U, Mom7 M, double* b3, double* x3);
 int launch_turb_finish(hipStream_t s, FvGeo g, TurbEqn e, const double* x3, double* X, int nut_mode, double cmu, const double* eps, double* nut);
 int launch_smagorinsky_nut(hipStream_t s, FvGeo g, const double* vGrad, double ck, double ce, double delta, double* nut);
 int launch_assemble_momentum(hipStream_t s, FvGeo g, const double* U, const double* Uold, const double* alpha, const double* alphaOld,
-                             CFace3 alphaf, CFace3 phi, const double* uSource, const double* uSourceDrag, const double* divG,
+                             CFace3 alphaf, CFace3 phi, const double* uSource, const double* uSourceDrag, const double* divG, const double* Dt,
                              const double* vGrad , Mom7 M, double* src, double* rAU);
 int launch_grad_magsqr(hipStream_t s, FvGeo g, const double* U, double* gradL);
 int launch_interp_rAU(hipStream_t s, FvGeo g, const double* rAU, Face3 rAUf);
@@ -44,7 +44,8 @@
                           CFace3 pflux, CFace3 alphaf, CFace3 rAUf, double* U, CFace3 phi, const double* alpha, const double* alphaOld, double* partials);
 
 int launch_corr_back(hipStream_t s, FvGeo g, const double* p, CFace3 phiHbyA, CFace3 rAUf, CFace3 alphaf, CFace3 psn, CFace3 phiForces, Face3 phi,
-                     const double* HbyA, const double* rAU, double* U, const double* alpha, const double* alphaOld, double* partials, bool faces_from_cells);
+                     const double* HbyA, const double* rAU, double* U, const double* alpha, const double* alphaOld, double* partials, bool faces_from_cells,
+                     double* usum = nullptr);
 int launch_corr_front(hipStream_t s, FvGeo g, const double* HbyA, const double* U, CFace3 dcorr, CFace3 rAUf, CFace3 alphaf, CFace3 phiForces, Face3 phiHbyA,
                       Face3 psn, const double* rAU, const double* alpha, const double* alphaOld, PMat A, double* rhs, bool store_A, const double* x,
                       const double* xsum_dev, double xsum_val, double inv_n, double* res, double* partials, bool faces_from_cells);
diff --git a/yade-openfoam-coupling_amd/csrc/fv_solver.cpp b/yade-openfoam-coupling_amd/csrc/fv_solver.cpp
--- a/yade-openfoam-coupling_amd/csrc/fv_solver.cpp
+++ b/yade-openfoam-coupling_amd/csrc/fv_solver.cpp
@@ -34,6 +34,8 @@
     overlap_halos = opt.halo_overlap;
     fused_corrector = !opt.no_fused_corrector;
     faces_from_cells = !opt.faces_from_arrays;
+    stress_once = !opt.stress_per_sweep;
+    carry_usum = !opt.no_carried_usum;
     comm->set_aux_stream(comm_stream);
     const int S = comm->size;
     if (c->nz % S != 0) return fail(FY_ERR_INVALID, "nz (%d) must be divisible by the number of slabs (%d)", c->nz, S);
@@ -484,10 +486,13 @@
     int slot = 0, rc = FY_OK;
     const bool diag_fused = fuse_diag && red_host && n_deferred + 4 <= kDeferMax;
     if (fused_back) {
+        const bool with_usum = final_inner && carry_usum && comm->size == 1 && cs.momentum_predictor;
+        if (with_usum && !usum_partials.p) FY_TRY(usum_partials.alloc_exact(3 * (size_t)red_blocks(Nc)));
         FY_TRY(overlapped(XW_CORRECTOR, !p_ghosts_fresh, [&](hipStream_t on) { return halo_p(on); }, [&](const FvGeo& gw) {
             return FVK(launch_corr_back, stream, gw, p.p, C3(phiHbyA), C3(rAUf), C3(alphaf), C3(psn), C3(phiForces), F3(phi), HbyA.p, rAU.p, U.p, alpha.p,
-                        alpha.p, diag_fused ? partials.p : nullptr, ffc);
+                        alpha.p, diag_fused ? partials.p : nullptr, ffc, with_usum ? usum_partials.p : nullptr);
         }));
+        usum_valid = with_usum;
         phi_fresh = true;
         U_ghosts_fresh = false;
         if (pimple && p_relax_now > 0 && p_relax_now < 1) { FY_TRY(launch_relax_field(stream, p.p, pPrev.p, p_relax_now, nstore)); p_sum_valid = false; p_ghosts_fresh = false; }
@@ -589,8 +594,9 @@
     const bool want_vgrad = !pimple || curl_models, want_ddtU = pimple && (fm & FY_FORCE_ADDED_MASS);
     double* rec_out = (pimple && comm->size == 1) ? cpl->c.d_cellrec.p : nullptr;
     const bool defer_sweep = comm->size == 1 && cpl->c.gaussian;
+    const bool D_at_start = pimple && stress_once && g.upwind != 2;
     auto sweep_on = [&](const FvGeo& gw) -> int {
-        return FVK(launch_pre_coupling, stream, gw, U.p, p.p, alpha.p, C3(psn), vGrad.p, gradP.p, divT.p, nullptr, want_vgrad ? 1 : 0, 1, phi_now(),
+        return FVK(launch_pre_coupling, stream, gw, U.p, p.p, alpha.p, C3(psn), vGrad.p, gradP.p, divT.p, D_at_start ? Gt.p : nullptr, want_vgrad ? 1 : 0, 1, phi_now(),
                    want_ddtU ? ddtU.p : nullptr, Uold.p, rec_out, cpl->c.nu, cpl->c.rhoF,
                    (fused_corrector && !adjust_phi) ? F3(dcorr) : Face3{});
     };
@@ -640,7 +646,8 @@
         if (!usum_partials.p) FY_TRY(usum_partials.alloc_exact(3 * (size_t)red_blocks(Nc)));
         FY_HIP(hipEventRecord(ev_usum0, stream));
         FY_HIP(hipStreamWaitEvent(comm_stream, ev_usum0, 0));
-        FY_TRY(launch_sum3(comm_stream, U.p + 3 * (size_t)g.c0, Nc, usum_partials.p));
+        if (!usum_valid) FY_TRY(launch_sum3(comm_stream, U.p + 3 * (size_t)g.c0, Nc, usum_partials.p));
+        usum_valid = false;
         FY_TRY(launch_reduce_finalize(comm_stream, usum_partials.p, Nc, 3, nullptr, xbar3.p));
         FY_HIP(hipEventRecord(ev_usum1, comm_stream));
         usum_pending = true;
@@ -656,6 +663,7 @@
 
     if (pimple && face_arrays) FY_TRY(FVK(launch_interp_alpha, stream, g, alpha.p, F3(alphaf)));
     const int nOuter = pimple ? std::max(cs.n_outer_correctors, 1) : 1;
+    const bool fold_div = pimple && stress_once && g.upwind < 3;
     for (int outer = 0; outer < nOuter; ++outer) {
         const bool final_outer = outer == nOuter - 1;
         g.u_relax = (final_outer && cs.u_relax_final > 0) ? cs.u_relax_final : cs.u_relax;
@@ -667,9 +675,11 @@
         clk_mom.begin(stream);
         if (pimple) {
             if (outer > 0) FY_TRY(halo_U());
-            FY_TRY(FVK(launch_pre_coupling, stream, g, U.p, p.p, alpha.p, C3(psn), vGrad.p, gradP.p, divT.p, Gt.p, g.upwind == 2 ? 1 : 0, 0));
-            FY_TRY(overlapped(XW_MOMENTUM, true, [&](hipStream_t on) { return halo(Gt.p + 2 * 3 * nstore, 3, plane, g.nz, g.gz, 1, on); },
-                              [&](const FvGeo& gw) { return FVK(launch_div_G, stream, gw, Gt.p, divG.p); }));
+            if (outer > 0 || !D_at_start)
+                FY_TRY(FVK(launch_pre_coupling, stream, g, U.p, p.p, alpha.p, C3(psn), vGrad.p, gradP.p, divT.p, Gt.p, g.upwind == 2 ? 1 : 0, 0));
+            if (!fold_div)
+                FY_TRY(overlapped(XW_MOMENTUM, true, [&](hipStream_t on) { return halo(Gt.p + 2 * 3 * nstore, 3, plane, g.nz, g.gz, 1, on); },
+                                  [&](const FvGeo& gw) { return FVK(launch_div_G, stream, gw, Gt.p, alpha.p, divG.p); }));
         }
         if (g.upwind == 2) FY_TRY(halo_cells(vGrad, 9, 1));
         if (g.upwind >= 3) {
@@ -677,8 +687,12 @@
             FY_TRY(FVK(launch_grad_magsqr, stream, g, U.p, gradL.p));
             FY_TRY(halo_cells(gradL, 3, 1));
         }
-        FY_TRY(FVK(launch_assemble_momentum, stream, g, U.p, Uold.p, alpha.p,  alpha.p, face_arrays ? C3(alphaf) : CFace3{}, phi_now(), uSource.p, uSourceDrag.p,
-                                        divG.p, g.upwind >= 3 ? gradL.p : vGrad.p, M7(), src.p, rAU.p));
+        {
+            FY_TRY(overlapped(XW_MOMENTUM, fold_div, [&](hipStream_t on) { return halo(Gt.p + 2 * 3 * nstore, 3, plane, g.nz, g.gz, 1, on); }, [&](const FvGeo& gw) {
+                return FVK(launch_assemble_momentum, stream, gw, U.p, Uold.p, alpha.p,  alpha.p, face_arrays ? C3(alphaf) : CFace3{}, phi_now(), uSource.p,
+                           uSourceDrag.p, divG.p, fold_div ? Gt.p : nullptr, g.upwind >= 3 ? gradL.p : vGrad.p, M7(), src.p, rAU.p);
+            }));
+        }
         rAU_new = true; hbya_ready = false;
         const bool bmom_fused = pimple && cs.momentum_predictor && fused_corrector;
         if (pimple) {
diff --git a/yade-openfoam-coupling_amd/csrc/fv_solver.hpp b/yade-openfoam-coupling_amd/csrc/fv_solver.hpp
--- a/yade-openfoam-coupling_amd/csrc/fv_solver.hpp
+++ b/yade-openfoam-coupling_amd/csrc/fv_solver.hpp
@@ -45,6 +45,7 @@
     hipEvent_t ev_usum0 = nullptr, ev_usum1 = nullptr;
     DevBuf<double> usum_partials;
     bool usum_pending = false;
+    bool carry_usum = true, usum_valid = false;
     bool coarse_pending = false, factor_pending = false, coarse_on_side = false, coarse_marked = false;
     int wait_coarse() { if (coarse_pending) { coarse_pending = false; FY_HIP(hipStreamWaitEvent(stream, ev_coarse, 0)); } return FY_OK; }
     int wait_factor() { FY_TRY(wait_coarse()); if (factor_pending) { factor_pending = false; FY_HIP(hipStreamWaitEvent(stream, ev_factor, 0)); } return FY_OK; }
@@ -207,6 +208,7 @@
     int precondition(const double* r_host, double* z_host);
     int prepare_p_init(bool with_halo = true);
     bool fused_corrector = true;
+    bool stress_once = true;
     bool hbya_ready = false;
     bool face_arrays = true;
     bool faces_from_cells = true;
diff --git a/yade-openfoam-coupling_amd/csrc/fv_solver_api.cpp b/yade-openfoam-coupling_amd/csrc/fv_solver_api.cpp
--- a/yade-openfoam-coupling_amd/csrc/fv_solver_api.cpp
+++ b/yade-openfoam-coupling_amd/csrc/fv_solver_api.cpp
@@ -141,6 +141,7 @@
     }
     s->s.carry_valid = false;
     s->s.p_sum_valid = false; s->s.p_ghosts_fresh = false;
+    s->s.usum_valid = false;
     if (std::string(name) == "U") {
         s->s.U_ghosts_fresh = false;
         FY_TRY(s->s.halo_U());
```

Result: no change. 205.6, median of 6 (+1.2%).
